# FocoosAI/focoos

Hardware: AMD Instinct MI355X
Metric: images/sec @ 640^2 (infer bs=32) (higher is better)
Workload: dtype bf16; 1 GPU; fai-detr-l-obj365 inference, bf16 MFMA, bs=32/GPU, 640x640, random-init weights (seed 0), uint8 HWC images resident in HBM, device post-process + D2H of packed detections included; global_batch=32, parallelism=replicas x1 (no data-path collective), steps_are=hipGraph replays, batches_in_flight=3, concurrent_batch_parts=1

## Files before the change

### focoos_amd/_lib.py

```python
from __future__ import annotations

import ctypes as C
import os
from typing import Optional

from .build import LIB_PATH, LIB_PATH_FP16

FX_ACT = {None: 0, "none": 0, "relu": 1, "silu": 2, "gelu": 3}


class FocoosAmdError(RuntimeError):
    pass


class FxConvDesc(C.Structure):
    _fields_ = [
        ("x", C.c_void_p), ("w", C.c_void_p), ("bias", C.c_void_p), ("residual", C.c_void_p), ("y", C.c_void_p),
        ("B", C.c_int32), ("H", C.c_int32), ("W", C.c_int32), ("C", C.c_int32), ("ldx", C.c_int32),
        ("Ho", C.c_int32), ("Wo", C.c_int32), ("N", C.c_int32), ("ldy", C.c_int32), ("ldr", C.c_int32),
        ("KH", C.c_int32), ("KW", C.c_int32), ("stride", C.c_int32), ("pad", C.c_int32),
        ("pool2", C.c_int32), ("act", C.c_int32), ("out_f32", C.c_int32), ("residual_after_act", C.c_int32),
        ("y_batch_stride", C.c_int64), ("w_frag", C.c_void_p), ("mask", C.c_void_p), ("ldm", C.c_int32), ("reserved0", C.c_int32),
    ]


def conv_frag_eligible(n: int, c: int, k: int, c32: bool = True) -> bool:
    if k == 1:
        return n % 256 == 0 and c % 256 == 0
    if k != 3:
        return False
    if c == 32:
        return c32 and n in (32, 64)
    return (n in (64, 128) or n % 256 == 0) and c % 64 == 0


class FxAugRecord(C.Structure):
    _fields_ = [
        ("crop_w", C.c_int32), ("crop_h", C.c_int32), ("pad_x", C.c_int32), ("pad_y", C.c_int32), ("res_w", C.c_int32), ("res_h", C.c_int32),
        ("crop_x", C.c_int32), ("crop_y", C.c_int32), ("flags", C.c_int32), ("reserved0", C.c_int32),
        ("brightness", C.c_float), ("contrast", C.c_float), ("saturation", C.c_float), ("reserved1", C.c_int32 * 3),
    ]


class FxPackEntry(C.Structure):
    _fields_ = [
        ("w", C.c_void_p), ("scale", C.c_void_p), ("bias", C.c_void_p), ("w_fwd", C.c_void_p), ("w_dgrad", C.c_void_p),
        ("w_fwd_frag", C.c_void_p), ("w_dgrad_frag", C.c_void_p), ("bias_out", C.c_void_p),
        ("N", C.c_int32), ("C", C.c_int32), ("KH", C.c_int32), ("KW", C.c_int32), ("ld_fwd", C.c_int32), ("ld_dgrad", C.c_int32),
        ("first_block", C.c_int32), ("n_offset", C.c_int32), ("n_total", C.c_int32), ("reserved", C.c_int32),
    ]


class FxPublishEntry(C.Structure):
    _fields_ = [
        ("w", C.c_void_p), ("bn_weight", C.c_void_p), ("bn_bias", C.c_void_p), ("bn_mean", C.c_void_p), ("bn_var", C.c_void_p),
        ("bias", C.c_void_p), ("w_rows", C.c_void_p), ("w_frag", C.c_void_p), ("bias_out", C.c_void_p), ("eps", C.c_double),
        ("N", C.c_int32), ("C", C.c_int32), ("KH", C.c_int32), ("KW", C.c_int32), ("Np", C.c_int32), ("first_block", C.c_int32),
    ]


class FxPwChainDesc(C.Structure):
    _fields_ = [
        ("x1", C.c_void_p), ("x2", C.c_void_p), ("residual", C.c_void_p), ("w1", C.c_void_p), ("bias1", C.c_void_p), ("y1", C.c_void_p),
        ("w2", C.c_void_p), ("bias2", C.c_void_p), ("y2", C.c_void_p),
        ("M", C.c_int32), ("K1a", C.c_int32), ("K1b", C.c_int32), ("N1", C.c_int32), ("N2", C.c_int32),
        ("ldx1", C.c_int32), ("ldx2", C.c_int32), ("ldr", C.c_int32), ("ldy1", C.c_int32), ("ldy2", C.c_int32),
        ("act1", C.c_int32), ("act2", C.c_int32),
        ("pool", C.c_void_p), ("ldp", C.c_int32), ("img_h", C.c_int32), ("img_w", C.c_int32), ("reserved0", C.c_int32),
    ]


class FxRcStage(C.Structure):
    _fields_ = [
        ("type", C.c_int32), ("K", C.c_int32), ("N", C.c_int32), ("act", C.c_int32),
        ("src", C.c_int32), ("dst", C.c_int32), ("aux", C.c_int32),
        ("ld", C.c_int32), ("ld2", C.c_int32), ("flags", C.c_int32),
        ("w", C.c_void_p), ("bias", C.c_void_p), ("gamma", C.c_void_p), ("beta", C.c_void_p), ("g0", C.c_void_p), ("g1", C.c_void_p),
    ]


class FxFrameDesc(C.Structure):
    _fields_ = [
        ("plane", C.c_void_p * 3), ("pitch", C.c_int32 * 3), ("height", C.c_int32), ("width", C.c_int32), ("format", C.c_int32),
        ("matrix", C.c_int32), ("reserved", C.c_int32 * 3),
    ]


_vp, _i, _f = C.c_void_p, C.c_int, C.c_float

SIGNATURES = {
    "fx_abi_version": [],
    "fx_build_flags": [],
    "fx_device_info": [_i, C.POINTER(C.c_int), C.c_char_p, _i],
    "fx_conv2d_nhwc_bf16": [C.POINTER(FxConvDesc), _vp],
    "fx_conv2d_variant": [_vp, C.c_char_p, _i],
    "fx_pw_chain_supported": [_i, _i, _i, _i],
    "fx_pw_chain_pool_supported": [_i, _i, _i, _i],
    "fx_conv3x3_flat_supported": [_i, _i, _i],
    "fx_pw_chain_bf16": [C.POINTER(FxPwChainDesc), _vp],
    "fx_stem_conv3x3s2": [_vp, _i, _vp, _vp, _vp, _vp, _vp, _i, _i, _i, _i, _vp],
    "fx_stem16_conv3x3s2": [_vp, _i, _vp, _vp, _vp, _vp, _vp, _i, _i, _i, _vp],
    "fx_conv3x3_c16_nhwc_bf16": [_vp, _i, _vp, _vp, _i, _vp, _i, _i, _i, _i, _i, _i, _i, _vp],
    "fx_semseg_eval_accumulate": [_vp, _vp, _i, _i, _i, _i, _i, _i, _i, _vp, C.c_int64, _vp, _vp, _i, _i, _vp, _vp, _vp, _vp, _vp],
    "fx_detr_eval_boxes_f32": [_vp, _vp, _vp, _i, _i, _i, _i, _vp, _vp, _vp, _vp, _vp],
    "fx_coco_match_workspace_bytes": [_i],
    "fx_coco_match_bbox": [_vp, _vp, _vp, _vp, _i, _i, _i, _vp, _vp, _vp, _vp, _vp, _vp, C.c_int64, _i, _vp, _vp, _vp, _vp, _vp, _vp, C.c_size_t,
                           _vp],
    "fx_mf_eval_masks_workspace_bytes": [_i, _i, _i],
    "fx_mf_eval_masks": [_vp, _vp, _vp, _i, _i, _i, _i, _i, _i, _i, _i, _vp, _vp, _vp, _vp, C.c_int64, _f, _vp, _vp, _vp, _vp, _vp, _vp, _vp, _vp,
                         _vp, _vp, C.c_size_t, _vp],
    "fx_coco_mask_inter": [_vp, _vp, _vp, C.c_int64, _vp, _vp, _vp, _i, _i, _i, _vp, _vp, _vp, _vp, _vp, C.c_int64, _vp, _vp, _vp, C.c_int64, _vp,
                           _vp, _vp],
    "fx_coco_match_segm": [_vp, _vp, _vp, _vp, _i, _i, _i, _i, _vp, _vp, _vp, _vp, _vp, _vp, _vp, C.c_int64, _i, _vp, _vp, _vp, _vp, _vp, _vp,
                           C.c_size_t, _vp],
    "fx_augment_images_u8": [_vp, _vp, _vp, _vp, _vp, C.c_int64, _vp, _vp, _i, _vp, _i, _i, _i, _vp, _vp],
    "fx_augment_labels": [_vp, _vp, _vp, _vp, _vp, _vp, C.c_int64, _vp, _vp, _vp, _i, _i, _vp, _i, _i, _i, _i, _vp, _vp],
    "fx_resize_bilinear_u8": [_vp, _i, _i, _vp, _i, _i, _vp],
    "fx_tile_gather_u8_f32": [_vp, _i, _i, _vp, _vp, _i, _vp, _i, _i, _vp],
    "fx_frames_ingest": [_vp, _vp, _i, _vp, _i, _i, _i, _vp],
    "fx_merge_detections_workspace_bytes": [_i, _i],
    "fx_merge_detections_nms": [_vp, _vp, _vp, _vp, _vp, _i, _i, _i, _i, _f, _i, _i, _vp, _vp, _vp, _vp, _vp, _vp, C.c_size_t, _vp],
    "fx_frames_tile_gather_f32": [_vp, _vp, _i, _vp, _vp, _i, _vp, _i, _i, _vp],
    "fx_roi_select": [_vp, _vp, _vp, _vp, _i, _i, _vp, _vp, _i, _vp, _vp, _vp, _vp, _vp, _vp, _i, _i, _i, _i, _f, _i, _vp, _vp, _vp, _vp, _vp],
    "fx_frames_roi_gather_f32": [_vp, _vp, _i, _vp, _i, _vp, _i, _i, _vp],
    "fx_roi_attributes": [_vp, _i, _vp, _vp, _i, _vp, _i, _i, _vp, _vp, _i, _vp, _vp, _vp, _vp, _vp, _i, _vp, _vp, _vp, _vp],
    "fx_merge_detections_batched_workspace_bytes": [_i, _i, _i],
    "fx_merge_detections_nms_batched": [_vp, _vp, _vp, _vp, _vp, _i, _i, _i, _i, _i, _f, _i, _i, _vp, _vp, _vp, _vp, _vp, _vp, C.c_size_t, _vp],
    "fx_annotate_labels_from_detections": [_vp, _vp, _vp, _vp, _i, _i, _vp, _vp, _i, _i, _i, _i, _i, _i, _vp, _vp],
    "fx_annotate_u8": [_vp, _vp, _i, _i, _i, _i, _i, _vp, _vp, _vp, _vp, _vp, _i, C.c_int64, _vp, _vp, _i, _i, _i, _i, _vp],
    "fx_track_update": [_vp, _vp, _vp, _vp, _i, _i, _vp, _vp, _vp, _vp, _vp, _vp, _vp, _vp, _i, _f, _f, _f, _f, _f, _i, _i, _f, _vp, _vp],
    "fx_track_reset": [_vp, _vp, _vp, _vp, _vp, _vp, _vp, _vp, _i, _i, _i, _vp],
    "fx_zone_update": [_vp, _vp, _vp, _i, _i, _vp, _vp, _i, _vp, _vp, _vp, _vp, _vp, _vp, _i, _i, _vp, _vp, _vp, _vp, _vp, _vp, _vp, _vp, _vp],
    "fx_zone_reset": [_vp, _vp, _vp, _vp, _vp, _i, _i, _i, _i, _vp],
    "fx_annotate_labels_tracked": [_vp, _vp, _vp, _vp, _vp, _i, _i, _vp, _vp, _i, _i, _i, _i, _i, _i, _vp, _vp],
    "fx_annotate_zone_records": [_vp, _vp, _vp, _vp, _vp, _vp, _i, _i, _vp, _vp, _vp, _vp, _vp, _i, _i, _i, _i, _i, _i, _vp, _vp],
    "fx_annotate_overlay_u8": [_vp, _vp, _i, _i, _i, _i, _i, _vp, _vp, _vp, _vp, _vp, _vp, _i, _i, _vp, _vp, _vp, _vp, _vp, _vp, _i, _i, _i, _i,
                               _vp],
    "fx_trace_update": [_vp, _vp, _vp, _i, _i, _vp, _vp, _i, _i, _vp, _vp, _vp, _vp, _vp, _vp],
    "fx_trace_reset": [_vp, _vp, _vp, _vp, _i, _i, _i, _vp],
    "fx_dwell_update": [_vp, _vp, _vp, _i, _i, _vp, _i, _vp, _vp, _vp, _vp, _vp, _vp, _i, _vp, _vp, _vp, _vp, _vp, _vp, _vp, _vp, _vp],
    "fx_dwell_reset": [_vp, _vp, _vp, _vp, _vp, _vp, _vp, _vp, _i, _i, _i, _i, _vp],
    "fx_heat_tiles": [_i, _i, _i],
    "fx_heat_update": [_vp, _vp, _vp, _vp, _i, _i, _i, _i, _i, _i, _i, _i, _i, _vp, _vp, _vp, _vp, _vp],
    "fx_annotate_heat_u8": [_vp, _vp, _i, _i, _i, _i, _i, _vp, _vp, _i, _i, _vp, _vp],
    "fx_redact_regions": [_vp, _vp, _vp, _i, _i, _vp, _i, _vp, _vp, _vp, _vp, _i, _i, _i, _i, _vp, _vp, _vp, _vp],
    "fx_redact_u8": [_vp, _vp, _i, _i, _i, _i, _vp, _vp, _vp, _i, _vp, _i, C.c_int64, _i, _i, _i, _i, _i, _i, _vp],
    "fx_mask_rle_workspace_bytes": [_i, _i, _i, _i],
    "fx_mask_rle_encode": [_vp, _vp, _vp, _i, _i, _i, _i, _i, _vp, _vp, _vp, _vp, C.c_size_t, _vp],
    "fx_mask_polygon_workspace_bytes": [_i, _i, _i, _i, _i],
    "fx_mask_polygon_encode": [_vp, _vp, _vp, _i, _i, _i, _i, _i, _i, _vp, _vp, _vp, _vp, C.c_size_t, _vp],
    "fx_maxpool3x3s2_nhwc_bf16": [_vp, _i, _vp, _i, _i, _i, _i, _i, _vp],
    "fx_stem_conv12_u8_bf16": [_vp, _vp, _vp, _vp, _vp, _vp, _vp, _vp, _i, _i, _i, _i, _vp],
    "fx_stem_conv_pool_supported": [_i, _i, _i, _i],
    "fx_stem_conv3x3_relu_maxpool_bf16": [_vp, _i, _vp, _vp, _vp, _i, _i, _i, _i, _vp],
    "fx_avgpool2x2_nhwc_bf16": [_vp, _i, _vp, _i, _i, _i, _i, _i, _vp],
    "fx_resize_bilinear_nhwc_bf16": [_vp, _i, _vp, _i, _i, _i, _i, _i, _i, _i, _vp],
    "fx_add_rows_bf16": [_vp, _i, _vp, _i, _i, _vp, _i, _i, _i, _vp],
    "fx_layernorm_bf16": [_vp, _i, _vp, _i, _vp, _vp, _vp, _i, _i, _i, _vp],
    "fx_mha_bf16": [_vp, _i, _vp, _i, _vp, _i, _vp, _i, _i, _i, _i, _i, _vp],
    "fx_mha_workspace_bytes": [_i, _i, _i, _i, _i],
    "fx_mha_masked_bf16": [_vp, _i, _vp, _i, _vp, _i, _vp, _i, _i, _i, _i, _i, _vp, _i, _vp, C.c_size_t, _vp],
    "fx_upsample_nearest_add_nhwc_bf16": [_vp, _i, _vp, _i, _vp, _i, _i, _i, _i, _i, _i, _i, _vp],
    "fx_upsample_nearest_bwd_nhwc_bf16": [_vp, _i, _vp, _i, _i, _i, _i, _i, _i, _i, _vp],
    "fx_query_pixel_logits_bf16": [_vp, _i, _vp, _i, _i, _vp, _i, _vp, _i, _i, _i, _i, _i, _vp],
    "fx_mf_class_head": [_vp, _i, _vp, _vp, _vp, _i, _i, _i, _vp],
    "fx_mf_upsample_probs_f32": [_vp, _i, _i, _vp, _i, _i, _i, _vp],
    "fx_mf_upsample_probs_bf16": [_vp, _i, _i, _vp, _i, _i, _i, _vp],
    "fx_mf_postprocess_workspace_bytes": [_i, _i, _i],
    "fx_mf_postprocess_workspace_bytes_fused": [_i, _i, _i, _i, _i, _i],
    "fx_mf_postprocess": [_vp, _i, _i, _i, _i, _vp, _vp, _i, _i, _f, _f, _i, _vp, C.c_size_t, _vp, _vp, _vp, _vp, _vp, _vp, _vp, _vp],
    "fx_msda_bf16": [_vp, _i, _vp, _vp, _i, _i, _vp, _i, _vp, _i, _vp, _i, _vp, _i, _i, _i, _i, _i, _vp],
    "fx_rowmax_f32": [_vp, _i, _vp, _i, _i, _vp],
    "fx_enc_score_head_bf16": [_vp, _i, _vp, _i, _vp, _vp, _vp, _vp, _f, _vp, _vp, _i, _vp, _i, _vp, _i, _vp],
    "fx_row_chain": [_vp, _i, _i, _i, _vp],
    "fx_topk_rows_f32": [_vp, _i, _i, _i, _i, _vp, _vp, _vp],
    "fx_topk_rows_workspace_bytes": [_i, _i, _i],
    "fx_topk_rows_ws_f32": [_vp, _i, _i, _i, _i, _vp, _vp, _vp, C.c_size_t, _vp],
    "fx_gather_rows_bf16": [_vp, _i, _i, _vp, _i, _vp, _i, _i, _i, _vp],
    "fx_fill_rows_bf16": [_vp, _i, _i, _vp, _i, _vp, _i, _i, _vp],
    "fx_linear_k4_relu": [_vp, _vp, _vp, _vp, _i, _i, _i, _vp],
    "fx_bbox_head": [_vp, _i, _vp, _vp, _vp, _vp, _vp, _i, _i, _vp, _vp, _i, _i, _vp],
    "fx_detr_head_out": [_vp, _i, _vp, _vp, _vp, _i, _i, _vp],
    "fx_detr_postprocess": [_vp, _vp, _vp, _vp, _i, _i, _i, _i, _f, _vp, _vp, _vp, _vp, _vp],
    "fx_detr_match_cost_f32": [_vp, _i, _vp, _vp, _vp, _vp, _i, _i, _i, _i, _f, _f, _f, _f, _f, _vp, _vp],
    "fx_lsa_f32": [_vp, _i, _i, _i, _vp, _vp, _vp, _vp],
    "fx_lsa_status_f32": [_vp, _i, _i, _i, _vp, _vp, _vp, _vp, _vp],
    "fx_detr_set_loss_workspace_bytes": [_i, _i, _i],
    "fx_detr_set_loss_f32": [_vp, _i, _vp, _vp, _vp, _vp, _vp, _vp, _i, _i, _i, _i, _f, _f, _f, _f, _f, _f, _vp, _vp, _vp],
    "fx_detr_box_loss_f32": [_vp, _vp, _vp, _vp, _vp, _vp, _i, _i, _i, _i, _f, _f, _vp, _vp, _vp, _vp, _vp],
    "fx_detr_box_loss_bwd_f32": [_vp, _vp, _vp, _i, _i, _i, _vp, _vp, _vp, _vp],
    "fx_msda_f32_fwd": [_vp, _vp, _vp, _i, _i, _vp, _vp, _vp, _i, _i, _i, _i, _vp],
    "fx_msda_f32_bwd": [_vp, _vp, _vp, _i, _i, _vp, _vp, _vp, _vp, _vp, _vp, _i, _i, _i, _i, _vp],
    "fx_msda_train_fwd": [_vp, _i, _i, _vp, _vp, _i, _i, _vp, _vp, _vp, _i, _i, _i, _i, _vp],
    "fx_msda_train_bwd": [_vp, _i, _i, _vp, _vp, _i, _i, _vp, _vp, _vp, _vp, _i, _i, _vp, _vp, _i, _i, _i, _i, _vp],
    "fx_msda_bwd_slab_supported": [_vp, _i, _i, _i, _i, _i],
    "fx_msda_prep_bf16": [_vp, _i, _vp, _i, _vp, _vp, _vp, _i, _i, _i, _i, _vp],
    "fx_msda_prep_bwd_bf16": [_vp, _vp, _vp, _vp, _vp, _i, _vp, _i, _i, _i, _i, _i, _vp],
    "fx_msda_train_bwd_slab": [_vp, _i, _i, _vp, _vp, _vp, _i, _i, _vp, _vp, _vp, _i, _vp, _i, _vp, _vp, _i, _i, _i, _i, _vp],
    "fx_adamw_workspace_bytes": [],
    "fx_adamw_step_f32": [_vp, _vp, _vp, _vp, C.c_int64, _vp, _vp, _vp, _vp, _i, _i, _f, _f, _f, _f, _vp, _vp, _vp],
    "fx_adamw_step_scaled_f32": [_vp, _vp, _vp, _vp, C.c_int64, _vp, _vp, _vp, _vp, _i, _f, _f, _f, _f, _vp, _vp, _vp, _f, _f, _i, _vp],
    "fx_conv2d_wgrad_nhwc_bf16": [_vp, _i, _vp, _i, _vp, _i, _i, _i, _i, _i, _i, _i, _i, _i, _i, _i, _vp],
    "fx_conv2d_wgrad_bias_nhwc_bf16": [_vp, _i, _vp, _i, _vp, _vp, _i, _i, _i, _i, _i, _i, _i, _i, _i, _i, _i, _vp],
    "fx_point_sample_f32": [_vp, _i, _i, _i, _vp, _vp, _vp, _vp, _i, _i, _vp],
    "fx_mask_match_cost_f32": [_vp, _i, _vp, _vp, _vp, _vp, _i, _i, _i, _i, _i, C.c_float, C.c_float, C.c_float, _i, _vp, _vp],
    "fx_mask_match_cost_workspace_bytes": [_i, _i, _i],
    "fx_mask_match_cost_ws_f32": [_vp, _i, _vp, _vp, _vp, _vp, _i, _i, _i, _i, _i, C.c_float, C.c_float, C.c_float, _i, _vp, _vp, C.c_size_t, _vp],
    "fx_mask_set_loss_workspace_bytes": [_i, _i, _i, _i],
    "fx_mask_set_loss_f32": [_vp, _i, _vp, _i, _i, _vp, _i, _i, _i, _vp, _vp, _i, _vp, _vp, _vp, _i, _vp, _i, _i, _i, _i, _i, C.c_float, C.c_float,
                             C.c_float, C.c_float, C.c_float, _vp, C.c_size_t, _vp, _vp],
    "fx_mask_set_loss_cls_f32": [_vp, _i, _vp, _i, _i, _vp, _i, _i, _i, _vp, _vp, _i, _vp, _vp, _vp, _i, _vp, _i, _i, _i, _i, _i, C.c_float, _i, C.c_float,
                                 C.c_float, C.c_float, C.c_float, C.c_float, C.c_float, _vp, C.c_size_t, _vp, _vp],
    "fx_mask_class_loss_workspace_bytes": [_i, _i],
    "fx_mask_class_loss_f32": [_vp, _i, _vp, _vp, _vp, _vp, _i, _i, _i, _i, C.c_float, C.c_float, C.c_float, C.c_float, _vp, C.c_size_t, _vp, _vp],
    "fx_mask_class_loss_bwd_f32": [_vp, _i, _vp, _vp, _vp, _vp, _i, _i, _i, _i, C.c_float, C.c_float, C.c_float, C.c_float, _vp, _vp, _i, _vp],
    "fx_dwconv3x3s2_nhwc_bf16": [_vp, _i, _vp, _vp, _vp, _i, _i, _i, _i, _i, _vp],
    "fx_dwconv3x3s2_nhwc_f32out": [_vp, _i, _vp, _vp, _vp, _i, _i, _i, _i, _i, _vp],
    "fx_global_mean_nhwc_bf16": [_vp, _i, _vp, _i, _i, _i, _i, _vp],
    "fx_pooled_linear_f32": [_vp, _i, _vp, _vp, _i, _vp, _i, _i, _i, _i, _vp],
    "fx_channel_gate_nhwc_bf16": [_vp, _i, _vp, _i, _i, _vp, _i, _vp, _i, _vp, _i, _i, _i, _i, _vp],
    "fx_seg_postprocess_workspace_bytes": [_i, _i, _i, _i, _i, _i],
    "fx_seg_postprocess": [_vp, _i, _i, _i, _i, _vp, _vp, _i, _i, C.c_float, _i, _vp, C.c_size_t, _vp, _vp, _vp, _vp, _vp, _vp, _vp, _vp, _vp],
    "fx_pack_conv_weights_f32": [_vp, _vp, _vp, _vp, _vp, _vp, _i, _i, _i, _i, _vp],
    "fx_unpack_conv_wgrad_f32": [_vp, _vp, _vp, _i, _i, _i, _i, _i, _i, _vp],
    "fx_linear_wgrad_bias_bf16": [_vp, _i, _vp, _i, _vp, _i, _vp, _i, _i, _i, _i, _i, _vp],
    "fx_conv2d_wgrad_splits": [_i, _i, _i, _i, _i, _i, _i],
    "fx_conv2d_wgrad_variant": [_i, _i, _i, _i, _i, _i, _i, _i, _i, C.c_char_p, _i],
    "fx_conv2d_wgrad_partial_nhwc_bf16": [_vp, _i, _vp, _i, _vp, C.c_int64, _i, _i, _i, _i, _i, _i, _i, _i, _i, _i, _i, _i, _vp],
    "fx_unpack_conv_wgrad_sum_f32": [_vp, C.c_int64, _i, _vp, _vp, _i, _i, _i, _i, _i, _i, _vp],
    "fx_relu_bwd_bf16": [_vp, _i, _vp, _i, _vp, _i, _vp, _i, C.c_int64, _i, _i, _vp],
    "fx_zero_insert2_nhwc_bf16": [_vp, _i, _vp, _i, _i, _i, _i, _i, _i, _i, _vp],
    "fx_avgpool2x2_bwd_nhwc_bf16": [_vp, _i, _vp, _i, _i, _i, _i, _i, _vp],
    "fx_maxpool3x3s2_bwd_nhwc_bf16": [_vp, _i, _vp, _i, _vp, _i, _i, _i, _i, _i, _vp, _vp],
    "fx_normalize_pad8": [_vp, _i, _vp, _vp, _vp, C.c_int64, _vp],
    "fx_stem_conv3x3s2_linear": [_vp, _i, _vp, _vp, _vp, _vp, _vp, _i, _i, _i, _i, _vp],
    "fx_bn_stats_bf16": [_vp, _i, _i, _vp, C.c_int64, _i, _vp],
    "fx_bn_finalize_f32": [_vp, C.c_float, _vp, _vp, C.c_float, C.c_float, _vp, _vp, _vp, _vp, _vp, _vp, _vp, _i, _vp],
    "fx_bn_apply_bf16": [_vp, _i, _i, _vp, _vp, _vp, _i, _i, _vp, _i, C.c_int64, _i, _vp],
    "fx_bn_bwd_stats_bf16": [_vp, _i, _vp, _i, _i, _vp, _i, _vp, _vp, _vp, _vp, _i, _vp, C.c_int64, _i, _vp],
    "fx_bn_bwd_apply_bf16": [_vp, _i, _vp, _i, _i, _vp, _i, _vp, _vp, _vp, _vp, _i, _vp, C.c_float, _vp, _i, _vp, _i, C.c_int64, _i, _vp, _vp, _vp],
    "fx_act_fwd_bf16": [_vp, _i, _vp, _i, C.c_int64, _i, _i, _vp],
    "fx_act_bwd_bf16": [_vp, _i, _vp, _i, _vp, _i, C.c_int64, _i, _i, _vp],
    "fx_colsum_bf16": [_vp, _i, _vp, C.c_int64, _i, _vp],
    "fx_layernorm_bwd_bf16": [_vp, _i, _vp, _i, _vp, _vp, _i, _vp, _vp, _i, _i, _vp],
    "fx_resize_bilinear_bwd_nhwc_bf16": [_vp, _i, _vp, _i, _i, _i, _i, _i, _i, _i, _vp],
    "fx_cast_f32_bf16": [_vp, _vp, C.c_int64, _vp],
    "fx_mha_bwd_workspace_bytes": [_i, _i, _i, _i],
    "fx_mha_bwd_bf16": [_vp, _i, _vp, _i, _vp, _i, _vp, _i, _vp, _i, _vp, _i, _vp, _i, _vp, _i, _i, _i, _i, _i, _vp, C.c_size_t, _vp],
    "fx_mha_masked_bwd_bf16": [_vp, _i, _vp, _i, _vp, _i, _vp, _i, _vp, _i, _vp, _i, _vp, _i, _i, _i, _i, _i, _vp, _i, _vp, C.c_size_t, _vp],
    "fx_mask_set_loss_bwd_f32": [_vp, _i, _vp, _i, _i, _vp, _i, _i, _i, _vp, _vp, _i, _vp, _vp, _vp, _i, _vp, _i, _i, _i, _i, _i, C.c_float, C.c_float,
                                 C.c_float, C.c_float, C.c_float, _vp, C.c_size_t, _vp, _vp, _i, _vp, _vp],
    "fx_mask_set_loss_cls_bwd_f32": [_vp, _i, _vp, _i, _i, _vp, _i, _i, _i, _vp, _vp, _i, _vp, _vp, _vp, _i, _vp, _i, _i, _i, _i, _i, C.c_float, _i, C.c_float,
                                     C.c_float, C.c_float, C.c_float, C.c_float, C.c_float, _vp, C.c_size_t, _vp, _vp, _i, _vp, _vp],
    "fx_planes_to_rows_bf16": [_vp, _i, _i, _vp, _i, _i, _i, _vp],
    "fx_dwconv3x3s2_bwd_nhwc_bf16": [_vp, _i, _vp, _i, _vp, _vp, _i, _vp, _i, _i, _i, _i, _vp],
    "fx_rowdot_nhwc_bf16": [_vp, _i, _vp, _i, C.c_float, _vp, _i, _i, _i, _i, _i, _vp],
    "fx_bcast_vec_nhwc_bf16": [_vp, _i, C.c_float, _vp, _i, _i, _i, _i, _vp],
    "fx_scatter_rows_bf16": [_vp, _i, _vp, _i, _vp, _i, _i, _i, _i, _vp],
    "fx_pack_entry_blocks": [_i, _i, _i, _i],
    "fx_pack_weights_many_f32": [_vp, _i, _i, _vp],
    "fx_pack_frag_bf16": [_vp, _vp, _i, _i, _vp],
    "fx_publish_entry_blocks": [_i, _i, _i, _i],
    "fx_publish_weights_f32": [_vp, _i, _i, _vp],
    "fx_pack_linear_weights_f32": [_vp, _vp, _vp, _vp, _vp, _i, _i, _i, _i, _vp],
    "fx_box_refine_f32": [_vp, _vp, _vp, C.c_int64, _f, _vp],
    "fx_box_refine_bwd_f32": [_vp, _vp, _vp, _vp, _vp, C.c_int64, _f, _vp],
    "fx_vfl_loss_bf16": [_vp, _i, _vp, _vp, _f, _f, _f, _vp, _vp, _i, C.c_int64, _i, _vp],
    "fx_stream_fork": [_vp, _vp],
    "fx_stream_join": [_vp, _vp],
    "fx_graph_begin": [_vp],
    "fx_graph_end": [_vp, C.POINTER(C.c_void_p)],
    "fx_graph_launch": [_vp, _vp],
    "fx_graph_destroy": [_vp],
    "fx_graph_time": [_vp, _vp, _i, C.POINTER(C.c_float)],
}

_libs: dict = {}
_DTYPE = [os.environ.get("FX_DTYPE", "bf16")]


def compute_dtype() -> str:
    return _DTYPE[0]


def set_compute_dtype(name: str) -> str:
    if name not in ("bf16", "fp16"):
        raise FocoosAmdError(f"compute dtype {name!r}: the engine has a bfloat16 and an fp16 (+ loss scale) build")
    prev, _DTYPE[0] = _DTYPE[0], name
    return prev


class using_compute_dtype:

    def __init__(self, name: str):
        self.name, self.prev = name, None

    def __enter__(self):
        self.prev = set_compute_dtype(self.name)
        return self

    def __exit__(self, *exc):
        _DTYPE[0] = self.prev
        return False


def act_dtype():
    import torch

    return torch.float16 if _DTYPE[0] == "fp16" else torch.bfloat16


def lib_path(name: str = None) -> str:
    if (name or _DTYPE[0]) == "fp16":
        return os.environ.get("FOCOOS_AMD_LIB_FP16", LIB_PATH_FP16)
    return os.environ.get("FOCOOS_AMD_LIB", LIB_PATH)


FX_ABI_VERSION = 27


def load(name: str = None) -> C.CDLL:
    name = name or _DTYPE[0]
    if name in _libs:
        return _libs[name]
    import torch
    path = lib_path(name)
# ... 54 lines not shown
```

### focoos_amd/csrc/conv_common.h

```cpp
#pragma once
#include "common.h"

#ifndef FX_K64_MIN_KTOT
#define FX_K64_MIN_KTOT 1024
#endif

struct ConvArgs {
  const bf16_t* x;
  const bf16_t* w;
  const float* bias;
  const bf16_t* res;
  void* y;
  int B, H, W, C, ldx;
  int Ho, Wo, N, ldy, ldr;
  int KH, KW, stride, pad;
  int act, out_f32, res_after;
  int M, Ktot, nNt, Nstore;
  unsigned x_bytes, w_bytes, r_bytes;
  int64_t y_bstride;
  const bf16_t* mask;
  int ldm;
  unsigned m_bytes;
};

template <int BK>
__device__ __forceinline__ int lds_off(int row, int chunk) {
  constexpr int CPR = BK / 8;
  if constexpr (BK >= 128) {
    return row * (BK * 2) + ((chunk ^ (row & 15)) << 4);
  } else {
    constexpr int R = 256 / (BK * 2);
    return row * (BK * 2) + ((chunk ^ ((row / R) & (CPR - 1))) << 4);
  }
}

int fx_tune(const char* env_name, int default_value);

__device__ __forceinline__ uint4 buf_load16(__amdgpu_buffer_rsrc_t r, unsigned byte_off) {
  return __builtin_bit_cast(uint4, __builtin_amdgcn_raw_buffer_load_b128(r, byte_off, 0, 0));
}
#define FX_OOB 0xFFFFFFF0u

__device__ __forceinline__ size_t fx_y_row_offset(int m, int ldy, int HW, int64_t y_bstride) {
  size_t yo = (size_t)m * ldy;
  if (y_bstride) {
    const int bb = m / HW;
    yo = (size_t)bb * y_bstride + (size_t)(m - bb * HW) * ldy;
  }
  return yo;
}

typedef int (*ConvLauncher)(const ConvArgs& c, const bf16_t* w_frag, int mode, hipStream_t stream);
int fx_c3_epilogue_mode(int act, bool has_res, int res_after);

int fx_conv_dma_bn(const ConvArgs& a);
int fx_launch_conv_dma256(const ConvArgs& c, const bf16_t* w_frag, int mode, hipStream_t stream);
int fx_launch_conv_dma128(const ConvArgs& c, const bf16_t* w_frag, int mode, hipStream_t stream);

extern "C" int fx_conv3x3_flat_supported(int C, int N, int W);
bool fx_conv3x3_flat_fits(int C, int N, int W);
int fx_launch_conv3x3_flat(const ConvArgs& c, const bf16_t* w_frag, int mode, hipStream_t stream);
int fx_launch_pw_flat(const ConvArgs& c, const bf16_t* w_frag, int mode, hipStream_t stream);
bool fx_conv3x3_kplane_supported(int C, int N, int W);
int fx_c3k_small_m_max();
int fx_launch_conv3x3_kplane(const ConvArgs& c, const bf16_t* w_frag, int mode, hipStream_t stream);
bool fx_conv3x3s2_kplane_supported(int C, int N, int Wo, int M);
int fx_launch_conv3x3s2_kplane(const ConvArgs& c, const bf16_t* w_frag, int mode, hipStream_t stream);
bool fx_pw_kplane_supported(int C, int N, int mode);
int fx_launch_pw_kplane(const ConvArgs& c, const bf16_t* w_frag, int mode, hipStream_t stream);
bool fx_conv3x3_c32_supported(int C, int N, int W, int mode);
int fx_launch_conv3x3_c32(const ConvArgs& c, const bf16_t* w_frag, int mode, hipStream_t stream);
```

### focoos_amd/csrc/conv_igemm.hip

```cpp
#include <stdio.h>

#include "conv_common.h"

template <int BM, int BN, int BK, int WM, int WN, bool POOL, int NSTAGE = 2>
__global__ __launch_bounds__(256, (BK == 32 ? 4 : 2)) void conv_igemm_kernel(const ConvArgs p) {
  constexpr int CPR = BK / 8, RPP = 256 / CPR;
  constexpr int A_PASS = BM / RPP, B_PASS = (BN + RPP - 1) / RPP;
  constexpr int WTM = BM / WM, WTN = BN / WN, TM = WTM / 32, TN = WTN / 32;
  constexpr int A_BYTES = BM * BK * 2, B_BYTES = BN * BK * 2, STAGE = A_BYTES + B_BYTES;
  constexpr int EPI_LD = BN + 4;
  static_assert(WM * WN == 4, "4 waves");
  static_assert(BM % RPP == 0, "A passes");
  extern __shared__ __attribute__((aligned(16))) unsigned char smem[];

  const int tid = threadIdx.x, lane = tid & 63, wave = tid >> 6;
  const int wm = wave / WN, wn = wave % WN;
  const int bid = fx_xcd_remap(blockIdx.x, gridDim.x);
  const int mt = bid / p.nNt, nt = bid % p.nNt;
  const int m0 = mt * BM, n0 = nt * BN;

  const __amdgpu_buffer_rsrc_t xr = __builtin_amdgcn_make_buffer_rsrc((void*)p.x, 0, p.x_bytes, 0x00020000);
  const __amdgpu_buffer_rsrc_t wr = __builtin_amdgcn_make_buffer_rsrc((void*)p.w, 0, p.w_bytes, 0x00020000);

  const int kc = tid % CPR, r_in = tid / CPR;
// ... 201 lines not shown
        } else {
          bf16_t* dst = reinterpret_cast<bf16_t*>(p.y) + yoff;
          *reinterpret_cast<uint4*>(dst) = pack_bf16x8(v);
        }
      }
    }
    if (hh + 1 < BM / HALF) __syncthreads();
  }
}

template <int BM, int BN, int BK, int WM, int WN, bool POOL, int NSTAGE = 2>
static int launch_conv(const ConvArgs& c, const bf16_t*, int, hipStream_t stream) {
  constexpr int STAGE = (BM + BN) * BK * 2;
  constexpr int EPI = 64 * (BN + 4) * 4;
  constexpr int SMEM = (NSTAGE * STAGE > EPI) ? NSTAGE * STAGE : EPI;
  auto kern = conv_igemm_kernel<BM, BN, BK, WM, WN, POOL, NSTAGE>;
  static int attr_smem = 0;
  if (!fx_ensure_dyn_smem(reinterpret_cast<const void*>(kern), SMEM, attr_smem)) return FX_ERR_RUNTIME;
  ConvArgs a = c;
  a.nNt = (a.N + BN - 1) / BN;
  int nMt = (a.M + BM - 1) / BM;
  dim3 grid(nMt * a.nNt), block(256);
  hipLaunchKernelGGL(kern, grid, block, SMEM, stream, a);
  return fx_launch_status();
}

static int conv_prepare(const fx_conv_desc* d, ConvArgs& a) {
  FX_CHECK_ARG(d && d->x && d->w && d->y);
  FX_CHECK_ARG(d->B > 0 && d->H > 0 && d->W > 0 && d->Ho > 0 && d->Wo > 0 && d->N > 0);
  FX_CHECK_ARG(d->C > 0 && d->C % 32 == 0 && d->ldx >= d->C && d->ldx % 8 == 0);
  FX_CHECK_ARG(d->KH >= 1 && d->KW >= 1 && d->stride >= 1 && d->pad >= 0);
  const int Nstore = (d->N + 7) / 8 * 8;
  FX_CHECK_ARG(d->ldy >= Nstore && d->ldy % 8 == 0);
  FX_CHECK_ARG(!d->residual || (d->ldr >= Nstore && d->ldr % 8 == 0));
  FX_CHECK_ARG(((uintptr_t)d->x % 16) == 0 && ((uintptr_t)d->w % 16) == 0 && ((uintptr_t)d->y % 16) == 0);
  FX_CHECK_ARG(!d->residual || ((uintptr_t)d->residual % 16) == 0);
  FX_CHECK_ARG(!d->bias || ((uintptr_t)d->bias % 16) == 0);
  if (d->pool2) {
    FX_CHECK_ARG(d->KH == 1 && d->KW == 1 && d->stride == 1 && d->pad == 0);
    FX_CHECK_ARG(d->Ho == (d->H + 1) / 2 && d->Wo == (d->W + 1) / 2);
  } else {
    FX_CHECK_ARG(d->Ho == (d->H + 2 * d->pad - d->KH) / d->stride + 1);
    FX_CHECK_ARG(d->Wo == (d->W + 2 * d->pad - d->KW) / d->stride + 1);
  }
  if ((int64_t)d->B * d->H * d->W >= (1ll << 31) || (int64_t)d->B * d->Ho * d->Wo >= (1ll << 31)) return FX_ERR_UNSUPPORTED;
  const int64_t x_bytes = ((int64_t)d->B * d->H * d->W - 1) * d->ldx * 2 + (int64_t)d->C * 2;
  const int64_t Npad = (int64_t)(d->N + 127) / 128 * 128;
  const int64_t w_bytes = Npad * d->KH * d->KW * d->C * 2;
  const int64_t r_bytes = d->residual ? (((int64_t)d->B * d->Ho * d->Wo - 1) * d->ldr + Nstore) * 2 : 0;
  if (x_bytes >= 0xFFFFFFF0ll || w_bytes >= 0xFFFFFFF0ll || r_bytes >= 0xFFFFFFF0ll) return FX_ERR_UNSUPPORTED;
  a.x = reinterpret_cast<const bf16_t*>(d->x);
  a.w = reinterpret_cast<const bf16_t*>(d->w);
  a.bias = d->bias;
  a.res = reinterpret_cast<const bf16_t*>(d->residual);
  a.y = d->y;
  a.B = d->B; a.H = d->H; a.W = d->W; a.C = d->C; a.ldx = d->ldx;
  a.Ho = d->Ho; a.Wo = d->Wo; a.N = d->N; a.ldy = d->ldy; a.ldr = d->ldr;
  a.KH = d->KH; a.KW = d->KW; a.stride = d->stride; a.pad = d->pad;
  a.act = d->act; a.out_f32 = d->out_f32; a.res_after = d->residual_after_act;
  a.y_bstride = d->y_batch_stride;
  FX_CHECK_ARG(d->y_batch_stride >= 0 && d->y_batch_stride % 8 == 0);
  a.M = d->B * d->Ho * d->Wo;
  a.Ktot = d->KH * d->KW * d->C;
  a.Nstore = Nstore;
  a.nNt = 0;
  a.x_bytes = (unsigned)x_bytes;
  a.w_bytes = (unsigned)w_bytes;
  a.r_bytes = (unsigned)r_bytes;
  a.mask = reinterpret_cast<const bf16_t*>(d->mask);
  a.ldm = d->ldm;
  a.m_bytes = 0;
  if (d->mask) {
    FX_CHECK_ARG(d->ldm >= Nstore && d->ldm % 8 == 0 && ((uintptr_t)d->mask % 16) == 0 && !d->out_f32 && !d->pool2);
    const int64_t m_bytes = (((int64_t)d->B * d->Ho * d->Wo - 1) * d->ldm + Nstore) * 2;
    if (m_bytes >= 0xFFFFFFF0ll) return FX_ERR_UNSUPPORTED;
    a.m_bytes = (unsigned)m_bytes;
  }
  return FX_OK;
}

enum ConvRoute {
  R_C32, R_C3K, R_C3_FLAT, R_C3_S2, R_PWK, R_PW_FLAT, R_SMALL_M, R_DMA256, R_DMA128, R_POOL,
  R_K64_N128, R_K64_N64, R_K64_N32, R_K32_N128, R_K32_N64, R_K32_N32, R_UNSUPPORTED
};

static const struct {
  const char* label;
  bool by_c;
  ConvLauncher launch;
} kRoutes[R_UNSUPPORTED] = {
     {"conv3x3_c32<%d>", false, fx_launch_conv3x3_c32},
     {"conv3x3_kplane<%d>", false, fx_launch_conv3x3_kplane},
     {"conv3x3_flat<%d>", false, fx_launch_conv3x3_flat},
     {"conv3x3s2_kplane<%d>", false, fx_launch_conv3x3s2_kplane},
     {"pw_kplane<K%d>", true, fx_launch_pw_kplane},
     {"pw_flat<K%d>", true, fx_launch_pw_flat},
     {"conv_igemm<64,64,256,1stage>", false, launch_conv<64, 64, 256, 2, 2, false, 1>},
     {"conv_igemm_dma<256,256>", false, fx_launch_conv_dma256},
     {"conv_igemm_dma<256,128>", false, fx_launch_conv_dma128},
     {"conv_igemm<128,128,64,pool>", false, launch_conv<128, 128, 64, 2, 2, true>},
     {"conv_igemm<128,128,64>", false, launch_conv<128, 128, 64, 2, 2, false>},
     {"conv_igemm<128,64,64>", false, launch_conv<128, 64, 64, 2, 2, false>},
     {"conv_igemm<128,32,64>", false, launch_conv<128, 32, 64, 4, 1, false>},
     {"conv_igemm<128,128,32>", false, launch_conv<128, 128, 32, 2, 2, false>},
     {"conv_igemm<128,64,32>", false, launch_conv<128, 64, 32, 2, 2, false>},
     {"conv_igemm<128,32,32>", false, launch_conv<128, 32, 32, 4, 1, false>},
};

static ConvRoute conv_route(const fx_conv_desc* d, const ConvArgs& a, int mode) {
  const bool frag = d->w_frag && ((uintptr_t)d->w_frag % 16) == 0 && !d->mask && !d->pool2 && !d->out_f32;
  const int c3_min_m = fx_tune("FX_CONV3_MIN_M", 5000), pw_min_m = fx_tune("FX_PW_MIN_M", 5000);
  static const int c3_on = fx_tune("FX_CONV3_FLAT", 1), c3k_on = fx_tune("FX_C3_KPLANE", 1), c32_on = fx_tune("FX_C3_C32", 1);
  if (frag && c3_on && d->stride == 1 && d->KH == 3 && d->KW == 3 && d->pad == 1 && !d->y_batch_stride &&
      ((mode >= 0 && mode <= 3) || mode == 5) && a.M >= c3_min_m) {
    if (d->C == 32) {
      if (c32_on && fx_conv3x3_c32_supported(d->C, d->N, d->W, mode)) return R_C32;
    } else if (c3k_on && fx_conv3x3_kplane_supported(d->C, d->N, d->W)) {
      return R_C3K;
    } else if (fx_conv3x3_flat_fits(d->C, d->N, d->W)) {
      return R_C3_FLAT;
    }
  }
  static const int pw_on = fx_tune("FX_PW_FLAT", 1), pwk_on = fx_tune("FX_PW_KPLANE", 1);
  if (frag && pw_on && d->stride == 1 && d->KH == 1 && d->KW == 1 && d->pad == 0 && d->C % 256 == 0 && d->N % 256 == 0 && a.M >= pw_min_m &&
      (mode == 0 || mode == 1 || (mode >= 3 && mode <= 6)))
    return (pwk_on && fx_pw_kplane_supported(d->C, d->N, mode)) ? R_PWK : R_PW_FLAT;
  static const int s2_on = fx_tune("FX_C3S2_KPLANE", 1);
  if (frag && s2_on && d->stride == 2 && d->KH == 3 && d->KW == 3 && d->pad == 1 && !d->residual && d->H == 2 * d->Ho && d->W == 2 * d->Wo &&
      a.M >= c3_min_m && (mode == 0 || mode == 1 || mode == 3) && fx_conv3x3s2_kplane_supported(d->C, d->N, d->Wo, a.M))
    return R_C3_S2;
  static const int k64_min = fx_tune("FX_K64_MIN_KTOT", FX_K64_MIN_KTOT);
  static const int small_m = fx_tune("FX_SMALL_M", 16384);
  static const int small_k = fx_tune("FX_SMALL_M_KTOT", 2048);
  if (!d->pool2 && a.M <= small_m && d->C % 256 == 0 && a.Ktot <= small_k) return R_SMALL_M;
  if (!d->pool2 && !d->mask) {
    const int bn = fx_conv_dma_bn(a);
    if (bn) return bn == 256 ? R_DMA256 : R_DMA128;
  }
  if (d->pool2) return d->C % 64 != 0 ? R_UNSUPPORTED : R_POOL;
  if ((d->C % 64 == 0) && (a.Ktot >= k64_min)) return d->N > 64 ? R_K64_N128 : (d->N > 32 ? R_K64_N64 : R_K64_N32);
  return d->N > 64 ? R_K32_N128 : (d->N > 32 ? R_K32_N64 : R_K32_N32);
}

extern "C" int fx_conv2d_nhwc_bf16(const fx_conv_desc* d, fx_stream_t stream) {
  ConvArgs a;
  const int rc = conv_prepare(d, a);
  if (rc != FX_OK) return rc;
  const int mode = fx_c3_epilogue_mode(a.act, a.res != nullptr, a.res_after);
  const ConvRoute r = conv_route(d, a, mode);
  if (r == R_UNSUPPORTED) return FX_ERR_UNSUPPORTED;
  return kRoutes[r].launch(a, reinterpret_cast<const bf16_t*>(d->w_frag), mode, reinterpret_cast<hipStream_t>(stream));
}

extern "C" int fx_conv2d_variant(const fx_conv_desc* d, char* out, int cap) {
  FX_CHECK_ARG(out && cap >= 48);
  ConvArgs a;
  const int rc = conv_prepare(d, a);
  if (rc != FX_OK) return rc;
  const ConvRoute r = conv_route(d, a, fx_c3_epilogue_mode(a.act, a.res != nullptr, a.res_after));
  if (r == R_UNSUPPORTED) return FX_ERR_UNSUPPORTED;
  snprintf(out, cap, kRoutes[r].label, kRoutes[r].by_c ? d->C : d->N);
  return FX_OK;
}
```

### focoos_amd/csrc/conv_pw_kplane.hip

```cpp
#include "kplane_common.h"

#ifndef FX_PWK_RES_DEPTH
#define FX_PWK_RES_DEPTH 3
#endif

int fx_tune(const char* env_name, int default_value);

struct PWKArgs {
  const bf16_t* x;
  const bf16_t* wp;
  const float* bias;
  const bf16_t* res;
  bf16_t* y;
  int N, ldx, ldy, ldr, M;
  int ntg;
  int HW;
  int64_t y_bstride;
  unsigned x_bytes, r_bytes;
  int rot;
};

template <int K, int ACT, int RESMODE, int TM = 4, int ABL = 0>
__global__ __launch_bounds__(256, TM == 4 ? 2 : 3) void conv_pw_kplane_kernel(const PWKArgs p) {
  constexpr int TN = 2, NW = 4, BM = TM * 32, BN = 256;
  constexpr int NTHR = 256, NDW = NTHR / 64;
  constexpr int KS = K / 16;
  constexpr int PLANE = BM * 16, XBYTES = 2 * KS * PLANE;
  constexpr int PF = 4;
  static_assert(KS % PF == 0 && (KS - 1) * PLANE < 65536, "plane offsets are 16-bit immediates");
  extern __shared__ __attribute__((aligned(16))) unsigned char smem[];
  float* biasL = reinterpret_cast<float*>(smem + XBYTES);

  const int tid = threadIdx.x, lane = tid & 63;
  const int wave = __builtin_amdgcn_readfirstlane(tid >> 6);
  const int l32 = lane & 31, half = lane >> 5;
  const int m0 = fx_xcd_remap(blockIdx.x, gridDim.x) * BM;
  const int nt_first = blockIdx.y * p.ntg;
  const int NT = min(p.N / BN, nt_first + p.ntg);
  const int cnt = NT - nt_first;
  const int rot = p.rot ? (int)(blockIdx.x % (unsigned)cnt) : 0;
  auto tile_of = [&](int k) { const int t = k + rot; return nt_first + (t >= cnt ? t - cnt : t); };

  for (int i = tid; i < p.N; i += NTHR) biasL[i] = p.bias ? p.bias[i] : 0.0f;
  {
    const __amdgpu_buffer_rsrc_t xr = __builtin_amdgcn_make_buffer_rsrc((void*)p.x, 0, p.x_bytes, 0x00020000);
    constexpr int NP = K / 8;
    static_assert(BM % 64 == 0, "64-row DMA blocks");
    for (int i = wave; i < (BM / 64) * NP; i += NDW) {
      const int blk = i / NP, c = i % NP;
      const int m = m0 + blk * 64 + lane;
      const int pln = (c & 1) * KS + (c >> 1);
      if constexpr (!(ABL & 16)) pw_dma16(xr, smem + pln * PLANE + blk * 1024, m < p.M ? (unsigned)(m * p.ldx + c * 8) * 2u : FX_OOB);
    }
  }
  f32x16 acc[TN][TM];
  bf16x8 ar[PF][TN];
  const unsigned wvoff = lane * 16;
  const bf16_t* wwave = p.wp + (size_t)(wave * TN) * KS * 512;
  auto w_ptr = [&](int a, int nt, int ks) -> const bf16_t* { return wwave + ((size_t)(nt * 8 + a) * KS + ks) * 512; };
#pragma unroll
  for (int a = 0; a < TN; ++a) {
    const bf16_t* w0 = w_ptr(a, tile_of(0), 0);
    c3_static_for<PF>([&](auto ic) {
      constexpr int i = decltype(ic)::value;
      ar[i][a] = bf16x8{0, 0, 0, 0, 0, 0, 0, 0};
      kp_ldg<i * 1024>(ar[i][a], wvoff, w0);
    });
  }
  const int lds0 = (int)(unsigned)(size_t)((__attribute__((address_space(3))) unsigned char*)smem);
  int addr[TM];
#pragma unroll
  for (int b = 0; b < TM; ++b) addr[b] = lds0 + (b * 32 + l32) * 16 + half * KS * PLANE;
  asm volatile("s_waitcnt vmcnt(0)" ::: "memory");
  __syncthreads();

  for (int kt = 0; kt < cnt; ++kt) {
    const int nt = tile_of(kt);
    const int n0 = nt * BN;
    const int ntn = kt + 1 < cnt ? tile_of(kt + 1) : nt;
#pragma unroll
    for (int a = 0; a < TN; ++a)
#pragma unroll
      for (int gq = 0; gq < 4; ++gq) {
        const float4 bb = *reinterpret_cast<const float4*>(biasL + n0 + (wave * TN + a) * 32 + 8 * gq + 4 * half);
#pragma unroll
        for (int b = 0; b < TM; ++b) {
          acc[a][b][4 * gq] = bb.x; acc[a][b][4 * gq + 1] = bb.y; acc[a][b][4 * gq + 2] = bb.z; acc[a][b][4 * gq + 3] = bb.w;
        }
      }
    bf16x8 xb[2][TM];
#pragma unroll
    for (int b = 0; b < TM; ++b) xb[0][b] = kp_lds_read<0>(addr[b]);
#pragma unroll 1
    for (int g = 0; g < KS / PF; ++g) {
      const bool last = g == KS / PF - 1;
      const bf16_t* wnext[TN];
#pragma unroll
      for (int a = 0; a < TN; ++a) wnext[a] = w_ptr(a, last ? ntn : nt, last ? 0 : (g + 1) * PF);
      const int aoff = g * PF * PLANE;
      auto kstep = [&](auto jc) {
        constexpr int j = decltype(jc)::value;
        if constexpr (TN == 1) c3_wait<(PF - 1) * TN>(ar[j][0]); else c3_wait<(PF - 1) * TN>(ar[j][0], ar[j][1]);
#pragma unroll
        for (int a = 0; a < TN; ++a) {
#pragma unroll
          for (int b = 0; b < TM; ++b) {
            if constexpr (!(ABL & 8)) acc[a][b] = FX_MFMA_32x32x16(ar[j][a], xb[j & 1][b], acc[a][b]);
            if (a == 0) {
              if constexpr (j + 1 < PF) xb[(j + 1) & 1][b] = kp_lds_read<(j + 1) * PLANE>(addr[b] + aoff);
              else xb[0][b] = kp_lds_read<PF * PLANE>(addr[b] + (last ? -PF * PLANE : aoff));
            }
            if constexpr (!(ABL & 1)) {
              if (b == TM - 1) kp_ldg<j * 1024>(ar[j][a], wvoff, wnext[a]);
            }
            __builtin_amdgcn_sched_barrier(0);
          }
        }
      };
      c3_static_for<PF>(kstep);
    }
    constexpr int RD = (FX_PWK_RES_DEPTH < TM) ? FX_PWK_RES_DEPTH : TM;
    constexpr int RS = RD + 1 > TM ? TM : RD + 1;
    uint4 rr[RS][TN * 2];
    if constexpr (ABL & 4) {
#pragma unroll
      for (int i = 0; i < RS * TN * 2; ++i) (&rr[0][0])[i] = make_uint4(0, 0, 0, 0);
    }
    auto ld_res = [&](int b, uint4* dst) {
      const int m = min(m0 + b * 32 + l32, p.M - 1);
      const bf16_t* rrow = p.res + (size_t)m * p.ldr + n0 + wave * TN * 32 + half * 8;
#pragma unroll
      for (int a = 0; a < TN; ++a)
#pragma unroll
        for (int g2 = 0; g2 < 2; ++g2) dst[a * 2 + g2] = *reinterpret_cast<const uint4*>(rrow + a * 32 + g2 * 16);
    };
    if constexpr (RESMODE != 0 && !(ABL & 4)) {
#pragma unroll
      for (int b = 0; b < RD && b < TM; ++b) ld_res(b, rr[b % RS]);
    }
#pragma unroll
    for (int b = 0; b < TM; ++b) {
      if constexpr (RESMODE != 0 && !(ABL & 4)) {
        if (b + RD < TM) ld_res(b + RD, rr[(b + RD) % RS]);
      }
      const int row = b * 32 + l32;
      const int m = m0 + row;
      bf16_t* yrow = p.y + fx_y_row_offset(m, p.ldy, p.HW, p.y_bstride) + n0 + wave * TN * 32 + half * 8;
      const bool live = m < p.M;
#pragma unroll
      for (int a = 0; a < TN; ++a)
#pragma unroll
        for (int g2 = 0; g2 < 2; ++g2) {
          unsigned pk[2][2], rq[2][2] = {{0u, 0u}, {0u, 0u}};
          if constexpr (RESMODE != 0) {
            const uint4 R = rr[b % RS][a * 2 + g2];
            rq[0][0] = R.x; rq[0][1] = R.y; rq[1][0] = R.z; rq[1][1] = R.w;
            kp_swap_rows(rq);
          }
#pragma unroll
          for (int q = 0; q < 2; ++q) {
            const int gq = 2 * g2 + q;
            float v[4];
            const float r[4] = {bf16lo_to_f32(rq[q][0]), bf16hi_to_f32(rq[q][0]), bf16lo_to_f32(rq[q][1]),
                                bf16hi_to_f32(rq[q][1])};
#pragma unroll
            for (int e = 0; e < 4; ++e) {
              v[e] = acc[a][b][4 * gq + e];
              if constexpr (RESMODE == 1) v[e] += r[e];
              v[e] = kp_act<ACT>(v[e]);
              if constexpr (RESMODE == 3) v[e] = r[e] > 0.0f ? v[e] : 0.0f;
            }
            pk[q][0] = pack_bf16x2(v[0], v[1]);
            pk[q][1] = pack_bf16x2(v[2], v[3]);
          }
          kp_swap_rows(pk);
          if (live && !((ABL & 2) && p.M > 0)) *reinterpret_cast<uint4*>(yrow + a * 32 + g2 * 16) = make_uint4(pk[0][0], pk[0][1], pk[1][0], pk[1][1]);
        }
    }
  }
#pragma unroll
  for (int i = 0; i < PF; ++i) {
    if constexpr (TN == 1) c3_wait<0>(ar[i][0]); else c3_wait<0>(ar[i][0], ar[i][1]);
  }
}

template <int K, int ACT, int RESMODE, int TM = 4, int ABL = 0>
static int launch_pwk(PWKArgs& a, hipStream_t stream) {
  constexpr int BM = TM * 32, BN = 256;
  const int smem = BM * K * 2 + a.N * 4;
  if (smem > 160 * 1024) return FX_ERR_UNSUPPORTED;
  const int mt = (a.M + BM - 1) / BM, NT = a.N / BN;
  static const int target = fx_tune("FX_PWK_TARGET_WGS", 512);
  const int want = K == 256 ? target : target / 2;
  int groups = mt >= want * 3 / 4 ? 1 : (want + mt - 1) / mt;
  if (groups > NT) groups = NT;
  a.ntg = (NT + groups - 1) / groups;
  groups = (NT + a.ntg - 1) / a.ntg;
  static const int rot = fx_tune("FX_PWK_ROT", 1);
  a.rot = rot;
  auto kern = conv_pw_kplane_kernel<K, ACT, RESMODE, TM, ABL>;
  static int attr_smem = 0;
  if (!fx_ensure_dyn_smem(reinterpret_cast<const void*>(kern), smem, attr_smem)) return FX_ERR_RUNTIME;
  hipLaunchKernelGGL(kern, dim3(mt, groups), dim3(256), smem, stream, a);
  return fx_launch_status();
}

bool fx_pw_kplane_supported(int C, int N, int mode) {
  if (N <= 0 || N % 256 != 0 || N > 4096) return false;
  static const int k512_res = fx_tune("FX_PWK_K512_RES", 1);
  if (C == 256) return mode == 0 || mode == 1 || mode == 3 || mode == 4 || mode == 5 || mode == 6;
  if (C == 512) return mode == 0 || mode == 1 || mode == 3 || (k512_res && (mode == 4 || mode == 5 || mode == 6));
  return false;
}

int fx_launch_pw_kplane(const ConvArgs& c, const bf16_t* w_frag, int mode, hipStream_t stream) {
  if (!fx_pw_kplane_supported(c.C, c.N, mode)) return FX_ERR_UNSUPPORTED;
  PWKArgs a{};
  a.x = c.x; a.wp = w_frag; a.bias = c.bias; a.res = c.res; a.y = reinterpret_cast<bf16_t*>(c.y);
  a.N = c.N; a.ldx = c.ldx; a.ldy = c.ldy; a.ldr = c.ldr; a.M = c.M;
  a.HW = c.Ho * c.Wo; a.y_bstride = c.y_bstride; a.x_bytes = c.x_bytes; a.r_bytes = c.r_bytes;
  if (c.C == 256) {
    switch (mode) {
      case 0: return launch_pwk<256, FX_ACT_RELU, 0>(a, stream);
      case 1: return launch_pwk<256, FX_ACT_SILU, 0>(a, stream);
      case 3: return launch_pwk<256, FX_ACT_NONE, 0>(a, stream);
      case 4: return launch_pwk<256, FX_ACT_RELU, 1>(a, stream);
      case 5: return launch_pwk<256, FX_ACT_NONE, 3>(a, stream);
      case 6: return launch_pwk<256, FX_ACT_NONE, 1>(a, stream);
    }
  } else {
    switch (mode) {
      case 0: return launch_pwk<512, FX_ACT_RELU, 0>(a, stream);
      case 1: return launch_pwk<512, FX_ACT_SILU, 0>(a, stream);
      case 3: return launch_pwk<512, FX_ACT_NONE, 0>(a, stream);
      case 4: return launch_pwk<512, FX_ACT_RELU, 1>(a, stream);
      case 5: return launch_pwk<512, FX_ACT_NONE, 3>(a, stream);
      case 6: return launch_pwk<512, FX_ACT_NONE, 1>(a, stream);
    }
  }
  return FX_ERR_UNSUPPORTED;
}
```

### focoos_amd/csrc/pixel_ops.hip

```cpp
#include <stdlib.h>

#include "common.h"

static int fx_env_int(const char* name, int dflt) {
  const char* v = getenv(name);
  return v ? atoi(v) : dflt;
}

template <typename TIn, bool RELU>
__global__ __launch_bounds__(256) void stem_conv_kernel(const TIn* __restrict__ x, const float* __restrict__ wt ,
                                                         const float* __restrict__ bias, const float* __restrict__ mean,
                                                         const float* __restrict__ inv_std, bf16_t* __restrict__ y, int B, int H,
                                                         int W, int Ho, int Wo) {
  __shared__ __attribute__((aligned(16))) float ws[27 * 32];
  for (int i = threadIdx.x; i < 27 * 32; i += 256) ws[i] = wt[i];
  __syncthreads();
  const int total = B * Ho * Wo;
  const int gid = blockIdx.x * 256 + threadIdx.x;
  const int o = gid >> 2, cg = gid & 3;
  if (o >= total) return;
  const int b = o / (Ho * Wo), rem = o - b * Ho * Wo;
  const int ho = rem / Wo, wo = rem - ho * Wo;
  const float m0 = mean[0], m1 = mean[1], m2 = mean[2], s0 = inv_std[0], s1 = inv_std[1], s2 = inv_std[2];
  float acc[8];
  {
    float4 b0 = *reinterpret_cast<const float4*>(bias + cg * 8), b1 = *reinterpret_cast<const float4*>(bias + cg * 8 + 4);
    acc[0] = b0.x; acc[1] = b0.y; acc[2] = b0.z; acc[3] = b0.w; acc[4] = b1.x; acc[5] = b1.y; acc[6] = b1.z; acc[7] = b1.w;
  }
#pragma unroll 1
  for (int kh = 0; kh < 3; ++kh) {
    const int hi = ho * 2 - 1 + kh;
    const int hc = min(max(hi, 0), H - 1);
#pragma unroll
    for (int kw = 0; kw < 3; ++kw) {
      const int wi = wo * 2 - 1 + kw;
      const int wc = min(max(wi, 0), W - 1);
      const bool ok = (hi == hc) && (wi == wc);
      const TIn* px = x + ((int64_t)(b * H + hc) * W + wc) * 3;
      float v[3] = {ok ? ((float)px[0] - m0) * s0 : 0.0f, ok ? ((float)px[1] - m1) * s1 : 0.0f, ok ? ((float)px[2] - m2) * s2 : 0.0f};
#pragma unroll
      for (int c = 0; c < 3; ++c) {
        const float* wr = ws + ((kh * 3 + kw) * 3 + c) * 32 + cg * 8;
        float4 w0 = *reinterpret_cast<const float4*>(wr), w1 = *reinterpret_cast<const float4*>(wr + 4);
        acc[0] = fmaf(v[c], w0.x, acc[0]); acc[1] = fmaf(v[c], w0.y, acc[1]); acc[2] = fmaf(v[c], w0.z, acc[2]); acc[3] = fmaf(v[c], w0.w, acc[3]);
        acc[4] = fmaf(v[c], w1.x, acc[4]); acc[5] = fmaf(v[c], w1.y, acc[5]); acc[6] = fmaf(v[c], w1.z, acc[6]); acc[7] = fmaf(v[c], w1.w, acc[7]);
      }
    }
  }
  if (RELU) {
#pragma unroll
    for (int n = 0; n < 8; ++n) acc[n] = fmaxf(acc[n], 0.0f);
  }
  *reinterpret_cast<uint4*>(y + (int64_t)o * 32 + cg * 8) = pack_bf16x8(acc);
}

__device__ __forceinline__ void stem_run8(__amdgpu_buffer_rsrc_t r, int a, unsigned& lo, unsigned& hi, unsigned& b8) {
  const unsigned a4 = (unsigned)a & ~3u;
  const unsigned sh = (unsigned)a & 3u;
  const unsigned d0 = __builtin_amdgcn_raw_buffer_load_b32(r, a4, 0, 0);
  const unsigned d1 = __builtin_amdgcn_raw_buffer_load_b32(r, a4 + 4u, 0, 0);
  const unsigned d2 = __builtin_amdgcn_raw_buffer_load_b32(r, a4 + 8u, 0, 0);
  lo = __builtin_amdgcn_alignbyte(d1, d0, sh);
  hi = __builtin_amdgcn_alignbyte(d2, d1, sh);
  b8 = (sh == 0 ? d2 : __builtin_amdgcn_alignbyte(0u, d2, sh)) & 0xffu;
}

__device__ __forceinline__ void stem_run9_f32(__amdgpu_buffer_rsrc_t r, int elem, float* f, float& f8) {
  const unsigned off = (unsigned)elem * 4u;
#pragma unroll
  for (int j = 0; j < 8; ++j) f[j] = __uint_as_float(__builtin_amdgcn_raw_buffer_load_b32(r, off + 4u * j, 0, 0));
  f8 = __uint_as_float(__builtin_amdgcn_raw_buffer_load_b32(r, off + 32u, 0, 0));
}

template <typename TIn, bool RELU>
__global__ __launch_bounds__(256) void stem_mfma_kernel(const TIn* __restrict__ x, unsigned x_bytes, const float* __restrict__ wt ,
                                                         const float* __restrict__ bias, const float* __restrict__ mean,
                                                         const float* __restrict__ inv_std, bf16_t* __restrict__ y, int B, int H, int W, int Ho,
                                                         int Wo, int tiles_per_wave) {
  const int lane = threadIdx.x & 63, wave = threadIdx.x >> 6;
  const int col = lane & 31, hh = lane >> 5;
  const __amdgpu_buffer_rsrc_t xr = __builtin_amdgcn_make_buffer_rsrc((void*)x, 0, x_bytes, 0x00020000);
  bf16x8 a1, a2;
  {
    float f1[8], f2[8];
#pragma unroll
    for (int j = 0; j < 8; ++j) {
      const int rr1 = hh ? 2 : 0;
      f1[j] = wt[((rr1 * 3 + j / 3) * 3 + j % 3) * 32 + col];
      if (hh == 0) f2[j] = wt[((1 * 3 + j / 3) * 3 + j % 3) * 32 + col];
      else f2[j] = j < 3 ? wt[((j * 3 + 2) * 3 + 2) * 32 + col] : 0.0f;
    }
    a1 = __builtin_bit_cast(bf16x8, pack_bf16x8(f1));
    a2 = __builtin_bit_cast(bf16x8, pack_bf16x8(f2));
  }
  const float m0 = mean[0], m1 = mean[1], m2 = mean[2], s0 = inv_std[0], s1 = inv_std[1], s2 = inv_std[2];
  const float mj[8] = {m0, m1, m2, m0, m1, m2, m0, m1}, sj[8] = {s0, s1, s2, s0, s1, s2, s0, s1};
  float bs[16];
#pragma unroll
  for (int r = 0; r < 16; ++r) bs[r] = bias[(r & 3) + 8 * (r >> 2) + 4 * hh];
  const int total = B * Ho * Wo;
  const int tile0 = (blockIdx.x * 4 + wave) * tiles_per_wave;
#pragma unroll 1
  for (int ti = 0; ti < tiles_per_wave; ++ti) {
    const int o = (tile0 + ti) * 32 + col;
    if ((tile0 + ti) * 32 >= total) break;
    const bool act = o < total;
    const int oo = act ? o : total - 1;
    const int b = oo / (Ho * Wo), rem = oo - b * Ho * Wo;
    const int ho = rem / Wo, wo = rem - ho * Wo;
    const int wi0 = 2 * wo - 1;
    const bool c0 = wi0 >= 0, c2 = wi0 + 2 < W;
    auto run = [&](int rr, float* f, float& f8) {
      const int hi_ = 2 * ho - 1 + rr;
      const bool rv = act && hi_ >= 0 && hi_ < H;
      const bool neg = wi0 < 0;
      const int elem = rv ? ((b * H + hi_) * W + (neg ? 0 : wi0)) * 3 : 0;
      float raw[8], raw8;
      if (sizeof(TIn) == 1) {
        unsigned lo, hi, b8;
        stem_run8(xr, elem, lo, hi, b8);
        if (neg) {
          b8 = (hi >> 8) & 0xffu;
          hi = __builtin_amdgcn_alignbyte(hi, lo, 1);
          lo = __builtin_amdgcn_alignbyte(lo, 0u, 1);
        }
        const unsigned w[2] = {lo, hi};
#pragma unroll
        for (int j = 0; j < 8; ++j) raw[j] = (float)((w[j >> 2] >> (8 * (j & 3))) & 0xffu);
        raw8 = (float)b8;
      } else {
        float t[8], t8;
        stem_run9_f32(xr, elem, t, t8);
#pragma unroll
        for (int j = 0; j < 8; ++j) raw[j] = neg ? (j >= 3 ? t[j - 3] : 0.0f) : t[j];
        raw8 = neg ? t[5] : t8;
      }
#pragma unroll
      for (int j = 0; j < 8; ++j) {
        const bool ok = rv && (j < 3 ? c0 : (j < 6 ? true : c2));
        f[j] = ok ? (raw[j] - mj[j]) * sj[j] : 0.0f;
      }
      f8 = (rv && c2) ? (raw8 - m2) * s2 : 0.0f;
    };
    float f1[8], fb[8], ta, tb;
    run(hh ? 2 : 0, f1, ta);
    run(1, fb, tb);
    const float ta_row0 = __shfl_xor(ta, 32, 64);
    float f2[8];
#pragma unroll
    for (int j = 0; j < 8; ++j) f2[j] = hh ? 0.0f : fb[j];
    if (hh) f2[0] = ta_row0, f2[1] = tb, f2[2] = ta;
    const bf16x8 b1 = __builtin_bit_cast(bf16x8, pack_bf16x8(f1)), b2 = __builtin_bit_cast(bf16x8, pack_bf16x8(f2));
    f32x16 acc;
#pragma unroll
    for (int r = 0; r < 16; ++r) acc[r] = bs[r];
    acc = FX_MFMA_32x32x16(a1, b1, acc);
    acc = FX_MFMA_32x32x16(a2, b2, acc);
    if (act) {
#pragma unroll
      for (int g = 0; g < 4; ++g) {
        float v0 = acc[4 * g], v1 = acc[4 * g + 1], v2 = acc[4 * g + 2], v3 = acc[4 * g + 3];
        if (RELU) v0 = fmaxf(v0, 0.0f), v1 = fmaxf(v1, 0.0f), v2 = fmaxf(v2, 0.0f), v3 = fmaxf(v3, 0.0f);
        uint2 pk;
        pk.x = pack_bf16x2(v0, v1);
        pk.y = pack_bf16x2(v2, v3);
        *reinterpret_cast<uint2*>(y + (int64_t)o * 32 + 8 * g + 4 * hh) = pk;
      }
    }
  }
}

static int stem_launch(const void* x, int in_f32, const float* w, const float* bias, const float* mean, const float* inv_std, void* y, int B,
                       int H, int W, int Cout, int relu, fx_stream_t stream_) {
  FX_CHECK_ARG(x && w && bias && mean && inv_std && y && B > 0 && H > 0 && W > 0);
  if (Cout != 32) return FX_ERR_UNSUPPORTED;
  int Ho = (H + 2 - 3) / 2 + 1, Wo = (W + 2 - 3) / 2 + 1;
  int64_t total = (int64_t)B * Ho * Wo;
  if (total * 4 >= (1ll << 31)) return FX_ERR_UNSUPPORTED;
  int grid = (int)((total * 4 + 255) / 256);
  hipStream_t stream = reinterpret_cast<hipStream_t>(stream_);
#define STEM_GO(T, R) \
  hipLaunchKernelGGL((stem_conv_kernel<T, R>), dim3(grid), dim3(256), 0, stream, (const T*)x, w, bias, mean, inv_std, (bf16_t*)y, B, H, W, Ho, Wo)
  const int64_t x_bytes = (int64_t)B * H * W * 3 * (in_f32 ? 4 : 1);
  static const int use_mfma = fx_env_int("FX_STEM_MFMA", 1);
  if (use_mfma && x_bytes < 0xFFFFFFF0ll) {
    const unsigned x_records = (unsigned)((x_bytes + 3) & ~3ll);
    const int tiles = (int)((total + 31) / 32);
    const int tpw = 8;
    const int blocks = (tiles + 4 * tpw - 1) / (4 * tpw);
#define STEM_MFMA(T, R)                                                                                                                       \
  hipLaunchKernelGGL((stem_mfma_kernel<T, R>), dim3(blocks), dim3(256), 0, stream, (const T*)x, x_records, w, bias, mean, inv_std, (bf16_t*)y, B, H, \
                     W, Ho, Wo, tpw)
    if (in_f32) {
      if (relu) STEM_MFMA(float, true); else STEM_MFMA(float, false);
    } else {
      if (relu) STEM_MFMA(uint8_t, true); else STEM_MFMA(uint8_t, false);
    }
#undef STEM_MFMA
    return fx_launch_status();
  }
  if (in_f32) {
    if (relu) STEM_GO(float, true); else STEM_GO(float, false);
  } else {
    if (relu) STEM_GO(uint8_t, true); else STEM_GO(uint8_t, false);
  }
#undef STEM_GO
  return fx_launch_status();
}

extern "C" int fx_stem_conv3x3s2(const void* x, int in_f32, const float* w, const float* bias, const float* mean, const float* inv_std,
                                 void* y, int B, int H, int W, int Cout, fx_stream_t stream_) {
  return stem_launch(x, in_f32, w, bias, mean, inv_std, y, B, H, W, Cout, 1, stream_);
}

extern "C" int fx_stem_conv3x3s2_linear(const void* x, int in_f32, const float* w, const float* bias, const float* mean, const float* inv_std,
                                        void* y, int B, int H, int W, int Cout, fx_stream_t stream_) {
  return stem_launch(x, in_f32, w, bias, mean, inv_std, y, B, H, W, Cout, 0, stream_);
}

__device__ __forceinline__ void bilinear_src(int dst, float scale, int in_size, int& i0, int& i1, float& l0, float& l1) {
  float src = scale * ((float)dst + 0.5f) - 0.5f;
  src = src < 0.0f ? 0.0f : src;
  i0 = (int)src;
  if (i0 > in_size - 1) i0 = in_size - 1;
  i1 = i0 + ((i0 < in_size - 1) ? 1 : 0);
  l1 = src - (float)i0;
  l0 = 1.0f - l1;
}

__global__ __launch_bounds__(256) void resize_u8_kernel(const uint8_t* __restrict__ x, int H, int W, float* __restrict__ y, int Ho,
                                                         int Wo, float sh, float sw) {
  int total = Ho * Wo * 3;
  for (int i = blockIdx.x * 256 + threadIdx.x; i < total; i += gridDim.x * 256) {
    int c = i % 3, p = i / 3;
    int wo = p % Wo, ho = p / Wo;
    int h0, h1, w0, w1;
    float lh0, lh1, lw0, lw1;
    bilinear_src(ho, sh, H, h0, h1, lh0, lh1);
    bilinear_src(wo, sw, W, w0, w1, lw0, lw1);
    float p00 = x[((int64_t)h0 * W + w0) * 3 + c], p01 = x[((int64_t)h0 * W + w1) * 3 + c];
    float p10 = x[((int64_t)h1 * W + w0) * 3 + c], p11 = x[((int64_t)h1 * W + w1) * 3 + c];
    y[i] = lh0 * (lw0 * p00 + lw1 * p01) + lh1 * (lw0 * p10 + lw1 * p11);
  }
}

extern "C" int fx_resize_bilinear_u8(const uint8_t* x, int H, int W, float* y, int Ho, int Wo, fx_stream_t stream_) {
  FX_CHECK_ARG(x && y && H > 0 && W > 0 && Ho > 0 && Wo > 0);
  int total = Ho * Wo * 3;
  int grid = (total + 255) / 256;
  if (grid > 4096) grid = 4096;
  hipLaunchKernelGGL(resize_u8_kernel, dim3(grid), dim3(256), 0, reinterpret_cast<hipStream_t>(stream_), x, H, W, y, Ho, Wo,
                     (float)H / (float)Ho, (float)W / (float)Wo);
  return fx_launch_status();
}

__global__ __launch_bounds__(256) void resize_nhwc_kernel(const bf16_t* __restrict__ x, int ldx, bf16_t* __restrict__ y, int ldy, int B,
                                                           int H, int W, int C8, int c8_shift, int bpr, int Ho, int Wo, float sh, float sw) {
  const unsigned bid = (unsigned)fx_xcd_remap(blockIdx.x, gridDim.x);
  const unsigned row = bid / (unsigned)bpr;
  const unsigned t = (bid - row * (unsigned)bpr) * 256u + threadIdx.x;
  if (t >= (unsigned)(Wo * C8)) return;
  const unsigned b = row / (unsigned)Ho, ho = row - b * (unsigned)Ho;
  const unsigned wo = c8_shift >= 0 ? t >> c8_shift : t / (unsigned)C8;
  const unsigned c8 = t - wo * (unsigned)C8;
  int h0, h1, w0, w1;
  float lh0, lh1, lw0, lw1;
  bilinear_src((int)ho, sh, H, h0, h1, lh0, lh1);
  bilinear_src((int)wo, sw, W, w0, w1, lw0, lw1);
  const bf16_t* base = x + (int64_t)b * H * W * ldx + c8 * 8;
  float f00[8], f01[8], f10[8], f11[8], o[8];
  unpack_bf16x8(*reinterpret_cast<const uint4*>(base + ((int64_t)h0 * W + w0) * ldx), f00);
  unpack_bf16x8(*reinterpret_cast<const uint4*>(base + ((int64_t)h0 * W + w1) * ldx), f01);
  unpack_bf16x8(*reinterpret_cast<const uint4*>(base + ((int64_t)h1 * W + w0) * ldx), f10);
  unpack_bf16x8(*reinterpret_cast<const uint4*>(base + ((int64_t)h1 * W + w1) * ldx), f11);
#pragma unroll
  for (int j = 0; j < 8; ++j) o[j] = lh0 * (lw0 * f00[j] + lw1 * f01[j]) + lh1 * (lw0 * f10[j] + lw1 * f11[j]);
  *reinterpret_cast<uint4*>(y + ((int64_t)row * Wo + wo) * ldy + c8 * 8) = pack_bf16x8(o);
}

extern "C" int fx_resize_bilinear_nhwc_bf16(const void* x, int ldx, void* y, int ldy, int B, int H, int W, int C, int Ho, int Wo,
                                            fx_stream_t stream_) {
  FX_CHECK_ARG(x && y && B > 0 && H > 0 && W > 0 && Ho > 0 && Wo > 0 && C > 0 && C % 8 == 0);
  FX_CHECK_ARG(ldx >= C && ldy >= C && ldx % 8 == 0 && ldy % 8 == 0);
  const int C8 = C / 8;
  const int64_t per_row = (int64_t)Wo * C8;
  const int64_t bpr = (per_row + 255) / 256;
  const int64_t grid = (int64_t)B * Ho * bpr;
  if (per_row >= (1ll << 31) || grid >= (1ll << 31)) return FX_ERR_UNSUPPORTED;
  const int shift = (C8 & (C8 - 1)) == 0 ? __builtin_ctz((unsigned)C8) : -1;
  hipLaunchKernelGGL(resize_nhwc_kernel, dim3((unsigned)grid), dim3(256), 0, reinterpret_cast<hipStream_t>(stream_), (const bf16_t*)x, ldx,
                     (bf16_t*)y, ldy, B, H, W, C8, shift, (int)bpr, Ho, Wo, (float)H / (float)Ho, (float)W / (float)Wo);
  return fx_launch_status();
}

__global__ __launch_bounds__(256) void maxpool_kernel(const bf16_t* __restrict__ x, int ldx, bf16_t* __restrict__ y, int ldy, int B, int H,
                                                       int W, int C8, int Ho, int Wo) {
  int64_t total = (int64_t)B * Ho * Wo * C8;
  const int bid = fx_xcd_remap(blockIdx.x, gridDim.x);
  for (int64_t i = (int64_t)bid * 256 + threadIdx.x; i < total; i += (int64_t)gridDim.x * 256) {
    int c8 = (int)(i % C8);
    int64_t p = i / C8;
    int wo = (int)(p % Wo);
    int64_t q = p / Wo;
    int ho = (int)(q % Ho), b = (int)(q / Ho);
    float m[8];
#pragma unroll
    for (int j = 0; j < 8; ++j) m[j] = -INFINITY;
#pragma unroll
    for (int kh = 0; kh < 3; ++kh) {
      int hi = ho * 2 - 1 + kh;
      if ((unsigned)hi >= (unsigned)H) continue;
#pragma unroll
      for (int kw = 0; kw < 3; ++kw) {
        int wi = wo * 2 - 1 + kw;
        if ((unsigned)wi >= (unsigned)W) continue;
        float f[8];
        unpack_bf16x8(*reinterpret_cast<const uint4*>(x + ((int64_t)(b * H + hi) * W + wi) * ldx + c8 * 8), f);
#pragma unroll
        for (int j = 0; j < 8; ++j) m[j] = fmaxf(m[j], f[j]);
      }
    }
    *reinterpret_cast<uint4*>(y + p * ldy + c8 * 8) = pack_bf16x8(m);
  }
}

extern "C" int fx_maxpool3x3s2_nhwc_bf16(const void* x, int ldx, void* y, int ldy, int B, int H, int W, int C, fx_stream_t stream_) {
  FX_CHECK_ARG(x && y && B > 0 && H > 0 && W > 0 && C > 0 && C % 8 == 0 && ldx >= C && ldy >= C && ldx % 8 == 0 && ldy % 8 == 0);
  int Ho = (H + 2 - 3) / 2 + 1, Wo = (W + 2 - 3) / 2 + 1;
  int64_t total = (int64_t)B * Ho * Wo * (C / 8);
  int64_t grid = (total + 255) / 256;
  if (grid > 256 * 256) grid = 256 * 256;
  hipLaunchKernelGGL(maxpool_kernel, dim3((int)grid), dim3(256), 0, reinterpret_cast<hipStream_t>(stream_), (const bf16_t*)x, ldx,
                     (bf16_t*)y, ldy, B, H, W, C / 8, Ho, Wo);
  return fx_launch_status();
}

__global__ __launch_bounds__(256) void avgpool2_kernel(const bf16_t* __restrict__ x, int ldx, bf16_t* __restrict__ y, int ldy, int B, int H,
                                                        int W, int C8, int Ho, int Wo) {
  int64_t total = (int64_t)B * Ho * Wo * C8;
  const int bid = fx_xcd_remap(blockIdx.x, gridDim.x);
  for (int64_t i = (int64_t)bid * 256 + threadIdx.x; i < total; i += (int64_t)gridDim.x * 256) {
    int c8 = (int)(i % C8);
    int64_t p = i / C8;
    int wo = (int)(p % Wo);
    int64_t q = p / Wo;
    int ho = (int)(q % Ho), b = (int)(q / Ho);
    float s[8] = {0, 0, 0, 0, 0, 0, 0, 0};
    int cnt = 0;
#pragma unroll
    for (int dy = 0; dy < 2; ++dy)
#pragma unroll
      for (int dx = 0; dx < 2; ++dx) {
        int hi = 2 * ho + dy, wi = 2 * wo + dx;
        if (hi < H && wi < W) {
          float f[8];
          unpack_bf16x8(*reinterpret_cast<const uint4*>(x + ((int64_t)(b * H + hi) * W + wi) * ldx + c8 * 8), f);
#pragma unroll
          for (int j = 0; j < 8; ++j) s[j] += f[j];
          ++cnt;
        }
      }
    float inv = 1.0f / (float)cnt;
#pragma unroll
    for (int j = 0; j < 8; ++j) s[j] *= inv;
    *reinterpret_cast<uint4*>(y + p * ldy + c8 * 8) = pack_bf16x8(s);
  }
}

extern "C" int fx_avgpool2x2_nhwc_bf16(const void* x, int ldx, void* y, int ldy, int B, int H, int W, int C, fx_stream_t stream_) {
  FX_CHECK_ARG(x && y && B > 0 && H > 0 && W > 0 && C > 0 && C % 8 == 0 && ldx >= C && ldy >= C && ldx % 8 == 0 && ldy % 8 == 0);
  int Ho = (H + 1) / 2, Wo = (W + 1) / 2;
  int64_t total = (int64_t)B * Ho * Wo * (C / 8);
  int64_t grid = (total + 255) / 256;
  if (grid > 256 * 32) grid = 256 * 32;
  hipLaunchKernelGGL(avgpool2_kernel, dim3((int)grid), dim3(256), 0, reinterpret_cast<hipStream_t>(stream_), (const bf16_t*)x, ldx,
                     (bf16_t*)y, ldy, B, H, W, C / 8, Ho, Wo);
  return fx_launch_status();
}
```

### focoos_amd/csrc/resize_common.h

```cpp
#pragma once
#include "common.h"

__device__ __forceinline__ void fx_resize_src(int dst, float scale, int in_size, int& i0, int& i1, float& l0, float& l1) {
#pragma clang fp contract(off)
  float src = fmaf(scale, (float)dst + 0.5f, -0.5f);
  src = src < 0.0f ? 0.0f : src;
  i0 = (int)src;
  if (i0 > in_size - 1) i0 = in_size - 1;
  i1 = i0 + ((i0 < in_size - 1) ? 1 : 0);
  l1 = src - (float)i0;
  l0 = 1.0f - l1;
}

__device__ __forceinline__ float fx_resize_filter(float lh0, float lh1, float lw0, float lw1, float p00, float p01, float p10, float p11) {
#pragma clang fp contract(off)
  const float top = fmaf(lw1, p01, lw0 * p00), bottom = fmaf(lw1, p11, lw0 * p10);
  return fmaf(lh0, top, lh1 * bottom);
}

static inline bool fx_windows_ok(const int32_t* wh, int N, int H, int W) {
  for (int i = 0; i < N; ++i) {
    const int x0 = wh[4 * i], y0 = wh[4 * i + 1], w = wh[4 * i + 2], h = wh[4 * i + 3];
    if (w <= 0 || h <= 0 || x0 < 0 || y0 < 0 || x0 > W - w || y0 > H - h) return false;
  }
  return true;
}
```

### focoos_amd/csrc/score_head.hip

```cpp
#include "pw_common.h"

struct ScoreHeadArgs {
  const bf16_t* mem;
  const uint8_t* valid;
  const bf16_t* w1p;
  const bf16_t* w2p;
  const float* b1;
  const float* gamma;
  const float* beta;
  const float* b2;
  bf16_t* om;
  float* scores;
  int ldm, ldo, S, M;
  float eps;
  unsigned mem_bytes;
};

template <int TN2>
__global__ __launch_bounds__(256, 2) void score_head_kernel(const ScoreHeadArgs p) {
  constexpr int BM = 64, TM = 2, KS = 16, PF = 4;
  extern __shared__ __attribute__((aligned(16))) unsigned char smem[];
  unsigned char* T = smem;
  float* red = reinterpret_cast<float*>(smem + BM * 512);

  const int tid = threadIdx.x, lane = tid & 63;
  const int wave = __builtin_amdgcn_readfirstlane(tid >> 6);
  const int l32 = lane & 31, half = lane >> 5;
  const int m0 = blockIdx.x * BM;

  const __amdgpu_buffer_rsrc_t mr = __builtin_amdgcn_make_buffer_rsrc((void*)p.mem, 0, p.mem_bytes, 0x00020000);
  for (int i = wave; i < BM * 32 / 64; i += 4) {
    const int q = i * 64 + lane;
    const int row = q >> 5, pc = q & 31;
    const int lc = pc ^ (row & 15);
    const int m = m0 + row;
    bool ok = m < p.M;
    if (ok && p.valid) ok = p.valid[m % p.S] != 0;
    pw_dma16(mr, T + i * 1024, ok ? (unsigned)(m * p.ldm + lc * 8) * 2u : FX_OOB);
  }

  f32x16 acc[2][TM];
#pragma unroll
  for (int a = 0; a < 2; ++a)
#pragma unroll
    for (int gq = 0; gq < 4; ++gq) {
      const float4 bb = *reinterpret_cast<const float4*>(p.b1 + wave * 64 + a * 32 + 8 * gq + 4 * half);
#pragma unroll
      for (int b = 0; b < TM; ++b) {
        acc[a][b][4 * gq] = bb.x; acc[a][b][4 * gq + 1] = bb.y; acc[a][b][4 * gq + 2] = bb.z; acc[a][b][4 * gq + 3] = bb.w;
      }
    }
  const bf16_t* w1 = p.w1p + (size_t)(wave * 2 * KS) * 512 + lane * 8;
  bf16x8 a1[PF][2];
#pragma unroll
  for (int i = 0; i < PF; ++i) {
    a1[i][0] = pw_ldg_frag(w1 + i * 512);
    a1[i][1] = pw_ldg_frag(w1 + (KS + i) * 512);
  }
  asm volatile("s_waitcnt vmcnt(0)" ::: "memory");
  __syncthreads();
#pragma unroll 1
  for (int ks0 = 0; ks0 < KS; ks0 += PF) {
    int l32k = l32;
    asm volatile("" : "+v"(l32k));
#pragma unroll
    for (int i = 0; i < PF; ++i) {
      bf16x8 xb[TM];
#pragma unroll
      for (int b = 0; b < TM; ++b) {
        const int row = b * 32 + l32k;
        xb[b] = *reinterpret_cast<const bf16x8*>(T + row * 512 + ((((ks0 + i) * 2 + half) ^ (row & 15)) << 4));
      }
#pragma unroll
      for (int a = 0; a < 2; ++a)
#pragma unroll
        for (int b = 0; b < TM; ++b) acc[a][b] = FX_MFMA_32x32x16(a1[i][a], xb[b], acc[a][b]);
      const int kn = ks0 + i + PF;
      const int kc = kn < KS ? kn : KS - 1;
      a1[i][0] = pw_ldg_frag(w1 + kc * 512);
      a1[i][1] = pw_ldg_frag(w1 + (KS + kc) * 512);
    }
  }
  const bf16_t* w2 = p.w2p + (size_t)(wave * TN2 * KS) * 512 + lane * 8;
  bf16x8 a2[PF][TN2];
#pragma unroll
  for (int i = 0; i < PF; ++i)
#pragma unroll
    for (int a = 0; a < TN2; ++a) a2[i][a] = pw_ldg_frag(w2 + (size_t)(a * KS + i) * 512);

  float mean[TM], rstd[TM];
  {
    float s[TM];
#pragma unroll
    for (int b = 0; b < TM; ++b) {
      float t = 0.0f;
#pragma unroll
      for (int a = 0; a < 2; ++a)
#pragma unroll
        for (int r = 0; r < 16; ++r) t += acc[a][b][r];
      t += __shfl_xor(t, 32);
      s[b] = t;
    }
    __syncthreads();
    if (half == 0) {
#pragma unroll
      for (int b = 0; b < TM; ++b) red[wave * 64 + b * 32 + l32] = s[b];
    }
    __syncthreads();
#pragma unroll
    for (int b = 0; b < TM; ++b) {
      const int r = b * 32 + l32;
      mean[b] = (red[r] + red[64 + r] + red[128 + r] + red[192 + r]) * (1.0f / 256.0f);
    }
#pragma unroll
    for (int b = 0; b < TM; ++b) {
      float t = 0.0f;
#pragma unroll
      for (int a = 0; a < 2; ++a)
#pragma unroll
        for (int r = 0; r < 16; ++r) {
          const float d = acc[a][b][r] - mean[b];
          t += d * d;
        }
      t += __shfl_xor(t, 32);
      s[b] = t;
    }
    __syncthreads();
    if (half == 0) {
#pragma unroll
      for (int b = 0; b < TM; ++b) red[wave * 64 + b * 32 + l32] = s[b];
    }
    __syncthreads();
#pragma unroll
    for (int b = 0; b < TM; ++b) {
      const int r = b * 32 + l32;
      rstd[b] = rsqrtf((red[r] + red[64 + r] + red[128 + r] + red[192 + r]) * (1.0f / 256.0f) + p.eps);
    }
  }
#pragma unroll
  for (int a = 0; a < 2; ++a)
#pragma unroll
    for (int gq = 0; gq < 4; ++gq) {
      const int n = wave * 64 + a * 32 + 8 * gq + 4 * half;
      const float4 gg = *reinterpret_cast<const float4*>(p.gamma + n);
      const float4 be = *reinterpret_cast<const float4*>(p.beta + n);
#pragma unroll
      for (int b = 0; b < TM; ++b) {
        const int row = b * 32 + l32;
        const float v0 = (acc[a][b][4 * gq] - mean[b]) * rstd[b] * gg.x + be.x;
        const float v1 = (acc[a][b][4 * gq + 1] - mean[b]) * rstd[b] * gg.y + be.y;
        const float v2 = (acc[a][b][4 * gq + 2] - mean[b]) * rstd[b] * gg.z + be.z;
        const float v3 = (acc[a][b][4 * gq + 3] - mean[b]) * rstd[b] * gg.w + be.w;
        uint2 o;
        o.x = pack_bf16x2(v0, v1);
        o.y = pack_bf16x2(v2, v3);
        *reinterpret_cast<uint2*>(T + row * 512 + (((n >> 3) ^ (row & 15)) << 4) + half * 8) = o;
      }
    }
  __syncthreads();
#pragma unroll
  for (int i = 0; i < BM * 32 / 256; ++i) {
    const int q = tid + i * 256;
    const int row = q >> 5, lc = q & 31;
    const uint4 v = *reinterpret_cast<const uint4*>(T + row * 512 + ((lc ^ (row & 15)) << 4));
    const int m = m0 + row;
    if (m < p.M) *reinterpret_cast<uint4*>(p.om + (size_t)m * p.ldo + lc * 8) = v;
  }
  f32x16 acc2[TN2][TM];
#pragma unroll
  for (int a = 0; a < TN2; ++a)
#pragma unroll
    for (int gq = 0; gq < 4; ++gq) {
      const float4 bb = *reinterpret_cast<const float4*>(p.b2 + (wave * TN2 + a) * 32 + 8 * gq + 4 * half);
#pragma unroll
      for (int b = 0; b < TM; ++b) {
        acc2[a][b][4 * gq] = bb.x; acc2[a][b][4 * gq + 1] = bb.y; acc2[a][b][4 * gq + 2] = bb.z; acc2[a][b][4 * gq + 3] = bb.w;
      }
    }
#pragma unroll 1
  for (int ks0 = 0; ks0 < KS; ks0 += PF) {
    int l32k = l32;
    asm volatile("" : "+v"(l32k));
#pragma unroll
    for (int i = 0; i < PF; ++i) {
      bf16x8 tb[TM];
#pragma unroll
      for (int b = 0; b < TM; ++b) {
        const int row = b * 32 + l32k;
        tb[b] = *reinterpret_cast<const bf16x8*>(T + row * 512 + ((((ks0 + i) * 2 + half) ^ (row & 15)) << 4));
      }
#pragma unroll
      for (int a = 0; a < TN2; ++a)
#pragma unroll
        for (int b = 0; b < TM; ++b) acc2[a][b] = FX_MFMA_32x32x16(a2[i][a], tb[b], acc2[a][b]);
      const int kn = ks0 + i + PF;
      const int kc = kn < KS ? kn : KS - 1;
#pragma unroll
      for (int a = 0; a < TN2; ++a) a2[i][a] = pw_ldg_frag(w2 + (size_t)(a * KS + kc) * 512);
    }
  }
  float mx[TM];
#pragma unroll
  for (int b = 0; b < TM; ++b) {
    float t = acc2[0][b][0];
#pragma unroll
    for (int a = 0; a < TN2; ++a)
#pragma unroll
      for (int r = 0; r < 16; ++r) t = fmaxf(t, acc2[a][b][r]);
    t = fmaxf(t, __shfl_xor(t, 32));
    mx[b] = t;
  }
  __syncthreads();
  if (half == 0) {
#pragma unroll
    for (int b = 0; b < TM; ++b) red[wave * 64 + b * 32 + l32] = mx[b];
  }
  __syncthreads();
  if (tid < BM && m0 + tid < p.M) p.scores[m0 + tid] = fmaxf(fmaxf(red[tid], red[64 + tid]), fmaxf(red[128 + tid], red[192 + tid]));
}

template <int TN2>
static int launch_score_head(const ScoreHeadArgs& a, hipStream_t stream) {
  constexpr int SMEM = 64 * 512 + 4 * 64 * 4;
  auto kern = score_head_kernel<TN2>;
  static int attr_smem = 0;
  if (!fx_ensure_dyn_smem(reinterpret_cast<const void*>(kern), SMEM, attr_smem)) return FX_ERR_RUNTIME;
  hipLaunchKernelGGL(kern, dim3((a.M + 63) / 64), dim3(256), SMEM, stream, a);
  return fx_launch_status();
}

extern "C" int fx_enc_score_head_bf16(const void* memory, int ldm, const uint8_t* valid, int S, const void* w1, const float* b1,
                                      const float* gamma, const float* beta, float eps, const void* w2, const float* b2, int n2_pad,
                                      void* output_memory, int ldo, float* scores, int M, fx_stream_t stream_) {
  FX_CHECK_ARG(memory && w1 && b1 && gamma && beta && w2 && b2 && output_memory && scores && M > 0 && S > 0);
  FX_CHECK_ARG(ldm >= 256 && ldm % 8 == 0 && ldo >= 256 && ldo % 8 == 0);
  FX_CHECK_ARG(((uintptr_t)memory % 16) == 0 && ((uintptr_t)w1 % 16) == 0 && ((uintptr_t)w2 % 16) == 0 && ((uintptr_t)output_memory % 16) == 0);
  FX_CHECK_ARG(((uintptr_t)b1 % 16) == 0 && ((uintptr_t)b2 % 16) == 0 && ((uintptr_t)gamma % 16) == 0 && ((uintptr_t)beta % 16) == 0);
  if (n2_pad != 128 && n2_pad != 256 && n2_pad != 384) return FX_ERR_UNSUPPORTED;
  const int64_t mem_bytes = ((int64_t)M - 1) * ldm * 2 + 512;
  if (mem_bytes >= 0xFFFFFFF0ll) return FX_ERR_UNSUPPORTED;
  ScoreHeadArgs a;
  a.mem = reinterpret_cast<const bf16_t*>(memory);
  a.valid = valid;
  a.w1p = reinterpret_cast<const bf16_t*>(w1);
  a.w2p = reinterpret_cast<const bf16_t*>(w2);
  a.b1 = b1; a.gamma = gamma; a.beta = beta; a.b2 = b2;
  a.om = reinterpret_cast<bf16_t*>(output_memory);
  a.scores = scores;
  a.ldm = ldm; a.ldo = ldo; a.S = S; a.M = M; a.eps = eps;
  a.mem_bytes = (unsigned)mem_bytes;
  hipStream_t stream = reinterpret_cast<hipStream_t>(stream_);
  if (n2_pad == 128) return launch_score_head<1>(a, stream);
  if (n2_pad == 256) return launch_score_head<2>(a, stream);
  return launch_score_head<3>(a, stream);
}
```

### focoos_amd/engine.py

```python
from __future__ import annotations

import contextlib
import ctypes as C
import functools
import math
import os
import weakref
from typing import Dict, List, Optional, Sequence, Tuple

import torch

from . import _lib
from ._lib import FX_ACT, FxConvDesc, FxPwChainDesc, FxRcStage, check
from .engine_stdc import StdcEngineMixin, StdcPlanMixin
from .state_spec import RESNET_BLOCKS

BN_EPS = 1e-5
DEFAULT_STREAMS = 2
MIN_PART_BATCH = 4
DEFAULT_PIPELINE_DEPTH = 3


def resolve_parts(B: int, nsplit: Optional[int], two_queue_safe: bool) -> int:
    if nsplit is None:
# ... 528 lines not shown
            rc(f"{li}.f1", sd[f"{p}.linear1.weight"], sd[f"{p}.linear1.bias"])
            rc(f"{li}.f2", sd[f"{p}.linear2.weight"], sd[f"{p}.linear2.bias"])
            RC[f"{li}.ffn_b"] = (None, self._dev(torch.cat([sd[f"{p}.linear1.bias"].float(), sd[f"{p}.linear2.bias"].float()])))
            self.dec_ffn = int(sd[f"{p}.linear1.weight"].shape[0])
            bb = f"{hp}.dec_bbox_classifier.{li}"
            rc(f"{li}.bb0", sd[f"{bb}.layers.0.weight"], sd[f"{bb}.layers.0.bias"])
            rc(f"{li}.bb1", sd[f"{bb}.layers.1.weight"], sd[f"{bb}.layers.1.bias"])
        self.nc_pad32 = (self.nc + 31) // 32 * 32
        rc("score", sd[f"{hp}.dec_score_classifier.{last}.weight"], sd[f"{hp}.dec_score_classifier.{last}.bias"], pad_to=self.nc_pad32)
        self.RC = RC
        self.P = P

    @staticmethod
    def _pos_embed_sine(h: int, w: int, npf: int, temperature: float = 10000.0) -> torch.Tensor:
        ys = torch.arange(h, dtype=torch.float32).view(h, 1).expand(h, w)
        xs = torch.arange(w, dtype=torch.float32).view(1, w).expand(h, w)
        i = torch.arange(npf, dtype=torch.float32)
        dim_t = temperature ** (2 * torch.div(i, 2, rounding_mode="floor") / npf)
        px, py = xs[..., None] / dim_t, ys[..., None] / dim_t
        out = torch.cat([py[..., 0::2].sin(), py[..., 1::2].cos(), px[..., 0::2].sin(), px[..., 1::2].cos()], dim=-1)
        return out.reshape(h * w, 2 * npf)

    @staticmethod
    def _anchors(shapes: Sequence[Tuple[int, int]], grid_size: float = 0.05, eps: float = 1e-2):
        out = []
        for lvl, (h, w) in enumerate(shapes):
            gy, gx = torch.meshgrid(torch.arange(h, dtype=torch.float32), torch.arange(w, dtype=torch.float32), indexing="ij")
            xy = (torch.stack([gx, gy], -1) + 0.5) / torch.tensor([w, h], dtype=torch.float32)
            wh = torch.ones_like(xy) * grid_size * (2.0 ** (2 - lvl))
            out.append(torch.cat([xy, wh], -1).reshape(h * w, 4))
        a = torch.cat(out, 0)
        valid = ((a > eps) & (a < 1 - eps)).all(-1)
        a = torch.log(a / (1 - a))
        a = torch.where(valid[:, None], a, torch.zeros_like(a))
        return a, torch.nonzero(~valid).flatten().to(torch.int32)

    def plan(self, B: int, H: int, W: int, f32_input: bool = False, nsplit: Optional[int] = None):
        return self._plan(B, H, W, f32_input, nsplit)

    def pipeline(self, B: int, H: int, W: int, depth: Optional[int] = None, f32_input: bool = False, nsplit: int = 1) -> "_Pipeline":
        return self._pipeline(B, H, W, depth, f32_input, nsplit)

    def forward(self, images: torch.Tensor, sizes: Optional[torch.Tensor] = None, threshold: Optional[float] = None,
                forced_topk: Optional[torch.Tensor] = None, use_graph: bool = True) -> "_Plan":
        return self._forward(images, sizes, threshold, forced_topk, use_graph)


def _copy_in(pl, images: torch.Tensor, sizes: Optional[torch.Tensor] = None, fill_sizes: bool = True) -> None:
    pl.input.copy_(images, non_blocking=True)
    if not fill_sizes:
        return
    if sizes is None:
        pl.sizes.copy_(torch.tensor([[pl.H, pl.W]] * pl.B, dtype=torch.int32), non_blocking=False)
    else:
        pl.sizes.copy_(sizes.to(torch.int32), non_blocking=True)


class _GraphOwner:

    graph = None
    graph_thr = None

    def _capture(self, warm_up, bodies) -> List[C.c_void_p]:
        warm_up()
        torch.cuda.current_stream(self.dev).synchronize()
        graphs = []
        for stream, body in bodies:
            check(self.lib.fx_graph_begin(C.c_void_p(stream)), "fx_graph_begin")
            try:
                body()
            finally:
                g = C.c_void_p()
                rc = self.lib.fx_graph_end(C.c_void_p(stream), C.byref(g))
            check(rc, "fx_graph_end")
            graphs.append(g)
        return graphs

    def _destroy_graphs(self) -> None:
        graphs, self.graph = self.graph, None
        for g in (graphs if isinstance(graphs, list) else [graphs]):
            if g is not None:
                check(self.lib.fx_graph_destroy(g), "fx_graph_destroy")

    def __del__(self):
        try:
            self._destroy_graphs()
        except Exception:
            pass


class _PlanBase(_GraphOwner):

    size_multiple = 32
    needed_res = (2, 3, 4, 5)

    def __init__(self, eng: _EngineBase, B: int, H: int, W: int, f32_input: bool, parent: Optional["_MultiPlan"] = None, index: int = 0):
        if H % self.size_multiple or W % self.size_multiple or H < 32 or W < 32:
            raise _lib.FocoosAmdError(f"input height/width must be multiples of {self.size_multiple} (and at least 32)")
        self.eng, self.B, self.H, self.W, self.f32_input = eng, B, H, W, f32_input
        self.parent, self.index = parent, index
        self.lib = eng.lib
        self.dev = eng.dev
        self.ops: List[Tuple] = []
        self.split_at: Optional[int] = None
        self.keep: List = []
        self.meta: Dict[int, dict] = {}
        self.bufs: Dict[str, NT] = {}
        self._win = None
        self._thr_cell = None
        self._build()

    def _new(self, name: str, B: int, H: int, W: int, Cc: int, dtype=torch.bfloat16) -> NT:
        if self._win is not None:
            b0, bs = self._win
            assert B == bs, (name, B, bs)
            full = self.bufs.get(name)
            if full is None:
                full = NT(torch.empty(self.B * H * W * Cc, dtype=dtype, device=self.dev), self.B, H, W, Cc, Cc, 0)
                self.bufs[name] = full
            return NT(full.t, bs, H, W, Cc, Cc, b0 * H * W * Cc)
        guard = int(os.environ.get("FX_GUARD", "0"))
        if guard:
            t = torch.empty(B * H * W * Cc + 2 * guard, dtype=dtype, device=self.dev)
            t.view(torch.uint8).fill_(0x5A)
            nt = NT(t, B, H, W, Cc, Cc, guard)
            self.guards = getattr(self, "guards", [])
            self.guards.append((name, t, guard))
        else:
            t = torch.empty(B * H * W * Cc, dtype=dtype, device=self.dev)
            nt = NT(t, B, H, W, Cc, Cc, 0)
        self.bufs[name] = nt
        return nt

    def check_guards(self):
        bad = []
        for name, t, g in getattr(self, "guards", []):
            u = t.view(torch.uint8)
            es = t.element_size()
            head, tail = u[: g * es], u[-g * es:]
            if not bool((head == 0x5A).all()) or not bool((tail == 0x5A).all()):
                bad.append((name, int((head != 0x5A).sum()), int((tail != 0x5A).sum())))
        return bad

    def _op(self, fn, *args):
        self.ops.append((fn, args))

    def _io(self, name: str, shape: Tuple[int, ...], dtype) -> torch.Tensor:
        if self.parent is not None:
            return self.parent.io_slice(name, shape, dtype, self.index)
        return torch.empty(*shape, dtype=dtype, device=self.dev)

    def conv(self, x: NT, pc: PackedConv, out: Optional[NT] = None, name: Optional[str] = None, stride: int = 1, act=None,
             residual: Optional[NT] = None, res_after: bool = False, pool2: bool = False, out_f32: bool = False,
             y_batch_stride: int = 0, extra_flops_per_pixel: float = 0.0) -> NT:
        assert x.C == pc.C, (name, x.C, pc.C)
        pad = (pc.KH - 1) // 2
        if pool2:
            Ho, Wo = (x.H + 1) // 2, (x.W + 1) // 2
        else:
            Ho, Wo = (x.H + 2 * pad - pc.KH) // stride + 1, (x.W + 2 * pad - pc.KW) // stride + 1
        if out is None:
            ncols = (pc.N + 7) // 8 * 8
            out = self._new(name, x.B, Ho, Wo, ncols, torch.float32 if out_f32 else torch.bfloat16)
            out.C = pc.N
        assert out.H == Ho and out.W == Wo and out.C == pc.N, (name, out.H, Ho, out.C, pc.N)
        d = FxConvDesc()
        d.x, d.w, d.bias = x.ptr, pc.w.data_ptr(), pc.b.data_ptr()
        d.residual = residual.ptr if residual is not None else None
        d.y = out.ptr
        d.B, d.H, d.W, d.C, d.ldx = x.B, x.H, x.W, x.C, x.ld
        d.Ho, d.Wo, d.N, d.ldy = Ho, Wo, pc.N, out.ld
        d.ldr = residual.ld if residual is not None else 0
        d.KH, d.KW, d.stride, d.pad = pc.KH, pc.KW, stride, pad
        d.pool2, d.act, d.out_f32 = int(pool2), FX_ACT[act], int(out_f32)
        d.residual_after_act = int(res_after)
        d.y_batch_stride = y_batch_stride
        d.w_frag = pc.wf.data_ptr() if pc.wf is not None else None
        self.keep.append(d)
        M = x.B * Ho * Wo
        flops = 2.0 * M * pc.N * pc.KH * pc.KW * pc.C + extra_flops_per_pixel * M
        label = C.create_string_buffer(64)
        check(self.lib.fx_conv2d_variant(C.byref(d), label, 64), "fx_conv2d_variant")
        variant = label.value.decode()
        alg_bytes = 2.0 * x.B * x.H * x.W * pc.C + (4.0 if out_f32 else 2.0) * M * pc.N + (2.0 * M * pc.N if residual is not None else 0.0) \
            + 2.0 * pc.N * pc.KH * pc.KW * pc.C
        self.meta[len(self.ops)] = {"kind": "conv", "variant": variant, "flops": flops, "flops_executed": flops - extra_flops_per_pixel * M, "bytes": alg_bytes,
                                    "name": name or "slice", "M": M, "N": pc.N, "K": pc.KH * pc.KW * pc.C}
        self._op(self.lib.fx_conv2d_nhwc_bf16, C.byref(d))
        return out

    def pw_chain(self, x1: NT, x2: Optional[NT], residual: Optional[NT], cc: Tuple, ca: Optional[Tuple], name1: str, name2: Optional[str],
                 pool_name: Optional[str] = None, keep_y1: bool = True):
        w1, b1, k1a, k1b, n1 = cc
        assert x1.C == k1a and (x2 is None) == (k1b == 0) and (x2 is None or x2.C == k1b), (name1, x1.C, k1a, k1b)
        M = x1.rows
        assert keep_y1 or (pool_name is not None and ca is not None)
        y1 = self._new(name1, x1.B, x1.H, x1.W, n1) if keep_y1 else None
        d = FxPwChainDesc()
        d.x1, d.ldx1, d.K1a = x1.ptr, x1.ld, k1a
        d.x2, d.ldx2, d.K1b = (x2.ptr, x2.ld, k1b) if x2 is not None else (None, 0, 0)
        d.residual, d.ldr = (residual.ptr, residual.ld) if residual is not None else (None, 0)
        d.w1, d.bias1, d.N1, d.M = w1.data_ptr(), b1.data_ptr(), n1, M
        d.y1, d.ldy1 = (y1.ptr, y1.ld) if y1 is not None else (None, 0)
        d.act1 = d.act2 = FX_ACT["relu"]
        y2, n2 = None, 0
        if ca is not None:
            w2, b2, n2 = ca
            y2 = self._new(name2, x1.B, x1.H, x1.W, n2)
            d.w2, d.bias2, d.y2, d.ldy2 = w2.data_ptr(), b2.data_ptr(), y2.ptr, y2.ld
        d.N2 = n2
        pooled = None
        if pool_name is not None:
            pooled = self._new(pool_name, x1.B, x1.H // 2, x1.W // 2, n1)
            d.pool, d.ldp, d.img_h, d.img_w = pooled.ptr, pooled.ld, x1.H, x1.W
        self.keep.append(d)
        self.meta[len(self.ops)] = {"kind": "conv", "variant": f"pw_chain<{k1a},{k1b},{n2}>" + ("+pool" if pooled is not None else "") + ("-y1" if y1 is None else ""),
                                    "flops": 2.0 * M * n1 * (k1a + k1b + n2),
                                    "name": name1 + ("+" + name2.rsplit("res_layers.", 1)[-1] if name2 else ""), "M": M, "N": n1, "K": k1a + k1b,
                                    "bytes": 2.0 * M * (k1a + k1b + (n1 if residual is not None else 0) + (n1 if y1 is not None else 0) + n2
                                                        + (n1 / 4 if pooled is not None else 0))}
        self._op(self.lib.fx_pw_chain_bf16, C.byref(d))
        if pool_name is not None:
            return y1, y2, pooled
        return y1, y2

    def linear(self, x: NT, pc: PackedConv, **kw) -> NT:
        return self.conv(x.as_rows() if (x.H != 1 or x.W != 1) else x, pc, **kw)

    def layernorm(self, x: NT, name_ln: str, out_name: str, residual: Optional[NT] = None) -> NT:
        g, b = self.eng.ln[name_ln]
        cols = int(g.numel())
        out = self._new(out_name, x.rows, 1, 1, cols)
        self._op(self.lib.fx_layernorm_bf16, x.ptr, x.ld, residual.ptr if residual is not None else None,
                 residual.ld if residual is not None else 0, g.data_ptr(), b.data_ptr(), out.ptr, out.ld, x.rows, cols)
        return out

    def add_rows(self, x: NT, y: NT, y_rows: int, out_name: str) -> NT:
        out = self._new(out_name, x.rows, 1, 1, x.C)
        self._op(self.lib.fx_add_rows_bf16, x.ptr, x.ld, y.ptr, y.ld, y_rows, out.ptr, out.ld, x.rows, x.C)
        return out

    RC_S0, RC_S1, RC_S2, RC_S3, RC_BIG, RC_REF, RC_RED, RC_LDS = 0, 16384, 32768, 49152, 65536, 131072, 131584, 132608
    RC2_REF, RC2_RED, RC2_LDS = 65536, 66048, 67072

    def _rc_program(self, stages: List[FxRcStage], rows: int, label: str, flops: float, lds: Optional[int] = None):
        arr = (FxRcStage * len(stages))(*stages)
        host = torch.frombuffer(bytearray(bytes(arr)), dtype=torch.uint8)
        dev = host.to(self.dev)
        self.keep.append(dev)
        self.meta[len(self.ops)] = {"kind": "conv", "variant": "row_chain", "flops": flops, "name": label, "M": rows, "N": 0, "K": 0}
        self._op(self.lib.fx_row_chain, dev.data_ptr(), len(stages), rows, self.RC_LDS if lds is None else lds)

    def resize(self, x: NT, out: NT):
        self._op(self.lib.fx_resize_bilinear_nhwc_bf16, x.ptr, x.ld, out.ptr, out.ld, x.B, x.H, x.W, x.C, out.H, out.W)

    def mha(self, qkv: NT, B: int, L: int, out_name: str) -> NT:
        out = self._new(out_name, B * L, 1, 1, 256)
        q, k, v = qkv.slice(0, 256), qkv.slice(256, 256), qkv.slice(512, 256)
        self._op(self.lib.fx_mha_bf16, q.ptr, q.ld, k.ptr, k.ld, v.ptr, v.ld, out.ptr, out.ld, B, L, L, 8)
        return out

    def build_backbone(self) -> Dict[int, NT]:
        e, P, B, lib = self.eng, self.eng.P, self.B, self.lib
        H, W = self.H, self.W
        bb = "pixel_decoder.backbone"
        self.input = self._io("input", (B, H, W, 3), torch.float32 if self.f32_input else torch.uint8)
        self.sizes = self._io("sizes", (B, 2), torch.int32)
        blocks = RESNET_BLOCKS[e.depth]
        feats = {}
        use_chain = int(os.environ.get("FX_PW_CHAIN", "1")) != 0
        max_stage = int(os.environ.get("FX_PW_CHAIN_MAX_STAGE", "1"))
        pc2 = P[f"{bb}.conv1.conv1_2"]
        if os.environ.get("FX_STEM12_FUSE", "1") != "0" and not self.f32_input and pc2.wf is not None and pc2.N == 32:
            x = self._new("conv1_2", B, (H + 1) // 2, (W + 1) // 2, 32)
            M2 = x.rows
            self.meta[len(self.ops)] = {"kind": "conv", "variant": "stem_c1+c2", "flops": 2.0 * M2 * 32 * (27 + 288), "flops_executed": 2.0 * M2 * 32 * (32 * 1.29 + 288),
                                        "bytes": 3.0 * B * H * W + 2.0 * M2 * 32 + 2.0 * 32 * 288, "name": "conv1_1+conv1_2", "M": M2, "N": 32, "K": 288}
            self._op(lib.fx_stem_conv12_u8_bf16, self.input.data_ptr(), e.stem_w.data_ptr(), e.stem_b.data_ptr(), e.px_mean.data_ptr(), e.px_inv_std.data_ptr(),
                     pc2.wf.data_ptr(), pc2.b.data_ptr(), x.ptr, x.ld, B, H, W)
        else:
            c1 = self._new("conv1_1", B, (H + 1) // 2, (W + 1) // 2, 32)
            self._op(lib.fx_stem_conv3x3s2, self.input.data_ptr(), int(self.f32_input), e.stem_w.data_ptr(), e.stem_b.data_ptr(),
                     e.px_mean.data_ptr(), e.px_inv_std.data_ptr(), c1.ptr, B, H, W, 32)
            x = self.conv(c1, pc2, name="conv1_2", act="relu")
        pc3 = P[f"{bb}.conv1.conv1_3"]
        if os.environ.get("FX_STEM_FUSE", "1") != "0" and pc3.wf is not None and lib.fx_stem_conv_pool_supported(x.C, pc3.N, x.H, x.W) == 1:
            mp = self._new("maxpool", B, (x.H + 1) // 2, (x.W + 1) // 2, 64)
            M3 = B * x.H * x.W
            self.meta[len(self.ops)] = {"kind": "conv", "variant": "stem_c3+pool", "flops": 2.0 * M3 * 64 * 288, "flops_executed": 2.0 * M3 * 64 * 288 * 1.37,
                                        "bytes": 2.0 * M3 * 32 + 2.0 * mp.rows * 64 + 2.0 * 64 * 288, "name": "conv1_3+maxpool", "M": M3, "N": 64, "K": 288}
            self._op(lib.fx_stem_conv3x3_relu_maxpool_bf16, x.ptr, x.ld, pc3.wf.data_ptr(), pc3.b.data_ptr(), mp.ptr, mp.ld, B, x.H, x.W)
        else:
            x = self.conv(x, pc3, name="conv1_3", act="relu")
            mp = self._new("maxpool", B, (x.H + 1) // 2, (x.W + 1) // 2, 64)
            self._op(lib.fx_maxpool3x3s2_nhwc_bf16, x.ptr, x.ld, mp.ptr, mp.ld, B, x.H, x.W, 64)
        x = mp
        seq = [(si, bi) for si in range(4) for bi in range(blocks[si])]
        a_next: Optional[NT] = None
        pooled_next: Optional[NT] = None
        use_pool = int(os.environ.get("FX_PW_CHAIN_POOL", "1")) != 0
        for idx, (si, bi) in enumerate(seq):
            p = f"{bb}.res_layers.{si}.blocks.{bi}"
            stride = 2 if (bi == 0 and si != 0) else 1
            a = a_next if a_next is not None else self.conv(x, P[f"{p}.branch2a"], name=f"{p}.a", act="relu")
            a_next = None
            bmid = self.conv(a, P[f"{p}.branch2b"], name=f"{p}.b", stride=stride, act="relu")
            short_in = None
            if bi == 0:
                short_in = x
                if stride == 2 and pooled_next is not None:
                    short_in, pooled_next = pooled_next, None
                elif stride == 2:
                    short_in = self._new(f"{p}.pool", x.B, (x.H + 1) // 2, (x.W + 1) // 2, x.C)
                    self._op(lib.fx_avgpool2x2_nhwc_bf16, x.ptr, x.ld, short_in.ptr, short_in.ld, x.B, x.H, x.W, x.C)
            nxt = seq[idx + 1] if idx + 1 < len(seq) else None
            cc = e.chain_c.get((si, bi)) if (use_chain and si <= max_stage) else None
            n2 = 0
            if cc is not None:
                ca = e.chain_a.get(nxt) if nxt is not None else None
                if ca is not None and lib.fx_pw_chain_supported(cc[2], cc[3], cc[4], ca[2]) == 1:
                    n2 = ca[2]
                elif lib.fx_pw_chain_supported(cc[2], cc[3], cc[4], 0) != 1:
                    cc = None
            if cc is not None:
                nxt_name = f"{bb}.res_layers.{nxt[0]}.blocks.{nxt[1]}.a" if n2 else None
                want_pool = (use_pool and nxt is not None and nxt[0] == si + 1 and bi != 0 and bmid.H % 2 == 0 and bmid.W % 2 == 0
                             and lib.fx_pw_chain_pool_supported(cc[2], cc[3], cc[4], n2) == 1)
                if want_pool:
                    keep = bool(n2 == 0 or (si + 2) in self.needed_res or os.environ.get("FX_SKIP_UNUSED_RES", "1") == "0")
                    x, a_next, pooled_next = self.pw_chain(bmid, short_in, x, cc, e.chain_a[nxt] if n2 else None, f"{p}.c", nxt_name,
                                                           pool_name=f"{bb}.res_layers.{nxt[0]}.blocks.0.pool", keep_y1=keep)
                else:
                    x, a_next = self.pw_chain(bmid, short_in, None if bi == 0 else x, cc, e.chain_a[nxt] if n2 else None, f"{p}.c", nxt_name)
            else:
                short = x if bi != 0 else self.conv(short_in, P[f"{p}.short" if si == 0 else f"{p}.short.conv"], name=f"{p}.s")
                x = self.conv(bmid, P[f"{p}.branch2c"], name=f"{p}.c", residual=short, act="relu")
            if bi == blocks[si] - 1:
                feats[si + 2] = x
        for k, v in feats.items():
            if v is not None:
                self.bufs[f"res{k}"] = v
        return feats

    def patch_args(self, fn, args, thr: float):
        return args

    def _launch(self, ops, stream: int, thr: float):
        for fn, args in ops:
            check(fn(*self.patch_args(fn, args, thr), C.c_void_p(stream)), fn.__name__)

    def capture_and_launch(self, stream: int, thr: float):
        if self.graph is None or self.graph_thr != thr:
            self._destroy_graphs()
            launch = functools.partial(self._launch, self.ops, stream, thr)
            self.graph, self.graph_thr = self._capture(launch, [(stream, launch)])[0], thr
        check(self.lib.fx_graph_launch(self.graph, C.c_void_p(stream)), "fx_graph_launch")

    def _run_forced(self, stream: int, thr: float, forced):
        raise _lib.FocoosAmdError(f"{type(self).__name__} has no teacher forcing")

    def run(self, stream: int, thr: float, forced=None, use_graph: bool = True):
        if forced is not None:
            self._run_forced(stream, thr, forced)
        elif not use_graph:
            self._launch(self.ops, stream, thr)
        else:
            self.capture_and_launch(stream, thr)

    def time_graph(self, stream: int, iters: int) -> float:
        ms = C.c_float(0)
        check(self.lib.fx_graph_time(self.graph, C.c_void_p(stream), iters, C.byref(ms)), "fx_graph_time")
        return ms.value


class _Plan(StdcPlanMixin, _PlanBase):

    needed_res = (3, 4, 5)
    size_multiple = 1

    def _build(self):
        e, P, B, lib = self.eng, self.eng.P, self.B, self.lib
        H, W = self.H, self.W
        feats = self.build_stdc() if e.stdc else self.build_backbone()
        fd = e.fd
        pd = "pixel_decoder"
        (h8, w8), (h16, w16), (h32, w32) = ((feats[k].H, feats[k].W) for k in (3, 4, 5))
        if h8 * w8 + h16 * w16 + h32 * w32 < e.nq:
            raise _lib.FocoosAmdError(f"input {H}x{W} gives {h8 * w8 + h16 * w16 + h32 * w32} encoder tokens, fewer than the {e.nq} queries to select")
        cat80 = self._new("cat80", B, h8, w8, 2 * fd)
        cat40a = self._new("cat40a", B, h16, w16, 2 * fd)
        cat40b = self._new("cat40b", B, h16, w16, 2 * fd)
        cat20 = self._new("cat20", B, h32, w32, 2 * fd)
        self.conv(feats[3], P[f"{pd}.input_proj.0"], out=cat80.slice(fd, fd))
        self.conv(feats[4], P[f"{pd}.input_proj.1"], out=cat40a.slice(fd, fd))
        src = self.conv(feats[5], P[f"{pd}.input_proj.2"], name="proj5")
        L = h32 * w32
        if e.n_enc > 0:
            pos = e._pos_embed_sine(h32, w32, 128).to(device=self.dev, dtype=torch.bfloat16).contiguous()
            self.pos = NT(pos, L, 1, 1, 256, 256)
            s = src.as_rows()
            for li in range(e.n_enc):
                p = f"{pd}.encoder.0.layers.{li}"
                qk_in = self.add_rows(s, self.pos, L, f"aifi{li}.qk_in")
                qkv = self._new(f"aifi{li}.qkv", B * L, 1, 1, 768)
                self.linear(qk_in, P[f"{p}.qk"], out=qkv.slice(0, 512))
                self.linear(s, P[f"{p}.v"], out=qkv.slice(512, 256))
                att = self.mha(qkv, B, L, f"aifi{li}.att")
                o = self.linear(att, P[f"{p}.out_proj"], name=f"aifi{li}.o", residual=s)
                s1 = self.layernorm(o, f"{p}.norm1", f"aifi{li}.s1")
                f1 = self.linear(s1, P[f"{p}.linear1"], name=f"aifi{li}.f1", act="gelu")
                f2 = self.linear(f1, P[f"{p}.linear2"], name=f"aifi{li}.f2", residual=s1)
                s = self.layernorm(f2, f"{p}.norm2", f"aifi{li}.s2")
            self.bufs["aifi"] = s
            src = NT(s.t, B, h32, w32, 256, 256, s.off)

        def csp(xin: NT, p: str, out_name: str) -> NT:
            c12 = self.conv(xin, P[f"{p}.conv12"], name=f"{p}.c12", act="silu")
            x1 = c12.slice(0, fd)
            for j in range(3):
                last = j == 2
                x1 = self.conv(x1, P[f"{p}.bottlenecks.{j}.rep"], name=out_name if last else f"{p}.rep{j}", act="silu",
                               residual=c12.slice(fd, fd) if last else None, res_after=True,
                               extra_flops_per_pixel=2.0 * fd * fd)
            return x1

        lat0 = self.conv(src, P[f"{pd}.lateral_convs.0"], out=cat20.slice(fd, fd), act="silu")
        self.resize(lat0, cat40a.slice(0, fd))
        fpn0 = csp(cat40a, f"{pd}.fpn_blocks.0", "fpn0")
        lat1 = self.conv(fpn0, P[f"{pd}.lateral_convs.1"], out=cat40b.slice(fd, fd), act="silu")
        self.resize(lat1, cat80.slice(0, fd))
        out80 = csp(cat80, f"{pd}.fpn_blocks.1", "enc_s8")
        d0 = self._new("down0", B, h16, w16, fd)
        self.resize(out80, d0)
        self.conv(d0, P[f"{pd}.downsample_convs.0"], out=cat40b.slice(0, fd), act="silu")
        out40 = csp(cat40b, f"{pd}.pan_blocks.0", "enc_s16")
        d1 = self._new("down1", B, h32, w32, fd)
        self.resize(out40, d1)
        self.conv(d1, P[f"{pd}.downsample_convs.1"], out=cat20.slice(0, fd), act="silu")
        out20 = csp(cat20, f"{pd}.pan_blocks.1", "enc_s32")
        hp = "head.predictor"
        shapes = [(h32, w32), (h16, w16), (h8, w8)]
        S = sum(a * b for a, b in shapes)
        self.S = S
        starts = [0, shapes[0][0] * shapes[0][1], shapes[0][0] * shapes[0][1] + shapes[1][0] * shapes[1][1]]
        memory = self._new("memory", B, S, 1, 256)
        for i, (f, st) in enumerate(zip((out20, out40, out80), starts)):
            lvl = NT(memory.t, B, f.H, f.W, 256, 256, memory.off + st * 256)
            self.conv(f, P[f"{hp}.input_proj.{i}"], out=lvl, y_batch_stride=S * 256)
        mem_rows = memory.as_rows()
        anchors, invalid = e._anchors(shapes)
        self.anchors = anchors.to(self.dev).contiguous()
        self.invalid = invalid.to(self.dev).contiguous()
        self.shapes_t = torch.tensor(shapes, dtype=torch.int32, device=self.dev)
        self.starts_t = torch.tensor(starts, dtype=torch.int32, device=self.dev)
        Q, K = e.nq, e.nc
        self.enc_scores = self._io("enc_scores", (B, S), torch.float32)
        if e.score_head is not None and int(os.environ.get("FX_SCORE_HEAD", "1")) != 0:
            w1, b1, w2, b2, ncp = e.score_head
            valid = torch.ones(S, dtype=torch.uint8)
            valid[invalid.long()] = 0
            self.valid_u8 = valid.to(self.dev)
            om = self._new("output_memory", B * S, 1, 1, 256)
            g_, b_ = e.ln[f"{hp}.enc_output.1"]
            self.meta[len(self.ops)] = {"kind": "conv", "variant": f"score_head<{ncp}>", "flops": 2.0 * B * S * 256 * (256 + K), "name": "enc_output+enc_score+max",
                                        "M": B * S, "N": 256 + K, "K": 256, "bytes": 2.0 * B * S * 256 * 2 + 4.0 * B * S}
            self._op(lib.fx_enc_score_head_bf16, mem_rows.ptr, mem_rows.ld, self.valid_u8.data_ptr(), S, w1.data_ptr(), b1.data_ptr(), g_.data_ptr(),
                     b_.data_ptr(), C.c_float(1e-5), w2.data_ptr(), b2.data_ptr(), ncp, om.ptr, om.ld, self.enc_scores.data_ptr(), B * S)
        else:
            om_lin = self.linear(mem_rows, P[f"{hp}.enc_output.0"], name="om_lin")
            om = self.layernorm(om_lin, f"{hp}.enc_output.1", "output_memory")
            self._op(lib.fx_fill_rows_bf16, om.ptr, om.ld, S, self.invalid.data_ptr(), int(self.invalid.numel()), e.invalid_row.data_ptr(), B, 256)
            enc_logits = self.linear(om, P[f"{hp}.enc_score"], name="enc_logits", out_f32=True)
            self._op(lib.fx_rowmax_f32, enc_logits.ptr, enc_logits.ld, self.enc_scores.data_ptr(), B * S, K)
        self.enc_topk_val = self._io("enc_topk_val", (B, Q), torch.float32)
        self.enc_topk = self._io("enc_topk", (B, Q), torch.int32)
        self._op(lib.fx_topk_rows_f32, self.enc_scores.data_ptr(), S, B, S, Q, self.enc_topk_val.data_ptr(), self.enc_topk.data_ptr())
        self.split_at = len(self.ops)
        R = B * Q
        tgt = self._new("target", R, 1, 1, 256)
        self._op(lib.fx_gather_rows_bf16, om.ptr, om.ld, S, self.enc_topk.data_ptr(), Q, tgt.ptr, tgt.ld, B, 256)
        hb = self.linear(tgt, P[f"{hp}.enc_bbox.0"], name="encbb.0", act="relu")
        hb = self.linear(hb, P[f"{hp}.enc_bbox.1"], name="encbb.1", act="relu")
        self.ref_unact = torch.empty(R, 4, dtype=torch.float32, device=self.dev)
        refs = [torch.empty(R, 4, dtype=torch.float32, device=self.dev) for _ in range(e.nl + 1)]
        wl, bl = e.bbox_last["enc"]
        self._op(lib.fx_bbox_head, hb.ptr, hb.ld, wl.data_ptr(), bl.data_ptr(), None, self.anchors.data_ptr(), self.enc_topk.data_ptr(), Q, 1,
                 refs[0].data_ptr(), self.ref_unact.data_ptr(), R, 256)
        value = self.linear(mem_rows, P[f"{hp}.value_all"], name="value_all")
        if int(os.environ.get("FX_ROW_CHAIN", "1")) != 0 and e.hd == 256:
            logits = self._build_decoder_row_chain(tgt, refs, value, R, B, Q, S)
        else:
            logits = self._build_decoder_per_op(tgt, refs, value, R, B, Q, S)
        self.refs = refs
        self.probs = self._io("probs", (B, Q, K), torch.float32)
        self.boxes = self._io("boxes", (B, Q, 4), torch.float32)
        self._op(lib.fx_detr_head_out, logits.ptr, logits.ld, refs[e.nl].data_ptr(), self.probs.data_ptr(), self.boxes.data_ptr(), R, K)
        tk = min(e.top_k, Q * K)
        self.top_k = tk
        self.det_scores = self._io("det_scores", (B, tk), torch.float32)
        self.det_flat = self._io("det_flat", (B, tk), torch.int32)
        self.det_labels = self._io("det_labels", (B, tk), torch.int32)
        self.det_queries = self._io("det_queries", (B, tk), torch.int32)
        self.det_boxes = self._io("det_boxes", (B, tk, 4), torch.int32)
        self.det_count = self._io("det_count", (B,), torch.int32)
        nws = int(lib.fx_topk_rows_workspace_bytes(B, Q * K, tk))
        self.topk_ws = torch.empty(max(nws, 8), dtype=torch.uint8, device=self.dev)
        self.keep.append(self.topk_ws)
        self._op(lib.fx_topk_rows_ws_f32, self.probs.data_ptr(), Q * K, B, Q * K, tk, self.det_scores.data_ptr(), self.det_flat.data_ptr(),
                 self.topk_ws.data_ptr(), C.c_size_t(self.topk_ws.numel()))
        self.post_index = len(self.ops)
        self._op(lib.fx_detr_postprocess, self.det_scores.data_ptr(), self.det_flat.data_ptr(), self.boxes.data_ptr(), self.sizes.data_ptr(), B, Q,
                 K, tk, None, self.det_labels.data_ptr(), self.det_queries.data_ptr(), self.det_boxes.data_ptr(), self.det_count.data_ptr())

    def _build_decoder_per_op(self, tgt: NT, refs, value: NT, R: int, B: int, Q: int, S: int) -> NT:
        e, P, lib = self.eng, self.eng.P, self.lib
        hp = "head.predictor"
        qp1 = self._new("qpos_h", R, 1, 1, 512)
        for li in range(e.nl):
            p = f"{hp}.decoder.layers.{li}"
            ref = refs[li]
            self._op(lib.fx_linear_k4_relu, ref.data_ptr(), e.qpos0[0].data_ptr(), e.qpos0[1].data_ptr(), qp1.ptr, qp1.ld, R, 512)
            qpos = self.linear(qp1, P[f"{hp}.qpos1"], name=f"dec{li}.qpos")
            qk_in = self.add_rows(tgt, qpos, R, f"dec{li}.qk_in")
            qkv = self._new(f"dec{li}.qkv", R, 1, 1, 768)
            self.linear(qk_in, P[f"{p}.qk"], out=qkv.slice(0, 512))
            self.linear(tgt, P[f"{p}.v"], out=qkv.slice(512, 256))
            att = self.mha(qkv, B, Q, f"dec{li}.att")
            o = self.linear(att, P[f"{p}.out_proj"], name=f"dec{li}.o", residual=tgt)
            t1 = self.layernorm(o, f"{p}.norm1", f"dec{li}.t1")
            q2 = self.add_rows(t1, qpos, R, f"dec{li}.q2")
            offaw = self.linear(q2, P[f"{p}.cross_attn.offaw"], name=f"dec{li}.offaw", out_f32=True)
            ms = self._new(f"dec{li}.msda", R, 1, 1, 256)
            vsl = value.slice(li * 256, 256)
            self._op(lib.fx_msda_bf16, vsl.ptr, vsl.ld, self.shapes_t.data_ptr(), self.starts_t.data_ptr(), 3, 4, offaw.ptr, offaw.ld,
                     offaw.ptr + 192 * 4, offaw.ld, ref.data_ptr(), 1, ms.ptr, ms.ld, B, S, Q, 8)
            o2 = self.linear(ms, P[f"{p}.cross_attn.output_proj"], name=f"dec{li}.o2", residual=t1)
            t2 = self.layernorm(o2, f"{p}.norm2", f"dec{li}.t2")
            f1 = self.linear(t2, P[f"{p}.linear1"], name=f"dec{li}.f1", act="relu")
            f2 = self.linear(f1, P[f"{p}.linear2"], name=f"dec{li}.f2", residual=t2)
            tgt = self.layernorm(f2, f"{p}.norm3", f"dec{li}.out")
            hb = self.linear(tgt, P[f"{hp}.dec_bbox.{li}.0"], name=f"dec{li}.bb0", act="relu")
            hb = self.linear(hb, P[f"{hp}.dec_bbox.{li}.1"], name=f"dec{li}.bb1", act="relu")
            wl, bl = e.bbox_last[f"dec{li}"]
            self._op(lib.fx_bbox_head, hb.ptr, hb.ld, wl.data_ptr(), bl.data_ptr(), ref.data_ptr(), None, None, Q, 0, refs[li + 1].data_ptr(),
                     None, R, 256)
        logits = self.linear(tgt, P[f"{hp}.dec_score"], name="logits", out_f32=True)
        return logits

    def _build_decoder_row_chain(self, tgt: NT, refs, value: NT, R: int, B: int, Q: int, S: int) -> NT:
        e, lib = self.eng, self.lib
        RC = e.RC
        S0, S1, S2, S3, BIG, REF, RED = self.RC_S0, self.RC_S1, self.RC_S2, self.RC_S3, self.RC_BIG, self.RC_REF, self.RC_RED
        relu = FX_ACT["relu"]

        def st(type_, K=0, N=0, act=0, src=-1, dst=-1, aux=-1, ld=0, ld2=0, flags=0, w=None, bias=None, gamma=None, beta=None, g0=None, g1=None):
            s_ = FxRcStage()
            s_.type, s_.K, s_.N, s_.act, s_.src, s_.dst, s_.aux, s_.ld, s_.ld2, s_.flags = type_, K, N, act, src, dst, aux, ld, ld2, flags
            s_.w, s_.bias, s_.gamma, s_.beta, s_.g0, s_.g1 = w, bias, gamma, beta, g0, g1
            return s_

        def load(nt: NT, dst):
            return st(0, K=nt.C, dst=dst, g0=nt.ptr, ld=nt.ld)

        def gemm(key, src, K, N, dst=-1, act=0, out: Optional[NT] = None, f32=False):
            w, b = RC[key]
            return st(1, K=K, N=N, act=act, src=src, dst=dst, w=w.data_ptr(), bias=b.data_ptr(), g0=out.ptr if out is not None else None,
                      ld=out.ld if out is not None else 0, flags=int(f32))

        def gemm_ln(key, src, K, aux, ln_name, dst, out: Optional[NT] = None):
            w, b = RC[key]
            g_, b_ = e.ln[ln_name]
            return st(2, K=K, N=256, src=src, dst=dst, aux=aux, w=w.data_ptr(), bias=b.data_ptr(), gamma=g_.data_ptr(), beta=b_.data_ptr(),
                      g0=out.ptr if out is not None else None, ld=out.ld if out is not None else 0, ld2=RED)

        hp = "head.predictor"
        qkv = self._new("dec.qkv", R, 1, 1, 768)
        qpos = self._new("dec.qpos", R, 1, 1, 256)
        t1 = self._new("dec.t1", R, 1, 1, 256)
        offaw = self._new("dec.offaw", R, 1, 1, 288, torch.float32)
        ncp = e.nc_pad32
        logits = self._new("logits", R, 1, 1, ncp, torch.float32)
        logits.C = e.nc

        hidden = int(e.dec_ffn)
        lean = os.environ.get("FX_RC_LEAN", "1") != "0" and hidden % 256 == 0 and hidden <= 2048
        if lean:
            REF, RED = self.RC2_REF, self.RC2_RED
        lds = self.RC2_LDS if lean else None

        def gemm_ln(key, src, K, aux, ln_name, dst, out: Optional[NT] = None):
            w, b = RC[key]
            g_, b_ = e.ln[ln_name]
            return st(2, K=K, N=256, src=src, dst=dst, aux=aux, w=w.data_ptr(), bias=b.data_ptr(), gamma=g_.data_ptr(), beta=b_.data_ptr(),
                      g0=out.ptr if out is not None else None, ld=out.ld if out is not None else 0, ld2=RED)

        def ffn_ln(li, src, res, slot_a, slot_b, ln_name, dst, out: Optional[NT] = None):
            g_, b_ = e.ln[ln_name]
            return st(7, K=256, N=hidden, act=slot_a, flags=slot_b, src=src, aux=res, dst=dst, w=RC[f"{li}.f1"][0].data_ptr(), g1=RC[f"{li}.f2"][0].data_ptr(),
                      bias=RC[f"{li}.ffn_b"][1].data_ptr(), gamma=g_.data_ptr(), beta=b_.data_ptr(), g0=out.ptr if out is not None else None,
                      ld=out.ld if out is not None else 0, ld2=RED)

        def pre_attention(li, tgt_slot, ref_global=None):
            if lean:
                assert tgt_slot == S3
                k4 = st(4, N=512, dst=S0, ld2=S1, flags=4, aux=(-1 if ref_global is not None else REF), w=e.qpos0[0].data_ptr(), bias=e.qpos0[1].data_ptr(),
                        g0=ref_global)
                w, b = RC["qpos1"]
                q1 = st(1, K=512, N=256, src=S0, aux=S1, dst=S2, flags=4, w=w.data_ptr(), bias=b.data_ptr(), g0=qpos.ptr, ld=qpos.ld)
                return [k4, q1, st(3, K=256, src=S3, aux=S2, dst=S0), gemm(f"{li}.qk", S0, 256, 512, out=qkv.slice(0, 512)),
                        gemm(f"{li}.v", S3, 256, 256, out=qkv.slice(512, 256))]
            k4 = st(4, N=512, dst=BIG, aux=(-1 if ref_global is not None else REF), w=e.qpos0[0].data_ptr(), bias=e.qpos0[1].data_ptr(), g0=ref_global)
            return [k4, gemm("qpos1", BIG, 512, 256, dst=S1, out=qpos), st(3, K=256, src=tgt_slot, aux=S1, dst=S2),
                    gemm(f"{li}.qk", S2, 256, 512, out=qkv.slice(0, 512)), gemm(f"{li}.v", tgt_slot, 256, 256, out=qkv.slice(512, 256))]

        fl_pre = 2.0 * R * (512 * 256 + 256 * 768)
        first_slot = S3 if lean else S0
        self._rc_program([load(tgt, first_slot)] + pre_attention(0, first_slot, refs[0].data_ptr()), R, "dec0.pre", fl_pre, lds)
        for li in range(e.nl):
            p = f"{hp}.decoder.layers.{li}"
            att = self.mha(qkv, B, Q, f"dec{li}.att")
            prog = [load(att, S0), load(tgt, S1), load(qpos, S2), gemm_ln(f"{li}.o", S0, 256, S1, f"{p}.norm1", S3, out=t1),
                    st(3, K=256, src=S3, aux=S2, dst=S0), gemm(f"{li}.offaw", S0, 256, 288, out=offaw, f32=True)]
            self._rc_program(prog, R, f"dec{li}.post_attn", 2.0 * R * 256 * (256 + 288), lds)
            ms = self._new(f"dec{li}.msda", R, 1, 1, 256)
            vsl = value.slice(li * 256, 256)
            self._op(lib.fx_msda_bf16, vsl.ptr, vsl.ld, self.shapes_t.data_ptr(), self.starts_t.data_ptr(), 3, 4, offaw.ptr, offaw.ld,
                     offaw.ptr + 192 * 4, offaw.ld, refs[li].data_ptr(), 1, ms.ptr, ms.ld, B, S, Q, 8)
            out = self._new(f"dec{li}.out", R, 1, 1, 256)
            wl, bl = e.bbox_last[f"dec{li}"]
            last = li == e.nl - 1
            if lean:
                ffn = [ffn_ln(li, S2, S2, S0, S1, f"{p}.norm3", S3, out=out)]
            else:
# ... 157 lines not shown
```

### include/focoos_amd.h

```cpp
#ifndef FOCOOS_AMD_H
#define FOCOOS_AMD_H

#include <stddef.h>
#include <stdint.h>

#ifdef __cplusplus
extern "C" {
#endif

#define FX_ABI_VERSION 27

enum { FX_OK = 0, FX_ERR_INVALID_ARGUMENT = -1, FX_ERR_LAUNCH = -2, FX_ERR_UNSUPPORTED = -3, FX_ERR_RUNTIME = -4 };
enum { FX_ACT_NONE = 0, FX_ACT_RELU = 1, FX_ACT_SILU = 2, FX_ACT_GELU = 3 };
enum { FX_CLASS_LOSS_CE = 0, FX_CLASS_LOSS_FOCAL = 1, FX_CLASS_LOSS_BCE = 2, FX_CLASS_LOSS_BCE_FOCAL = 3 };

typedef void* fx_stream_t;

int fx_abi_version(void);
int fx_build_flags(void);
const char* fx_error_string(int code);
int fx_device_info(int device, int* cu_count, char* arch_name, int arch_name_len);

typedef struct fx_conv_desc {
  const void* x;
  const void* w;
  const float* bias;
  const void* residual;
  void* y;
  int32_t B, H, W, C, ldx;
  int32_t Ho, Wo, N, ldy, ldr;
  int32_t KH, KW, stride, pad;
  int32_t pool2;
  int32_t act;
  int32_t out_f32;
  int32_t residual_after_act;
  int64_t y_batch_stride;
  const void* w_frag;
  const void* mask;
  int32_t ldm, reserved0;
} fx_conv_desc;
int fx_conv2d_nhwc_bf16(const fx_conv_desc* d, fx_stream_t stream);
int fx_conv2d_variant(const fx_conv_desc* d, char* out, int cap);
int fx_conv3x3_flat_supported(int C, int N, int W);

typedef struct fx_pw_chain_desc {
  const void* x1;
  const void* x2;
  const void* residual;
  const void* w1;
  const float* bias1;
  void* y1;
  const void* w2;
  const float* bias2;
  void* y2;
  int32_t M, K1a, K1b, N1, N2;
  int32_t ldx1, ldx2, ldr, ldy1, ldy2;
  int32_t act1, act2;
  void* pool;
  int32_t ldp, img_h, img_w, reserved0;
} fx_pw_chain_desc;
int fx_pw_chain_supported(int K1a, int K1b, int N1, int N2);
int fx_pw_chain_pool_supported(int K1a, int K1b, int N1, int N2);
int fx_pw_chain_bf16(const fx_pw_chain_desc* d, fx_stream_t stream);

int fx_stem_conv3x3s2(const void* x, int in_f32, const float* w, const float* bias, const float* mean,
                      const float* inv_std, void* y, int B, int H, int W, int Cout, fx_stream_t stream);

int fx_stem_conv12_u8_bf16(const void* x_u8, const float* w1, const float* b1, const float* mean, const float* inv_std, const void* w2_frag,
                           const float* b2, void* y, int ldy, int B, int H, int W, fx_stream_t stream);

int fx_stem16_conv3x3s2(const void* x, int in_f32, const float* w, const float* bias, const float* mean, const float* inv_std, void* y, int B,
                        int H, int W, fx_stream_t stream);
int fx_conv3x3_c16_nhwc_bf16(const void* x, int ldx, const void* w_frag, const float* bias, int relu, void* y, int ldy, int B, int H, int W, int C,
                             int N, int stride, fx_stream_t stream);

int fx_semseg_eval_accumulate(const float* mask_probs, const float* probs, int B, int Q, int K, int h, int w, int Hin, int Win, const int32_t* sizes,
                              int64_t max_pixels, const void* gt, const int64_t* gt_off, int gt_int32, int ignore_label, int64_t* conf,
                              int32_t* status, int32_t* pred, float* score, fx_stream_t stream);

int fx_detr_eval_boxes_f32(const int32_t* idx, const float* boxes, const int32_t* sizes, int B, int Q, int K, int T,
                           int32_t* label, float* xyxy, int32_t* keep, float* xywh, fx_stream_t stream);

size_t fx_coco_match_workspace_bytes(int max_gt);
int fx_coco_match_bbox(const int32_t* label, const float* score, const int32_t* keep, const float* xywh, int B, int T, int K,
                       const double* gt_box, const int32_t* gt_cat, const int32_t* gt_flag, const double* gt_area, const int64_t* gt_off,
                       const int64_t* gt_off_host, int64_t n_gt, int max_gt, int32_t* rank, uint64_t* matched, uint64_t* ignored,
                       int64_t* npig, int32_t* status, void* ws, size_t ws_bytes, fx_stream_t stream);

size_t fx_mf_eval_masks_workspace_bytes(int B, int Q, int max_h);
int fx_mf_eval_masks(const float* mask_probs, const float* val, const int32_t* idx, int B, int Q, int K, int T, int h, int w, int Hin, int Win,
                     const int32_t* sizes, const int32_t* sizes_host, const int64_t* word_off, const int64_t* word_off_host, int64_t n_words,
                     float mask_threshold, void* words, int32_t* qlist, int32_t* nref, int32_t* count, int32_t* box, float* psum, int32_t* label,
                     int32_t* query, float* score, void* ws, size_t ws_bytes, fx_stream_t stream);
int fx_coco_mask_inter(const void* words, const int64_t* word_off, const int64_t* word_off_host, int64_t n_words, const int32_t* qlist,
                       const int32_t* nref, const int32_t* box, int B, int Q, int T, const int32_t* sizes, const int32_t* sizes_host,
                       const void* gt_words, const int64_t* gt_word_off, const int64_t* gt_word_off_host, int64_t n_gt_words,
                       const int32_t* gt_box, const int64_t* gt_off, const int64_t* gt_off_host, int64_t n_gt, int32_t* inter, int32_t* gcount,
                       fx_stream_t stream);
int fx_coco_match_segm(const int32_t* label, const float* score, const int32_t* query, const int32_t* dcount, int B, int T, int K, int Q,
                       const int32_t* inter, const int32_t* gcount, const int32_t* gt_cat, const int32_t* gt_flag, const double* gt_area,
                       const int64_t* gt_off, const int64_t* gt_off_host, int64_t n_gt, int max_gt, int32_t* rank, uint64_t* matched,
                       uint64_t* ignored, int64_t* npig, int32_t* status, void* ws, size_t ws_bytes, fx_stream_t stream);

typedef struct fx_aug_record {
  int32_t crop_w, crop_h, pad_x, pad_y, res_w, res_h, crop_x, crop_y, flags, reserved0;
  float brightness, contrast, saturation;
  int32_t reserved1[3];
} fx_aug_record;

int fx_augment_images_u8(const uint8_t* src, const int64_t* src_off, const int32_t* sizes, const fx_aug_record* recs, const int64_t* src_off_host,
                         int64_t src_bytes, const int32_t* sizes_host, const fx_aug_record* recs_host, int B, uint8_t* dst, int Ho, int Wo,
                         int pad_value, uint64_t* mean_ws, fx_stream_t stream);

int fx_augment_labels(const void* src, const int64_t* src_off, const int32_t* plane_rec, const int32_t* sizes, const fx_aug_record* recs,
                      const int64_t* src_off_host, int64_t src_count, const int32_t* plane_rec_host, const int32_t* sizes_host,
                      const fx_aug_record* recs_host, int P, int B, void* dst, int Ho, int Wo, int elem_int32, int pad_value, int32_t* flags,
                      fx_stream_t stream);

int fx_resize_bilinear_u8(const uint8_t* x, int H, int W, float* y, int Ho, int Wo, fx_stream_t stream);

int fx_tile_gather_u8_f32(const uint8_t* frame, int H, int W, const int32_t* windows, const int32_t* windows_host, int N, float* y, int Ho, int Wo,
                          fx_stream_t stream);

#define FX_MERGE_NMS_CAP 4096
enum { FX_MERGE_IOU = 0, FX_MERGE_IOS = 1 };
size_t fx_merge_detections_workspace_bytes(int N, int T);
int fx_merge_detections_nms(const float* det_scores, const int32_t* det_labels, const int32_t* det_boxes, const int32_t* det_count,
                            const int32_t* windows, int N, int T, int frame_h, int frame_w, float merge_threshold, int metric, int max_detections,
                            float* out_scores, int32_t* out_labels, int32_t* out_boxes, int32_t* out_count, int32_t* status, void* workspace,
                            size_t workspace_bytes, fx_stream_t stream);

size_t fx_merge_detections_batched_workspace_bytes(int S, int V, int T);
int fx_merge_detections_nms_batched(const float* det_scores, const int32_t* det_labels, const int32_t* det_boxes, const int32_t* det_count,
                                    const int32_t* windows, int S, int V, int T, int frame_h, int frame_w, float merge_threshold, int metric,
                                    int max_detections, float* out_scores, int32_t* out_labels, int32_t* out_boxes, int32_t* out_count,
                                    int32_t* status, void* workspace, size_t workspace_bytes, fx_stream_t stream);

#define FX_ANN_LNAME 24
#define FX_ANN_LMAX 32
#define FX_ANN_GLYPHS 95
#define FX_ANN_MAX_DIM 16384
enum { FX_ANN_BOXES = 1, FX_ANN_MASKS = 2, FX_ANN_LABELS = 4 };
typedef struct fx_annotate_record {
  int32_t x0, y0, w, h;
  uint32_t colour;
  int32_t nchar;
  uint8_t glyph[FX_ANN_LMAX];
} fx_annotate_record;

int fx_annotate_labels_from_detections(const float* scores, const int32_t* labels, const int32_t* boxes, const int32_t* count, int B, int T,
                                       const uint8_t* name_glyphs, const int32_t* name_len, int K, int H, int W, int s, int gw, int gh,
                                       fx_annotate_record* rec, fx_stream_t stream);

int fx_annotate_u8(const uint8_t* src, uint8_t* dst, int B, int H, int W, int b0, int T, const int32_t* det_count, const int32_t* det_labels,
                   const int32_t* det_boxes, const int32_t* det_area, const int32_t* mask_words, int words_per_row, int64_t plane_stride_words,
                   const fx_annotate_record* rec, const uint32_t* atlas, int gw, int gh, int s, int flags, fx_stream_t stream);

#define FX_TRACK_MAX_SLOTS 1024
#define FX_TRACK_MAX_STREAMS 65535
int fx_track_update(const float* det_scores, const int32_t* det_labels, const int32_t* det_boxes, const int32_t* det_count, int B, int T,
                    int32_t* trk_id, int32_t* trk_label, int32_t* trk_tsu, int32_t* trk_hits, float* trk_box, float* trk_vel, int32_t* next_id,
                    int32_t* status, int max_tracks, float high, float low, float new_thresh, float match_iou, float second_iou,
                    int track_buffer, int min_hits, float alpha, int32_t* track_ids, fx_stream_t stream);
int fx_track_reset(int32_t* trk_id, int32_t* trk_label, int32_t* trk_tsu, int32_t* trk_hits, float* trk_box, float* trk_vel, int32_t* next_id,
                   int32_t* status, int B, int max_tracks, int b, fx_stream_t stream);

size_t fx_mask_rle_workspace_bytes(int B, int Q, int H, int W);
int fx_mask_rle_encode(const int32_t* mask_words, const int32_t* det_count, const int32_t* det_boxes, int B, int Q, int H, int W, int capacity,
                       int32_t* rle_len, int32_t* rle_off, int32_t* rle_counts, void* workspace, size_t workspace_bytes, fx_stream_t stream);

size_t fx_mask_polygon_workspace_bytes(int B, int Q, int H, int W, int max_edges);
int fx_mask_polygon_encode(const int32_t* mask_words, const int32_t* det_count, const int32_t* det_boxes, int B, int Q, int H, int W, int capacity,
                           int max_edges, int32_t* poly_len, int32_t* poly_off, int32_t* poly_pool, void* workspace, size_t workspace_bytes,
                           fx_stream_t stream);

#define FX_ZONE_MAX_REGIONS 32
#define FX_ZONE_MAX_VERTS 64
enum { FX_ZONE_POLYGON = 0, FX_ZONE_LINE = 1 };
enum { FX_ZONE_ANY_CLASS = 1 };
typedef struct fx_zone_region {
  int32_t kind, anchor, flags, vert_first, vert_count;
  uint32_t class_words[8];
  int32_t reserved[3];
} fx_zone_region;
int fx_zone_update(const int32_t* det_labels, const int32_t* det_boxes, const int32_t* det_count, int B, int T, const int32_t* track_ids,
                   const int32_t* trk_id, int max_tracks, const fx_zone_region* regions, const int32_t* reg_first, const int32_t* verts,
                   const fx_zone_region* regions_host, const int32_t* reg_first_host, const int32_t* verts_host, int R_total, int V_total,
                   int32_t* st_id, int32_t* st_side, int32_t* in_total, int32_t* out_total, int32_t* now, uint32_t* det_inside,
                   uint32_t* det_in, uint32_t* det_out, fx_stream_t stream);
int fx_zone_reset(int32_t* st_id, int32_t* st_side, int32_t* in_total, int32_t* out_total, const int32_t* reg_first_host, int B, int max_tracks,
                  int b, int clear_counters, fx_stream_t stream);

enum { FX_FRAME_RGB24 = 0, FX_FRAME_BGR24 = 1, FX_FRAME_NV12 = 2, FX_FRAME_I420 = 3 };
enum { FX_FRAME_BT601_LIMITED = 0, FX_FRAME_BT601_FULL = 1, FX_FRAME_BT709_LIMITED = 2, FX_FRAME_BT709_FULL = 3 };
#define FX_FRAME_MAX_DIM 16384
#define FX_FRAME_MAX_BATCH 65535
typedef struct fx_frame_desc {
  const uint8_t* plane[3];
  int32_t pitch[3];
  int32_t height, width;
  int32_t format;
  int32_t matrix;
  int32_t reserved[3];
} fx_frame_desc;
int fx_frames_ingest(const fx_frame_desc* descs, const fx_frame_desc* descs_host, int B, void* y, int out_f32, int Ho, int Wo, fx_stream_t stream);

int fx_frames_tile_gather_f32(const fx_frame_desc* descs, const fx_frame_desc* descs_host, int S, const int32_t* windows,
                              const int32_t* windows_host, int V, float* y, int Ho, int Wo, fx_stream_t stream);

int fx_roi_select(const float* det_scores, const int32_t* det_labels, const int32_t* det_boxes, const int32_t* det_count, int S, int T,
                  const int32_t* track_ids, const int32_t* trk_id, int max_tracks, const int32_t* at_id, const int32_t* at_frame,
                  const int32_t* frame, const fx_frame_desc* descs, const fx_frame_desc* descs_host, const uint32_t* class_words, int n_words,
                  int K, int pad_q, int min_size, float min_score, int interval, int32_t* roi_win, int32_t* roi_det, int32_t* roi_count,
                  int32_t* roi_left, fx_stream_t stream);
int fx_frames_roi_gather_f32(const fx_frame_desc* descs, const fx_frame_desc* descs_host, int S, const int32_t* roi_win, int K, float* y, int Ho,
                             int Wo, fx_stream_t stream);
int fx_roi_attributes(const float* logits, int C, const int32_t* roi_det, const int32_t* roi_count, int K, const int32_t* det_count, int S, int T,
                      const int32_t* track_ids, const int32_t* trk_id, int max_tracks, int32_t* at_id, int32_t* at_label, float* at_logit,
                      int32_t* at_frame, int32_t* frame, int hold, int32_t* attr_label, float* attr_logit, int32_t* attr_age, fx_stream_t stream);

#define FX_OVL_RNAME 16
#define FX_TRACE_MAX_LEN 64
enum { FX_OVL_FILL = 1, FX_OVL_STROKE = 2, FX_OVL_TRACES = 4 };
int fx_annotate_labels_tracked(const float* scores, const int32_t* labels, const int32_t* boxes, const int32_t* count, const int32_t* track_ids,
                               int B, int T, const uint8_t* name_glyphs, const int32_t* name_len, int K, int H, int W, int s, int gw, int gh,
                               fx_annotate_record* rec, fx_stream_t stream);
int fx_annotate_zone_records(const fx_zone_region* regions, const int32_t* reg_first, const int32_t* verts, const fx_zone_region* regions_host,
                             const int32_t* reg_first_host, const int32_t* verts_host, int R_total, int V_total, const uint8_t* name_glyphs,
                             const int32_t* name_len, const int32_t* in_total, const int32_t* out_total, const int32_t* now, int B, int H, int W,
                             int s, int gw, int gh, fx_annotate_record* rec, fx_stream_t stream);
int fx_annotate_overlay_u8(const uint8_t* src, uint8_t* dst, int B, int H, int W, int b0, int streams, const fx_zone_region* regions,
                           const int32_t* reg_first, const int32_t* verts, const fx_zone_region* regions_host, const int32_t* reg_first_host,
                           const int32_t* verts_host, int R_total, int V_total, const int32_t* trk_id, const int32_t* trace_id,
                           const int32_t* trace_label, const int32_t* trace_len, const int32_t* trace_head, const int32_t* trace_xy,
                           int max_tracks, int L, int s, int flags, fx_stream_t stream);
int fx_trace_update(const int32_t* det_labels, const int32_t* det_boxes, const int32_t* det_count, int B, int T, const int32_t* track_ids,
                    const int32_t* trk_id, int max_tracks, int L, int32_t* trace_id, int32_t* trace_label, int32_t* trace_len,
                    int32_t* trace_head, int32_t* trace_xy, fx_stream_t stream);
int fx_trace_reset(int32_t* trace_id, int32_t* trace_label, int32_t* trace_len, int32_t* trace_head, int B, int max_tracks, int b,
                   fx_stream_t stream);

#define FX_HEAT_ONE 256
enum { FX_HEAT_ANY_CLASS = 1, FX_HEAT_TRACKED_ONLY = 2 };
int fx_dwell_update(const int32_t* det_count, const int32_t* track_ids, const uint32_t* det_inside, int B, int T, const int32_t* trk_id,
                    int max_tracks, const int32_t* dw_first, const int32_t* dw_bit, const int32_t* dw_first_host, const int32_t* dw_region_host,
                    const int32_t* dw_bit_host, const int32_t* reg_first_host, int D_total, int32_t* dw_id, int32_t* dw_enter, int32_t* dw_last,
                    int32_t* visits, int64_t* dwell_sum, int32_t* dwell_max, int32_t* frame, int32_t* det_dwell, fx_stream_t stream);
int fx_dwell_reset(int32_t* dw_id, int32_t* dw_enter, int32_t* dw_last, int32_t* visits, int64_t* dwell_sum, int32_t* dwell_max, int32_t* frame,
                   const int32_t* dw_first_host, int B, int max_tracks, int b, int clear_totals, fx_stream_t stream);
int fx_heat_tiles(int H, int W, int cell);
int fx_heat_update(const int32_t* det_labels, const int32_t* det_boxes, const int32_t* det_count, const int32_t* track_ids, int B, int T, int H,
                   int W, int cell, int radius, int anchor, int decay_shift, int flags, const uint32_t* class_words_host, int32_t* heat,
                   int32_t* heat_max, int32_t* part, fx_stream_t stream);
int fx_annotate_heat_u8(const uint8_t* src, uint8_t* dst, int B, int H, int W, int b0, int streams, const int32_t* heat, const int32_t* heat_max,
                        int cell, int full_scale, const uint32_t* lut, fx_stream_t stream);

#define FX_REDACT_MAX_REGIONS 2048
#define FX_REDACT_MAX_RADIUS 32
#define FX_REDACT_MAX_HOLD 1024
enum { FX_REDACT_PIXELATE = 0, FX_REDACT_BLUR = 1, FX_REDACT_FILL = 2 };
enum { FX_REDACT_BOX = 0, FX_REDACT_ELLIPSE = 1, FX_REDACT_MASK = 2 };
int fx_redact_regions(const int32_t* det_labels, const int32_t* det_boxes, const int32_t* det_count, int B, int T, const uint32_t* class_words,
                      int K, const int32_t* trk_id, const int32_t* trk_label, const int32_t* trk_tsu, const float* trk_box, int max_tracks,
                      int hold, int pad256, int top256, int32_t* regions, int32_t* region_slot, int32_t* region_count, fx_stream_t stream);
int fx_redact_u8(const uint8_t* src, uint8_t* dst, int B, int H, int W, int b0, const int32_t* regions, const int32_t* region_slot,
                 const int32_t* region_count, int R, const int32_t* mask_words, int words_per_row, int64_t plane_stride_words, int T, int mode,
                 int shape, int cell, int radius, int colour, fx_stream_t stream);

int fx_maxpool3x3s2_nhwc_bf16(const void* x, int ldx, void* y, int ldy, int B, int H, int W, int C, fx_stream_t stream);
int fx_stem_conv_pool_supported(int C, int N, int H, int W);
int fx_stem_conv3x3_relu_maxpool_bf16(const void* x, int ldx, const void* w_frag, const float* bias, void* y, int ldy, int B, int H, int W,
                                      fx_stream_t stream);

int fx_avgpool2x2_nhwc_bf16(const void* x, int ldx, void* y, int ldy, int B, int H, int W, int C, fx_stream_t stream);

int fx_resize_bilinear_nhwc_bf16(const void* x, int ldx, void* y, int ldy, int B, int H, int W, int C, int Ho, int Wo,
                                 fx_stream_t stream);

int fx_add_rows_bf16(const void* x, int ldx, const void* y, int ldy_, int y_rows, void* out, int ldo, int rows, int cols,
                     fx_stream_t stream);

int fx_layernorm_bf16(const void* x, int ldx, const void* residual, int ldr, const float* gamma, const float* beta, void* out,
                      int ldo, int rows, int cols, fx_stream_t stream);

int fx_mha_bf16(const void* q, int ldq, const void* k, int ldk, const void* v, int ldv, void* out, int ldo, int B, int Lq, int Lk,
                int heads, fx_stream_t stream);

int fx_msda_bf16(const void* value, int ldv, const int32_t* spatial_shapes, const int32_t* level_start, int L, int P,
                 const float* loc, int ld_loc, const float* attn, int ld_attn, const float* ref, int mode, void* out, int ldo,
                 int B, int S, int Q, int M, fx_stream_t stream);

int fx_rowmax_f32(const float* x, int ldx, float* out, int rows, int cols, fx_stream_t stream);

int fx_enc_score_head_bf16(const void* memory, int ldm, const uint8_t* valid, int S, const void* w1, const float* b1,
                           const float* gamma, const float* beta, float eps, const void* w2, const float* b2, int n2_pad,
                           void* output_memory, int ldo, float* scores, int M, fx_stream_t stream);

typedef struct fx_rc_stage {
  int32_t type, K, N, act;
  int32_t src, dst, aux;
  int32_t ld, ld2, flags;
  const void* w;
  const float* bias;
  const float* gamma;
  const float* beta;
  void* g0;
  void* g1;
} fx_rc_stage;
int fx_row_chain(const fx_rc_stage* program_device, int n_stages, int rows, int lds_bytes, fx_stream_t stream);

int fx_topk_rows_f32(const float* scores, int ld, int B, int n, int k, float* out_val, int32_t* out_idx, fx_stream_t stream);
size_t fx_topk_rows_workspace_bytes(int B, int n, int k);
int fx_topk_rows_ws_f32(const float* scores, int ld, int B, int n, int k, float* out_val, int32_t* out_idx, void* workspace, size_t workspace_bytes,
                        fx_stream_t stream);

int fx_gather_rows_bf16(const void* src, int lds, int rows_per_batch, const int32_t* idx, int k, void* out, int ldo, int B, int cols,
                        fx_stream_t stream);

int fx_fill_rows_bf16(void* x, int ldx, int rows_per_batch, const int32_t* rows_idx, int n_idx, const void* row_bf16, int B, int cols,
                      fx_stream_t stream);

int fx_linear_k4_relu(const float* ref, const float* w, const float* b, void* out, int ldo, int rows, int N, fx_stream_t stream);

int fx_bbox_head(const void* h, int ldh, const float* w, const float* b, const float* ref, const float* anchors, const int32_t* idx,
                 int rows_per_batch, int mode, float* new_ref, float* unact_out, int rows, int K, fx_stream_t stream);

int fx_detr_head_out(const float* logits, int ldl, const float* ref_cxcywh, float* probs, float* boxes_xyxy, int rows, int K,
                     fx_stream_t stream);

int fx_detr_postprocess(const float* topk_val, const int32_t* topk_idx, const float* boxes_xyxy, const int32_t* sizes, int B, int Q,
                        int K, int top_k, float threshold, int32_t* labels, int32_t* queries, int32_t* boxes_i32, int32_t* count,
                        fx_stream_t stream);

int fx_mha_workspace_bytes(int B, int Lq, int Lk, int heads, int masked);
int fx_mha_masked_bf16(const void* q, int ldq, const void* k, int ldk, const void* v, int ldv, void* out, int ldo, int B, int Lq, int Lk,
                       int heads, const uint32_t* mask_bits, int ld_mask_words, void* workspace, size_t workspace_bytes, fx_stream_t stream);

int fx_upsample_nearest_add_nhwc_bf16(const void* lateral, int ldl, const void* top, int ldt, void* out, int ldo, int B, int H, int W,
                                      int Hs, int Ws, int C, fx_stream_t stream);
int fx_upsample_nearest_bwd_nhwc_bf16(const void* dy, int lddy, void* dtop, int lddt, int B, int H, int W, int Hs, int Ws, int C,
                                      fx_stream_t stream);

int fx_query_pixel_logits_bf16(const void* embed, int lde, const void* feat, int ldf, int mode, float* out, int ldo, uint32_t* bits,
                               int ld_words, int B, int Q, int P, int C, fx_stream_t stream);

int fx_mf_class_head(const float* logits, int ldl, float* probs, float* score, int32_t* label, int rows, int K, int use_sigmoid,
                     fx_stream_t stream);

int fx_mf_upsample_probs_f32(const float* lowres, int h, int w, float* out, int H, int W, int BQ, fx_stream_t stream);
int fx_mf_upsample_probs_bf16(const float* lowres, int h, int w, void* out, int H, int W, int BQ, fx_stream_t stream);

int fx_mf_postprocess_workspace_bytes(int B, int Q, int H);
size_t fx_mf_postprocess_workspace_bytes_fused(int B, int Q, int h, int w, int H, int W);
int fx_mf_postprocess(const float* mask_probs_lowres, int h, int w, int H, int W, const float* score, const int32_t* label, int B, int Q,
                      float mask_threshold, float threshold, int use_mask_score, void* workspace, size_t workspace_bytes,
                      int32_t* det_count, int32_t* det_query, float* det_score, int32_t* det_label, int32_t* det_box, int32_t* det_area,
                      uint32_t* mask_words, fx_stream_t stream);

int fx_point_sample_f32(const void* src, int src_is_u8, int H, int W, const int32_t* src_index, const float* coords, const int32_t* coord_index,
                        float* out, int R, int P, fx_stream_t stream);

int fx_mask_match_cost_f32(const float* logits, int ldl, const float* pred_pts, const float* tgt_pts, const int32_t* tgt_labels,
                           const int32_t* tgt_offsets, int B, int Q, int K, int P, int Tmax, float w_class, float w_mask, float w_dice,
                           int cls_sigmoid, float* cost, fx_stream_t stream);
size_t fx_mask_match_cost_workspace_bytes(int B, int Q, int Tmax);
int fx_mask_match_cost_ws_f32(const float* logits, int ldl, const float* pred_pts, const float* tgt_pts, const int32_t* tgt_labels,
                              const int32_t* tgt_offsets, int B, int Q, int K, int P, int Tmax, float w_class, float w_mask, float w_dice,
                              int cls_sigmoid, float* cost, void* workspace, size_t workspace_bytes, fx_stream_t stream);

size_t fx_mask_set_loss_workspace_bytes(int B, int Q, int sum_T, int n_over);
int fx_mask_set_loss_f32(const float* logits, int ldl, const float* pred_masks, int h, int w, const void* tgt_masks, int tgt_is_u8, int H, int W,
                         const int32_t* tgt_labels, const int32_t* tgt_offsets, int sum_T, const int32_t* pred_idx, const int32_t* tgt_idx,
                         const float* rand_over, int n_over, const float* rand_extra, int n_extra, int num_points, int B, int Q, int K,
                         float eos_coef, float num_masks, float w_ce, float w_mask, float w_dice, void* workspace, size_t workspace_bytes,
                         float* out3, fx_stream_t stream);
int fx_mask_set_loss_cls_f32(const float* logits, int ldl, const float* pred_masks, int h, int w, const void* tgt_masks, int tgt_is_u8, int H, int W,
                             const int32_t* tgt_labels, const int32_t* tgt_offsets, int sum_T, const int32_t* pred_idx, const int32_t* tgt_idx,
                             const float* rand_over, int n_over, const float* rand_extra, int n_extra, int num_points, int B, int Q, int K,
                             float eos_coef, int cls_mode, float focal_alpha, float focal_gamma, float num_masks, float w_ce, float w_mask,
                             float w_dice, void* workspace, size_t workspace_bytes, float* out3, fx_stream_t stream);
size_t fx_mask_class_loss_workspace_bytes(int B, int Q);
int fx_mask_class_loss_f32(const float* logits, int ldl, const int32_t* tgt_labels, const int32_t* tgt_offsets, const int32_t* pred_idx,
                           const int32_t* tgt_idx, int B, int Q, int K, int mode, float focal_alpha, float focal_gamma, float num_masks, float w_ce,
                           void* workspace, size_t workspace_bytes, float* out1, fx_stream_t stream);
int fx_mask_class_loss_bwd_f32(const float* logits, int ldl, const int32_t* tgt_labels, const int32_t* tgt_offsets, const int32_t* pred_idx,
                               const int32_t* tgt_idx, int B, int Q, int K, int mode, float focal_alpha, float focal_gamma, float num_masks,
                               float w_ce, const float* grad1, float* dlogits, int lddl, fx_stream_t stream);

int fx_dwconv3x3s2_nhwc_bf16(const void* x, int ldx, const float* w, const float* bias, void* y, int ldy, int B, int H, int W, int C,
                             fx_stream_t stream);
int fx_dwconv3x3s2_nhwc_f32out(const void* x, int ldx, const float* w, const float* bias, float* y, int ldy, int B, int H, int W, int C,
                               fx_stream_t stream);

int fx_global_mean_nhwc_bf16(const void* x, int ldx, float* out, int ldo, int B, int P, int C, fx_stream_t stream);

int fx_pooled_linear_f32(const float* in, int ldi, const float* W, const float* bias, int act, float* out, int ldo, int B, int C, int N,
                         fx_stream_t stream);

int fx_channel_gate_nhwc_bf16(const void* x, int ldx, const float* gate, int ldg, int self_add, const float* add_vec, int ldv,
                              const void* add_map, int ldm, void* y, int ldy, int B, int P, int C, fx_stream_t stream);

size_t fx_seg_postprocess_workspace_bytes(int B, int Q, int h, int w, int H, int W);
int fx_seg_postprocess(const float* mask_probs_lowres, int h, int w, int H, int W, const float* score, const int32_t* label, int B, int Q,
                       float threshold, int use_mask_score, void* workspace, size_t workspace_bytes, int32_t* det_count, int32_t* det_query,
                       float* det_score, int32_t* det_label, int32_t* det_box, int32_t* det_area, uint32_t* mask_words, uint8_t* winner_out,
                       fx_stream_t stream);

int fx_detr_match_cost_f32(const float* logits, int ldl, const float* boxes, const int32_t* tgt_labels, const float* tgt_boxes,
                           const int32_t* tgt_offsets, int B, int Q, int K, int Tmax, float w_class, float w_bbox, float w_giou, float alpha,
                           float gamma, float* cost, fx_stream_t stream);

int fx_lsa_f32(const float* cost, int B, int Q, int Tmax, const int32_t* tgt_offsets, int32_t* pred_idx, int32_t* tgt_idx, fx_stream_t stream);
int fx_lsa_status_f32(const float* cost, int B, int Q, int Tmax, const int32_t* tgt_offsets, int32_t* pred_idx, int32_t* tgt_idx, int32_t* status,
                      fx_stream_t stream);

int fx_detr_set_loss_workspace_bytes(int B, int Q, int sum_T);
int fx_detr_set_loss_f32(const float* logits, int ldl, const float* boxes, const int32_t* tgt_labels, const float* tgt_boxes,
                         const int32_t* tgt_offsets, const int32_t* pred_idx, const int32_t* tgt_idx, int B, int Q, int K, int sum_T,
                         float num_boxes, float focal_alpha, float focal_gamma, float w_vfl, float w_bbox, float w_giou, void* workspace,
                         float* out3, fx_stream_t stream);

int fx_detr_box_loss_f32(const float* boxes, const int32_t* tgt_labels, const float* tgt_boxes, const int32_t* tgt_offsets,
                         const int32_t* pred_idx, const int32_t* tgt_idx, int B, int Q, int K, int sum_T, float scale_bbox, float scale_giou,
                         int32_t* q_cls, float* q_score, float* loss2, float* pair_grad, fx_stream_t stream);
int fx_detr_box_loss_bwd_f32(const float* pair_grad, const int32_t* tgt_offsets, const int32_t* pred_idx, int B, int Q, int sum_T,
                             const float* g_bbox, const float* g_giou, float* dboxes, fx_stream_t stream);

int fx_msda_f32_fwd(const float* value, const int32_t* spatial_shapes, const int32_t* level_start, int L, int P, const float* loc,
                    const float* attn, float* out, int B, int S, int Q, int M, fx_stream_t stream);
int fx_msda_f32_bwd(const float* value, const int32_t* spatial_shapes, const int32_t* level_start, int L, int P, const float* loc,
                    const float* attn, const float* grad_out, float* grad_value, float* grad_loc, float* grad_attn, int B, int S, int Q, int M,
                    fx_stream_t stream);
int fx_msda_train_fwd(const void* value, int value_bf16, int ldv, const int32_t* spatial_shapes, const int32_t* level_start, int L, int P,
                      const float* loc, const float* attn, float* out, int B, int S, int Q, int M, fx_stream_t stream);
int fx_msda_train_bwd(const void* value, int value_bf16, int ldv, const int32_t* spatial_shapes, const int32_t* level_start, int L, int P,
                      const float* loc, const float* attn, const float* grad_out, float* grad_value, int ldg, int zero_grad_value,
                      float* grad_loc, float* grad_attn, int B, int S, int Q, int M, fx_stream_t stream);
int fx_msda_bwd_slab_supported(const int32_t* shapes_host, int L, int P, int Q, int M, int grad_out_bf16);
int fx_msda_train_bwd_slab(const void* value, int value_bf16, int ldv, const int32_t* spatial_shapes, const int32_t* level_start,
                           const int32_t* shapes_host, int L, int P, const float* loc, const float* attn, const void* grad_out,
                           int grad_out_bf16, void* grad_value_bf16, int ldg, float* grad_loc, float* grad_attn, int B, int S, int Q, int M,
                           fx_stream_t stream);

int fx_msda_prep_bf16(const void* off, int ld_off, const void* logit, int ld_logit, const float* ref, float* loc, float* aw, int BQ, int M, int L,
                      int P, fx_stream_t stream);
int fx_msda_prep_bwd_bf16(const float* grad_loc, const float* grad_attn, const float* aw, const float* ref, void* grad_off, int ld_off,
                          void* grad_logit, int ld_logit, int BQ, int M, int L, int P, fx_stream_t stream);

int fx_adamw_workspace_bytes(void);
// ... 168 lines not shown
```

Before: 5007 images/s.

## Fold bilinear upsample into CSP 1x1 conv and skip full encoder output store

Adds a pw_kplane variant that computes the 2x bilinear upsample of the lateral feature directly into the LDS A-tile, replacing a separate resize kernel and its write to the concat buffer. It also splits the encoder score head so the full output_memory tensor is no longer written. Only the top-k selected rows have their enc_output projection and layernorm recomputed, in a new gather-mode kernel. The cost is extra per-row index math in the conv prologue and a second small GEMM pass over the selected rows.

```diff
diff --git a/focoos_amd/_lib.py b/focoos_amd/_lib.py
--- a/focoos_amd/_lib.py
+++ b/focoos_amd/_lib.py
@@ -94,6 +94,7 @@
     "fx_device_info": [_i, C.POINTER(C.c_int), C.c_char_p, _i],
     "fx_conv2d_nhwc_bf16": [C.POINTER(FxConvDesc), _vp],
     "fx_conv2d_variant": [_vp, C.c_char_p, _i],
+    "fx_conv2d_up2_nhwc_bf16": [C.POINTER(FxConvDesc), _vp, _i, _i, _i, _i, _vp],
     "fx_pw_chain_supported": [_i, _i, _i, _i],
     "fx_pw_chain_pool_supported": [_i, _i, _i, _i],
     "fx_conv3x3_flat_supported": [_i, _i, _i],
@@ -172,6 +173,8 @@
     "fx_msda_bf16": [_vp, _i, _vp, _vp, _i, _i, _vp, _i, _vp, _i, _vp, _i, _vp, _i, _i, _i, _i, _i, _vp],
     "fx_rowmax_f32": [_vp, _i, _vp, _i, _i, _vp],
     "fx_enc_score_head_bf16": [_vp, _i, _vp, _i, _vp, _vp, _vp, _vp, _f, _vp, _vp, _i, _vp, _i, _vp, _i, _vp],
+    "fx_enc_score_head_scores_bf16": [_vp, _i, _vp, _i, _vp, _vp, _vp, _vp, _f, _vp, _vp, _i, _vp, _i, _vp],
+    "fx_enc_output_rows_bf16": [_vp, _i, _vp, _i, _vp, _vp, _vp, _vp, _f, _vp, _i, _vp, _i, _i, _vp],
     "fx_row_chain": [_vp, _i, _i, _i, _vp],
     "fx_topk_rows_f32": [_vp, _i, _i, _i, _i, _vp, _vp, _vp],
     "fx_topk_rows_workspace_bytes": [_i, _i, _i],
diff --git a/focoos_amd/csrc/conv_common.h b/focoos_amd/csrc/conv_common.h
--- a/focoos_amd/csrc/conv_common.h
+++ b/focoos_amd/csrc/conv_common.h
@@ -68,5 +68,8 @@
 int fx_launch_conv3x3s2_kplane(const ConvArgs& c, const bf16_t* w_frag, int mode, hipStream_t stream);
 bool fx_pw_kplane_supported(int C, int N, int mode);
 int fx_launch_pw_kplane(const ConvArgs& c, const bf16_t* w_frag, int mode, hipStream_t stream);
+bool fx_pw_kplane_up2_supported(int C, int N, int gC, int mode);
+int fx_launch_pw_kplane_up2(const ConvArgs& c, const bf16_t* w_frag, int mode, const bf16_t* g, int ldg, int gH, int gW, int gC,
+                            hipStream_t stream);
 bool fx_conv3x3_c32_supported(int C, int N, int W, int mode);
 int fx_launch_conv3x3_c32(const ConvArgs& c, const bf16_t* w_frag, int mode, hipStream_t stream);
diff --git a/focoos_amd/csrc/conv_igemm.hip b/focoos_amd/csrc/conv_igemm.hip
--- a/focoos_amd/csrc/conv_igemm.hip
+++ b/focoos_amd/csrc/conv_igemm.hip
@@ -377,6 +377,20 @@
   return kRoutes[r].launch(a, reinterpret_cast<const bf16_t*>(d->w_frag), mode, reinterpret_cast<hipStream_t>(stream));
 }
 
+extern "C" int fx_conv2d_up2_nhwc_bf16(const fx_conv_desc* d, const void* src, int ld_src, int Hs, int Ws, int Cs, fx_stream_t stream) {
+  ConvArgs a;
+  const int rc = conv_prepare(d, a);
+  if (rc != FX_OK) return rc;
+  FX_CHECK_ARG(src && ((uintptr_t)src % 16) == 0 && Hs > 0 && Ws > 0 && Cs > 0 && Cs % 8 == 0 && Cs < d->C && ld_src >= Cs && ld_src % 8 == 0);
+  if (d->H != 2 * Hs || d->W != 2 * Ws) return FX_ERR_UNSUPPORTED;
+  if (d->KH != 1 || d->KW != 1 || d->stride != 1 || d->pad != 0 || d->pool2 || d->mask || d->out_f32 || d->residual) return FX_ERR_UNSUPPORTED;
+  if (!d->w_frag || ((uintptr_t)d->w_frag % 16) != 0) return FX_ERR_UNSUPPORTED;
+  const int mode = fx_c3_epilogue_mode(a.act, false, 0);
+  if (!fx_pw_kplane_up2_supported(d->C, d->N, Cs, mode)) return FX_ERR_UNSUPPORTED;
+  return fx_launch_pw_kplane_up2(a, reinterpret_cast<const bf16_t*>(d->w_frag), mode, reinterpret_cast<const bf16_t*>(src), ld_src, Hs, Ws, Cs,
+                                 reinterpret_cast<hipStream_t>(stream));
+}
+
 extern "C" int fx_conv2d_variant(const fx_conv_desc* d, char* out, int cap) {
   FX_CHECK_ARG(out && cap >= 48);
   ConvArgs a;
diff --git a/focoos_amd/csrc/conv_pw_kplane.hip b/focoos_amd/csrc/conv_pw_kplane.hip
--- a/focoos_amd/csrc/conv_pw_kplane.hip
+++ b/focoos_amd/csrc/conv_pw_kplane.hip
@@ -1,4 +1,5 @@
 #include "kplane_common.h"
+#include "resize_common.h"
 
 #ifndef FX_PWK_RES_DEPTH
 #define FX_PWK_RES_DEPTH 3
@@ -18,9 +19,12 @@
   int64_t y_bstride;
   unsigned x_bytes, r_bytes;
   int rot;
+  const bf16_t* g;
+  int ldg, gH, gW, Ho, Wo;
+  float gsh, gsw;
 };
 
-template <int K, int ACT, int RESMODE, int TM = 4, int ABL = 0>
+template <int K, int ACT, int RESMODE, int TM = 4, int ABL = 0, int GP = 0>
 __global__ __launch_bounds__(256, TM == 4 ? 2 : 3) void conv_pw_kplane_kernel(const PWKArgs p) {
   constexpr int TN = 2, NW = 4, BM = TM * 32, BN = 256;
   constexpr int NTHR = 256, NDW = NTHR / 64;
@@ -46,11 +50,40 @@
     const __amdgpu_buffer_rsrc_t xr = __builtin_amdgcn_make_buffer_rsrc((void*)p.x, 0, p.x_bytes, 0x00020000);
     constexpr int NP = K / 8;
     static_assert(BM % 64 == 0, "64-row DMA blocks");
+    static_assert(GP >= 0 && GP < NP, "at least one fetched piece");
     for (int i = wave; i < (BM / 64) * NP; i += NDW) {
       const int blk = i / NP, c = i % NP;
+      if (GP > 0 && c < GP) continue;
       const int m = m0 + blk * 64 + lane;
       const int pln = (c & 1) * KS + (c >> 1);
       if constexpr (!(ABL & 16)) pw_dma16(xr, smem + pln * PLANE + blk * 1024, m < p.M ? (unsigned)(m * p.ldx + c * 8) * 2u : FX_OOB);
+    }
+    if constexpr (GP > 0) {
+      static_assert(GP % 8 == 0 && BM <= NTHR, "whole 128-byte lines; one thread per table row");
+      unsigned char* rowp = smem + XBYTES + p.N * 4;
+      if (tid < BM) {
+        const int m = min(m0 + tid, p.M - 1);
+        const int b = m / p.HW, rem = m - b * p.HW;
+        const int ho = rem / p.Wo, wo = rem - ho * p.Wo;
+        int h0, h1, w0, w1;
+        float lh0, lh1, lw0, lw1;
+        fx_resize_src(ho, p.gsh, p.gH, h0, h1, lh0, lh1);
+        fx_resize_src(wo, p.gsw, p.gW, w0, w1, lw0, lw1);
+        const int r0 = (b * p.gH + h0) * p.gW, r1 = (b * p.gH + h1) * p.gW;
+        *reinterpret_cast<int4*>(rowp + tid * 32) = make_int4((r0 + w0) * p.ldg, (r0 + w1) * p.ldg, (r1 + w0) * p.ldg, (r1 + w1) * p.ldg);
+        *reinterpret_cast<float4*>(rowp + tid * 32 + 16) = make_float4(lh0, lh1, lw0, lw1);
+      }
+      __syncthreads();
+      constexpr int NPG = GP / 8;
+      const int c_lo = (lane & 3) | ((lane >> 5) << 2), rl = (lane >> 2) & 7;
+#pragma unroll 4
+      for (int it = wave; it < (BM / 8) * NPG; it += NDW) {
+        const int row = (it / NPG) * 8 + rl, c = (it % NPG) * 8 + c_lo;
+        const int4 o = *reinterpret_cast<const int4*>(rowp + row * 32);
+        const float4 l = *reinterpret_cast<const float4*>(rowp + row * 32 + 16);
+        const int pln = (c & 1) * KS + (c >> 1);
+        *reinterpret_cast<uint4*>(smem + pln * PLANE + row * 16) = fx_resize_vec8_nhwc(p.g + c * 8, o.x, o.y, o.z, o.w, l.x, l.y, l.z, l.w);
+      }
     }
   }
   f32x16 acc[TN][TM];
@@ -184,10 +217,10 @@
   }
 }
 
-template <int K, int ACT, int RESMODE, int TM = 4, int ABL = 0>
+template <int K, int ACT, int RESMODE, int TM = 4, int ABL = 0, int GP = 0>
 static int launch_pwk(PWKArgs& a, hipStream_t stream) {
   constexpr int BM = TM * 32, BN = 256;
-  const int smem = BM * K * 2 + a.N * 4;
+  const int smem = BM * K * 2 + a.N * 4 + (GP > 0 ? BM * 32 : 0);
   if (smem > 160 * 1024) return FX_ERR_UNSUPPORTED;
   const int mt = (a.M + BM - 1) / BM, NT = a.N / BN;
   static const int target = fx_tune("FX_PWK_TARGET_WGS", 512);
@@ -198,7 +231,7 @@
   groups = (NT + a.ntg - 1) / a.ntg;
   static const int rot = fx_tune("FX_PWK_ROT", 1);
   a.rot = rot;
-  auto kern = conv_pw_kplane_kernel<K, ACT, RESMODE, TM, ABL>;
+  auto kern = conv_pw_kplane_kernel<K, ACT, RESMODE, TM, ABL, GP>;
   static int attr_smem = 0;
   if (!fx_ensure_dyn_smem(reinterpret_cast<const void*>(kern), smem, attr_smem)) return FX_ERR_RUNTIME;
   hipLaunchKernelGGL(kern, dim3(mt, groups), dim3(256), smem, stream, a);
@@ -240,3 +273,20 @@
   }
   return FX_ERR_UNSUPPORTED;
 }
+
+bool fx_pw_kplane_up2_supported(int C, int N, int gC, int mode) { return C == 512 && gC == 256 && mode == 1 && fx_pw_kplane_supported(C, N, mode); }
+
+int fx_launch_pw_kplane_up2(const ConvArgs& c, const bf16_t* w_frag, int mode, const bf16_t* g, int ldg, int gH, int gW, int gC,
+                            hipStream_t stream) {
+  if (!fx_pw_kplane_up2_supported(c.C, c.N, gC, mode) || c.H != 2 * gH || c.W != 2 * gW) return FX_ERR_UNSUPPORTED;
+  if ((int64_t)c.B * gH * gW * ldg >= (1ll << 31)) return FX_ERR_UNSUPPORTED;
+  PWKArgs a{};
+  a.x = c.x; a.wp = w_frag; a.bias = c.bias; a.res = nullptr; a.y = reinterpret_cast<bf16_t*>(c.y);
+  a.N = c.N; a.ldx = c.ldx; a.ldy = c.ldy; a.ldr = 0; a.M = c.M;
+  a.HW = c.Ho * c.Wo; a.y_bstride = c.y_bstride; a.x_bytes = c.x_bytes; a.r_bytes = 0;
+  a.g = g; a.ldg = ldg; a.gH = gH; a.gW = gW; a.Ho = c.Ho; a.Wo = c.Wo;
+  a.gsh = (float)gH / (float)c.Ho; a.gsw = (float)gW / (float)c.Wo;
+  static const int bm64 = fx_tune("FX_UP2_BM64", 1);
+  if (bm64) return launch_pwk<512, FX_ACT_SILU, 0, 2, 0, 32>(a, stream);
+  return launch_pwk<512, FX_ACT_SILU, 0, 4, 0, 32>(a, stream);
+}
diff --git a/focoos_amd/csrc/pixel_ops.hip b/focoos_amd/csrc/pixel_ops.hip
--- a/focoos_amd/csrc/pixel_ops.hip
+++ b/focoos_amd/csrc/pixel_ops.hip
@@ -1,6 +1,7 @@
 #include <stdlib.h>
 
 #include "common.h"
+#include "resize_common.h"
 
 static int fx_env_int(const char* name, int dflt) {
   const char* v = getenv(name);
@@ -265,17 +266,12 @@
   const unsigned c8 = t - wo * (unsigned)C8;
   int h0, h1, w0, w1;
   float lh0, lh1, lw0, lw1;
-  bilinear_src((int)ho, sh, H, h0, h1, lh0, lh1);
-  bilinear_src((int)wo, sw, W, w0, w1, lw0, lw1);
+  fx_resize_src((int)ho, sh, H, h0, h1, lh0, lh1);
+  fx_resize_src((int)wo, sw, W, w0, w1, lw0, lw1);
   const bf16_t* base = x + (int64_t)b * H * W * ldx + c8 * 8;
-  float f00[8], f01[8], f10[8], f11[8], o[8];
-  unpack_bf16x8(*reinterpret_cast<const uint4*>(base + ((int64_t)h0 * W + w0) * ldx), f00);
-  unpack_bf16x8(*reinterpret_cast<const uint4*>(base + ((int64_t)h0 * W + w1) * ldx), f01);
-  unpack_bf16x8(*reinterpret_cast<const uint4*>(base + ((int64_t)h1 * W + w0) * ldx), f10);
-  unpack_bf16x8(*reinterpret_cast<const uint4*>(base + ((int64_t)h1 * W + w1) * ldx), f11);
-#pragma unroll
-  for (int j = 0; j < 8; ++j) o[j] = lh0 * (lw0 * f00[j] + lw1 * f01[j]) + lh1 * (lw0 * f10[j] + lw1 * f11[j]);
-  *reinterpret_cast<uint4*>(y + ((int64_t)row * Wo + wo) * ldy + c8 * 8) = pack_bf16x8(o);
+  *reinterpret_cast<uint4*>(y + ((int64_t)row * Wo + wo) * ldy + c8 * 8) =
+      fx_resize_vec8_nhwc(base, ((int64_t)h0 * W + w0) * ldx, ((int64_t)h0 * W + w1) * ldx, ((int64_t)h1 * W + w0) * ldx,
+                          ((int64_t)h1 * W + w1) * ldx, lh0, lh1, lw0, lw1);
 }
 
 extern "C" int fx_resize_bilinear_nhwc_bf16(const void* x, int ldx, void* y, int ldy, int B, int H, int W, int C, int Ho, int Wo,
diff --git a/focoos_amd/csrc/resize_common.h b/focoos_amd/csrc/resize_common.h
--- a/focoos_amd/csrc/resize_common.h
+++ b/focoos_amd/csrc/resize_common.h
@@ -18,6 +18,24 @@
   return fmaf(lh0, top, lh1 * bottom);
 }
 
+__device__ __forceinline__ float fx_resize_blend_nhwc(float lh0, float lh1, float lw0, float lw1, float f00, float f01, float f10, float f11) {
+#pragma clang fp contract(off)
+  const float top = fmaf(lw0, f00, lw1 * f01), bottom = fmaf(lw0, f10, lw1 * f11);
+  return fmaf(lh0, top, lh1 * bottom);
+}
+
+__device__ __forceinline__ uint4 fx_resize_vec8_nhwc(const bf16_t* base, int64_t o00, int64_t o01, int64_t o10, int64_t o11, float lh0, float lh1,
+                                                     float lw0, float lw1) {
+  float f00[8], f01[8], f10[8], f11[8], o[8];
+  unpack_bf16x8(*reinterpret_cast<const uint4*>(base + o00), f00);
+  unpack_bf16x8(*reinterpret_cast<const uint4*>(base + o01), f01);
+  unpack_bf16x8(*reinterpret_cast<const uint4*>(base + o10), f10);
+  unpack_bf16x8(*reinterpret_cast<const uint4*>(base + o11), f11);
+#pragma unroll
+  for (int j = 0; j < 8; ++j) o[j] = fx_resize_blend_nhwc(lh0, lh1, lw0, lw1, f00[j], f01[j], f10[j], f11[j]);
+  return pack_bf16x8(o);
+}
+
 static inline bool fx_windows_ok(const int32_t* wh, int N, int H, int W) {
   for (int i = 0; i < N; ++i) {
     const int x0 = wh[4 * i], y0 = wh[4 * i + 1], w = wh[4 * i + 2], h = wh[4 * i + 3];
diff --git a/focoos_amd/csrc/score_head.hip b/focoos_amd/csrc/score_head.hip
--- a/focoos_amd/csrc/score_head.hip
+++ b/focoos_amd/csrc/score_head.hip
@@ -14,9 +14,11 @@
   int ldm, ldo, S, M;
   float eps;
   unsigned mem_bytes;
+  const int* rows;
+  int Q;
 };
 
-template <int TN2>
+template <int TN2, int MODE = 0>
 __global__ __launch_bounds__(256, 2) void score_head_kernel(const ScoreHeadArgs p) {
   constexpr int BM = 64, TM = 2, KS = 16, PF = 4;
   extern __shared__ __attribute__((aligned(16))) unsigned char smem[];
@@ -35,8 +37,15 @@
     const int lc = pc ^ (row & 15);
     const int m = m0 + row;
     bool ok = m < p.M;
-    if (ok && p.valid) ok = p.valid[m % p.S] != 0;
-    pw_dma16(mr, T + i * 1024, ok ? (unsigned)(m * p.ldm + lc * 8) * 2u : FX_OOB);
+    int src = m, tok;
+    if constexpr (MODE == 2) {
+      tok = min(max(p.rows[ok ? m : 0], 0), p.S - 1);
+      src = (m / p.Q) * p.S + tok;
+    } else {
+      tok = m % p.S;
+    }
+    if (ok && p.valid) ok = p.valid[tok] != 0;
+    pw_dma16(mr, T + i * 1024, ok ? (unsigned)(src * p.ldm + lc * 8) * 2u : FX_OOB);
   }
 
   f32x16 acc[2][TM];
@@ -83,10 +92,12 @@
   }
   const bf16_t* w2 = p.w2p + (size_t)(wave * TN2 * KS) * 512 + lane * 8;
   bf16x8 a2[PF][TN2];
-#pragma unroll
-  for (int i = 0; i < PF; ++i)
-#pragma unroll
-    for (int a = 0; a < TN2; ++a) a2[i][a] = pw_ldg_frag(w2 + (size_t)(a * KS + i) * 512);
+  if constexpr (MODE != 2) {
+#pragma unroll
+    for (int i = 0; i < PF; ++i)
+#pragma unroll
+      for (int a = 0; a < TN2; ++a) a2[i][a] = pw_ldg_frag(w2 + (size_t)(a * KS + i) * 512);
+  }
 
   float mean[TM], rstd[TM];
   {
@@ -158,14 +169,17 @@
       }
     }
   __syncthreads();
-#pragma unroll
-  for (int i = 0; i < BM * 32 / 256; ++i) {
-    const int q = tid + i * 256;
-    const int row = q >> 5, lc = q & 31;
-    const uint4 v = *reinterpret_cast<const uint4*>(T + row * 512 + ((lc ^ (row & 15)) << 4));
-    const int m = m0 + row;
-    if (m < p.M) *reinterpret_cast<uint4*>(p.om + (size_t)m * p.ldo + lc * 8) = v;
-  }
+  if constexpr (MODE != 1) {
+#pragma unroll
+    for (int i = 0; i < BM * 32 / 256; ++i) {
+      const int q = tid + i * 256;
+      const int row = q >> 5, lc = q & 31;
+      const uint4 v = *reinterpret_cast<const uint4*>(T + row * 512 + ((lc ^ (row & 15)) << 4));
+      const int m = m0 + row;
+      if (m < p.M) *reinterpret_cast<uint4*>(p.om + (size_t)m * p.ldo + lc * 8) = v;
+    }
+  }
+  if constexpr (MODE == 2) return;
   f32x16 acc2[TN2][TM];
 #pragma unroll
   for (int a = 0; a < TN2; ++a)
@@ -219,26 +233,31 @@
   if (tid < BM && m0 + tid < p.M) p.scores[m0 + tid] = fmaxf(fmaxf(red[tid], red[64 + tid]), fmaxf(red[128 + tid], red[192 + tid]));
 }
 
-template <int TN2>
+template <int TN2, int MODE = 0>
 static int launch_score_head(const ScoreHeadArgs& a, hipStream_t stream) {
   constexpr int SMEM = 64 * 512 + 4 * 64 * 4;
-  auto kern = score_head_kernel<TN2>;
+  auto kern = score_head_kernel<TN2, MODE>;
   static int attr_smem = 0;
   if (!fx_ensure_dyn_smem(reinterpret_cast<const void*>(kern), SMEM, attr_smem)) return FX_ERR_RUNTIME;
   hipLaunchKernelGGL(kern, dim3((a.M + 63) / 64), dim3(256), SMEM, stream, a);
   return fx_launch_status();
 }
 
-extern "C" int fx_enc_score_head_bf16(const void* memory, int ldm, const uint8_t* valid, int S, const void* w1, const float* b1,
-                                      const float* gamma, const float* beta, float eps, const void* w2, const float* b2, int n2_pad,
-                                      void* output_memory, int ldo, float* scores, int M, fx_stream_t stream_) {
-  FX_CHECK_ARG(memory && w1 && b1 && gamma && beta && w2 && b2 && output_memory && scores && M > 0 && S > 0);
-  FX_CHECK_ARG(ldm >= 256 && ldm % 8 == 0 && ldo >= 256 && ldo % 8 == 0);
-  FX_CHECK_ARG(((uintptr_t)memory % 16) == 0 && ((uintptr_t)w1 % 16) == 0 && ((uintptr_t)w2 % 16) == 0 && ((uintptr_t)output_memory % 16) == 0);
-  FX_CHECK_ARG(((uintptr_t)b1 % 16) == 0 && ((uintptr_t)b2 % 16) == 0 && ((uintptr_t)gamma % 16) == 0 && ((uintptr_t)beta % 16) == 0);
-  if (n2_pad != 128 && n2_pad != 256 && n2_pad != 384) return FX_ERR_UNSUPPORTED;
-  const int64_t mem_bytes = ((int64_t)M - 1) * ldm * 2 + 512;
-  if (mem_bytes >= 0xFFFFFFF0ll) return FX_ERR_UNSUPPORTED;
+static int score_head_launch(const void* memory, int ldm, const uint8_t* valid, int S, const void* w1, const float* b1, const float* gamma,
+                             const float* beta, float eps, const void* w2, const float* b2, int n2_pad, void* output_memory, int ldo, float* scores,
+                             int M, const int* rows, int Q, int64_t mem_rows, fx_stream_t stream_) {
+  FX_CHECK_ARG(memory && w1 && b1 && gamma && beta && M > 0 && S > 0);
+  FX_CHECK_ARG(ldm >= 256 && ldm % 8 == 0 && ((uintptr_t)memory % 16) == 0 && ((uintptr_t)w1 % 16) == 0);
+  FX_CHECK_ARG(((uintptr_t)b1 % 16) == 0 && ((uintptr_t)gamma % 16) == 0 && ((uintptr_t)beta % 16) == 0);
+  FX_CHECK_ARG(!output_memory || (ldo >= 256 && ldo % 8 == 0 && ((uintptr_t)output_memory % 16) == 0));
+  if (rows) {
+    FX_CHECK_ARG(output_memory && Q > 0 && M % Q == 0);
+  } else {
+    FX_CHECK_ARG(w2 && b2 && scores && ((uintptr_t)w2 % 16) == 0 && ((uintptr_t)b2 % 16) == 0);
+    if (n2_pad != 128 && n2_pad != 256 && n2_pad != 384) return FX_ERR_UNSUPPORTED;
+  }
+  const int64_t mem_bytes = (mem_rows - 1) * ldm * 2 + 512;
+  if (mem_bytes >= 0xFFFFFFF0ll || mem_rows >= (1ll << 31)) return FX_ERR_UNSUPPORTED;
   ScoreHeadArgs a;
   a.mem = reinterpret_cast<const bf16_t*>(memory);
   a.valid = valid;
@@ -249,8 +268,36 @@
   a.scores = scores;
   a.ldm = ldm; a.ldo = ldo; a.S = S; a.M = M; a.eps = eps;
   a.mem_bytes = (unsigned)mem_bytes;
+  a.rows = rows; a.Q = Q;
   hipStream_t stream = reinterpret_cast<hipStream_t>(stream_);
+  if (rows) return launch_score_head<1, 2>(a, stream);
+  if (!output_memory) {
+    if (n2_pad == 128) return launch_score_head<1, 1>(a, stream);
+    if (n2_pad == 256) return launch_score_head<2, 1>(a, stream);
+    return launch_score_head<3, 1>(a, stream);
+  }
   if (n2_pad == 128) return launch_score_head<1>(a, stream);
   if (n2_pad == 256) return launch_score_head<2>(a, stream);
   return launch_score_head<3>(a, stream);
 }
+
+extern "C" int fx_enc_score_head_bf16(const void* memory, int ldm, const uint8_t* valid, int S, const void* w1, const float* b1,
+                                      const float* gamma, const float* beta, float eps, const void* w2, const float* b2, int n2_pad,
+                                      void* output_memory, int ldo, float* scores, int M, fx_stream_t stream_) {
+  FX_CHECK_ARG(output_memory);
+  return score_head_launch(memory, ldm, valid, S, w1, b1, gamma, beta, eps, w2, b2, n2_pad, output_memory, ldo, scores, M, nullptr, 0, M, stream_);
+}
+
+extern "C" int fx_enc_score_head_scores_bf16(const void* memory, int ldm, const uint8_t* valid, int S, const void* w1, const float* b1,
+                                             const float* gamma, const float* beta, float eps, const void* w2, const float* b2, int n2_pad,
+                                             float* scores, int M, fx_stream_t stream_) {
+  return score_head_launch(memory, ldm, valid, S, w1, b1, gamma, beta, eps, w2, b2, n2_pad, nullptr, 0, scores, M, nullptr, 0, M, stream_);
+}
+
+extern "C" int fx_enc_output_rows_bf16(const void* memory, int ldm, const uint8_t* valid, int S, const void* w1, const float* b1,
+                                       const float* gamma, const float* beta, float eps, const int32_t* rows, int Q, void* out, int ldo, int B,
+                                       fx_stream_t stream_) {
+  FX_CHECK_ARG(rows && B > 0 && Q > 0 && (int64_t)B * Q < (1ll << 31));
+  return score_head_launch(memory, ldm, valid, S, w1, b1, gamma, beta, eps, nullptr, nullptr, 0, out, ldo, nullptr, B * Q, rows, Q, (int64_t)B * S,
+                           stream_);
+}
diff --git a/focoos_amd/engine.py b/focoos_amd/engine.py
--- a/focoos_amd/engine.py
+++ b/focoos_amd/engine.py
@@ -704,7 +704,7 @@
 
     def conv(self, x: NT, pc: PackedConv, out: Optional[NT] = None, name: Optional[str] = None, stride: int = 1, act=None,
              residual: Optional[NT] = None, res_after: bool = False, pool2: bool = False, out_f32: bool = False,
-             y_batch_stride: int = 0, extra_flops_per_pixel: float = 0.0) -> NT:
+             y_batch_stride: int = 0, extra_flops_per_pixel: float = 0.0, up2_src: Optional[NT] = None) -> NT:
         assert x.C == pc.C, (name, x.C, pc.C)
         pad = (pc.KH - 1) // 2
         if pool2:
@@ -736,10 +736,31 @@
         variant = label.value.decode()
         alg_bytes = 2.0 * x.B * x.H * x.W * pc.C + (4.0 if out_f32 else 2.0) * M * pc.N + (2.0 * M * pc.N if residual is not None else 0.0) \
             + 2.0 * pc.N * pc.KH * pc.KW * pc.C
+        if up2_src is not None:
+            s = up2_src
+            assert variant.startswith("pw_kplane<") and (s.B, 2 * s.H, 2 * s.W) == (x.B, x.H, x.W), (name, variant)
+            alg_bytes += 2.0 * s.B * s.H * s.W * s.C - 2.0 * x.B * x.H * x.W * s.C
+            variant += "+up2"
         self.meta[len(self.ops)] = {"kind": "conv", "variant": variant, "flops": flops, "flops_executed": flops - extra_flops_per_pixel * M, "bytes": alg_bytes,
                                     "name": name or "slice", "M": M, "N": pc.N, "K": pc.KH * pc.KW * pc.C}
-        self._op(self.lib.fx_conv2d_nhwc_bf16, C.byref(d))
+        if up2_src is not None:
+            self._op(self.lib.fx_conv2d_up2_nhwc_bf16, C.byref(d), s.ptr, s.ld, s.H, s.W, s.C)
+        else:
+            self._op(self.lib.fx_conv2d_nhwc_bf16, C.byref(d))
         return out
+
+    def fold_up2(self, src: NT, cat: NT, pc: PackedConv) -> bool:
+        if os.environ.get("FX_FOLD_UPSAMPLE", "1") == "0" or pc.wf is None or pc.KH != 1:
+            return False
+        if (cat.H, cat.W) != (2 * src.H, 2 * src.W) or (cat.C, src.C, pc.C) != (512, 256, 512) or pc.N % 256 != 0:
+            return False
+        d = FxConvDesc()
+        d.x, d.w, d.bias, d.y, d.w_frag = cat.ptr, pc.w.data_ptr(), pc.b.data_ptr(), cat.ptr, pc.wf.data_ptr()
+        d.B, d.H, d.W, d.C, d.ldx = cat.B, cat.H, cat.W, cat.C, cat.ld
+        d.Ho, d.Wo, d.N, d.ldy = cat.H, cat.W, pc.N, (pc.N + 7) // 8 * 8
+        d.KH, d.KW, d.stride, d.pad, d.act = 1, 1, 1, 0, FX_ACT["silu"]
+        label = C.create_string_buffer(64)
+        return self.lib.fx_conv2d_variant(C.byref(d), label, 64) == 0 and label.value.decode() == "pw_kplane<K512>"
 
     def pw_chain(self, x1: NT, x2: Optional[NT], residual: Optional[NT], cc: Tuple, ca: Optional[Tuple], name1: str, name2: Optional[str],
                  pool_name: Optional[str] = None, keep_y1: bool = True):
@@ -966,8 +987,8 @@
             self.bufs["aifi"] = s
             src = NT(s.t, B, h32, w32, 256, 256, s.off)
 
-        def csp(xin: NT, p: str, out_name: str) -> NT:
-            c12 = self.conv(xin, P[f"{p}.conv12"], name=f"{p}.c12", act="silu")
+        def csp(xin: NT, p: str, out_name: str, up2_src: Optional[NT] = None) -> NT:
+            c12 = self.conv(xin, P[f"{p}.conv12"], name=f"{p}.c12", act="silu", up2_src=up2_src)
             x1 = c12.slice(0, fd)
             for j in range(3):
                 last = j == 2
@@ -977,11 +998,15 @@
             return x1
 
         lat0 = self.conv(src, P[f"{pd}.lateral_convs.0"], out=cat20.slice(fd, fd), act="silu")
-        self.resize(lat0, cat40a.slice(0, fd))
-        fpn0 = csp(cat40a, f"{pd}.fpn_blocks.0", "fpn0")
+        def top_down(lat: NT, cat: NT, p: str, out_name: str) -> NT:
+            if self.fold_up2(lat, cat, P[f"{p}.conv12"]):
+                return csp(cat, p, out_name, up2_src=lat)
+            self.resize(lat, cat.slice(0, fd))
+            return csp(cat, p, out_name)
+
+        fpn0 = top_down(lat0, cat40a, f"{pd}.fpn_blocks.0", "fpn0")
         lat1 = self.conv(fpn0, P[f"{pd}.lateral_convs.1"], out=cat40b.slice(fd, fd), act="silu")
-        self.resize(lat1, cat80.slice(0, fd))
-        out80 = csp(cat80, f"{pd}.fpn_blocks.1", "enc_s8")
+        out80 = top_down(lat1, cat80, f"{pd}.fpn_blocks.1", "enc_s8")
         d0 = self._new("down0", B, h16, w16, fd)
         self.resize(out80, d0)
         self.conv(d0, P[f"{pd}.downsample_convs.0"], out=cat40b.slice(0, fd), act="silu")
@@ -1012,12 +1037,17 @@
             valid = torch.ones(S, dtype=torch.uint8)
             valid[invalid.long()] = 0
             self.valid_u8 = valid.to(self.dev)
-            om = self._new("output_memory", B * S, 1, 1, 256)
+            no_om = os.environ.get("FX_SCORE_NO_OM", "1") != "0"
+            om = None if no_om else self._new("output_memory", B * S, 1, 1, 256)
             g_, b_ = e.ln[f"{hp}.enc_output.1"]
-            self.meta[len(self.ops)] = {"kind": "conv", "variant": f"score_head<{ncp}>", "flops": 2.0 * B * S * 256 * (256 + K), "name": "enc_output+enc_score+max",
-                                        "M": B * S, "N": 256 + K, "K": 256, "bytes": 2.0 * B * S * 256 * 2 + 4.0 * B * S}
-            self._op(lib.fx_enc_score_head_bf16, mem_rows.ptr, mem_rows.ld, self.valid_u8.data_ptr(), S, w1.data_ptr(), b1.data_ptr(), g_.data_ptr(),
-                     b_.data_ptr(), C.c_float(1e-5), w2.data_ptr(), b2.data_ptr(), ncp, om.ptr, om.ld, self.enc_scores.data_ptr(), B * S)
+            self.meta[len(self.ops)] = {"kind": "conv", "variant": f"score_head<{ncp}>" + ("-om" if no_om else ""), "flops": 2.0 * B * S * 256 * (256 + K),
+                                        "name": "enc_output+enc_score+max", "M": B * S, "N": 256 + K, "K": 256,
+                                        "bytes": 2.0 * B * S * 256 * (1 if no_om else 2) + 4.0 * B * S}
+            head = (mem_rows.ptr, mem_rows.ld, self.valid_u8.data_ptr(), S, w1.data_ptr(), b1.data_ptr(), g_.data_ptr(), b_.data_ptr(), C.c_float(1e-5))
+            if no_om:
+                self._op(lib.fx_enc_score_head_scores_bf16, *head, w2.data_ptr(), b2.data_ptr(), ncp, self.enc_scores.data_ptr(), B * S)
+            else:
+                self._op(lib.fx_enc_score_head_bf16, *head, w2.data_ptr(), b2.data_ptr(), ncp, om.ptr, om.ld, self.enc_scores.data_ptr(), B * S)
         else:
             om_lin = self.linear(mem_rows, P[f"{hp}.enc_output.0"], name="om_lin")
             om = self.layernorm(om_lin, f"{hp}.enc_output.1", "output_memory")
@@ -1030,7 +1060,13 @@
         self.split_at = len(self.ops)
         R = B * Q
         tgt = self._new("target", R, 1, 1, 256)
-        self._op(lib.fx_gather_rows_bf16, om.ptr, om.ld, S, self.enc_topk.data_ptr(), Q, tgt.ptr, tgt.ld, B, 256)
+        if om is None:
+            self.meta[len(self.ops)] = {"kind": "conv", "variant": "score_head<rows>", "flops": 2.0 * R * 256 * 256, "name": "enc_output(selected rows)",
+                                        "M": R, "N": 256, "K": 256, "bytes": 2.0 * R * 256 * 2}
+            self._op(lib.fx_enc_output_rows_bf16, *head, self.enc_topk.data_ptr(), Q, tgt.ptr, tgt.ld, B)
+            self.bufs["output_memory"] = tgt
+        else:
+            self._op(lib.fx_gather_rows_bf16, om.ptr, om.ld, S, self.enc_topk.data_ptr(), Q, tgt.ptr, tgt.ld, B, 256)
         hb = self.linear(tgt, P[f"{hp}.enc_bbox.0"], name="encbb.0", act="relu")
         hb = self.linear(hb, P[f"{hp}.enc_bbox.1"], name="encbb.1", act="relu")
         self.ref_unact = torch.empty(R, 4, dtype=torch.float32, device=self.dev)
diff --git a/include/focoos_amd.h b/include/focoos_amd.h
--- a/include/focoos_amd.h
+++ b/include/focoos_amd.h
@@ -41,6 +41,7 @@
 } fx_conv_desc;
 int fx_conv2d_nhwc_bf16(const fx_conv_desc* d, fx_stream_t stream);
 int fx_conv2d_variant(const fx_conv_desc* d, char* out, int cap);
+int fx_conv2d_up2_nhwc_bf16(const fx_conv_desc* d, const void* src, int ld_src, int Hs, int Ws, int Cs, fx_stream_t stream);
 int fx_conv3x3_flat_supported(int C, int N, int W);
 
 typedef struct fx_pw_chain_desc {
@@ -295,6 +296,11 @@
 int fx_enc_score_head_bf16(const void* memory, int ldm, const uint8_t* valid, int S, const void* w1, const float* b1,
                            const float* gamma, const float* beta, float eps, const void* w2, const float* b2, int n2_pad,
                            void* output_memory, int ldo, float* scores, int M, fx_stream_t stream);
+int fx_enc_score_head_scores_bf16(const void* memory, int ldm, const uint8_t* valid, int S, const void* w1, const float* b1,
+                                  const float* gamma, const float* beta, float eps, const void* w2, const float* b2, int n2_pad,
+                                  float* scores, int M, fx_stream_t stream);
+int fx_enc_output_rows_bf16(const void* memory, int ldm, const uint8_t* valid, int S, const void* w1, const float* b1, const float* gamma,
+                            const float* beta, float eps, const int32_t* rows, int Q, void* out, int ldo, int B, fx_stream_t stream);
 
 typedef struct fx_rc_stage {
   int32_t type, K, N, act;
```

Measured after the change: 5128 images/s (median of 3 runs). 2.4% higher.
